# MisEty/RTG-SLAM

Measured on AMD Instinct MI355X. Metric: hot_path_units_per_sec, higher is better.
Workload: dtype f32; 1 GPU; `value` counts UNITS, not SLAM frames (the SLAM frame rate by the reference's definition is `slam_frames_per_sec`, from the `slam_sequence` leg of --full).  One UNIT per step = 1 ICP track (3 levels x 5 GN iters, 1200x680, on a second HIP stream) + 1 map-optimisation iteration (raster fwd + masked L1 colour / gated depth loss + attach regulariser + raster bwd + fused Adam) over 1200000 random Gaus; gaussians=1200000, mode=single, parallelism=1 GPU

## Files before the change

include/rtgs_raster.h:

```cpp
#ifndef RTGS_RASTER_H
#define RTGS_RASTER_H

#include <stddef.h>
#include <stdint.h>

#ifdef __cplusplus
extern "C" {
#endif

#define RTGS_OK 0
#define RTGS_E_INVALID (-1)
#define RTGS_E_HIP (-2)
#define RTGS_E_ALLOC (-3)

#define RTGS_TILE 16

typedef struct rtgs_raster_settings {
  int32_t image_height;
  int32_t image_width;
  float tanfovx;
  float tanfovy;
  const float* bg;
  float scale_modifier;
  const float* viewmatrix;
// ... 168 lines not shown
                       float* m_raw8, float* v_raw8, const float* lr_xyz, const float* lr_shs, const float* lr_raw8,
                       uint8_t* ever_xyz, uint8_t* ever_shs, uint8_t* ever_raw8, int64_t rows, int32_t step, float beta1,
                       float beta2, float eps, const rtgs_attach* attach, float* confidence, const uint32_t* skip_flag,
                       const rtgs_activated* refresh, void* stream);

typedef struct rtgs_loss_cfg {
  float color_weight, depth_weight, ssim_weight, add_depth_thres;
  const uint8_t* render_mask;
  int32_t sums_zeroed;
} rtgs_loss_cfg;
size_t rtgs_slam_loss_scratch_bytes(int32_t H, int32_t W, int32_t with_ssim);
int rtgs_slam_loss(const float* color, const float* depth, const int32_t* depth_index, const float* gt_color,
                   const float* gt_depth, int32_t H, int32_t W, const rtgs_loss_cfg* cfg, void* scratch,
                   float* loss_out4, float* g_color, float* g_depth, void* stream);
int rtgs_slam_loss_sums(const float* color, const float* depth, const int32_t* depth_index, const float* gt_color,
                        const float* gt_depth, int32_t H, int32_t W, const rtgs_loss_cfg* cfg, void* scratch, void* stream);
int rtgs_slam_loss_grads(const float* color, const float* depth, const int32_t* depth_index, const float* gt_color,
                         const float* gt_depth, int32_t H, int32_t W, const rtgs_loss_cfg* cfg, void* scratch,
                         float* loss_out4, float* g_color, float* g_depth, void* stream);

typedef struct rtgs_map_step_args {
  const rtgs_raster_settings* settings;
  int32_t P, sh_coeffs;
  float *xyz, *shs, *raw8;
  const int32_t* tile_mask;
  const float *gt_color, *gt_depth;
  rtgs_loss_cfg loss;
  void* loss_scratch;
  float *opacity, *scales, *rotations, *normal;
  float *out_color, *out_depth;
  int32_t *out_color_index, *out_depth_index;
  float *out_color_weight, *out_depth_weight, *out_T;
  int32_t* out_radii;
  float *dL_dcolor, *dL_ddepth, *loss4;
  float *d_xyz, *d_opacity, *d_shs, *d_scales, *d_rotations, *d_normal, *d_raw8;
  void* grad_scratch;
  uint8_t* row_state;
  float *m_xyz, *v_xyz, *m_shs, *v_shs, *m_raw8, *v_raw8;
  const float *lr_xyz, *lr_shs, *lr_raw8;
  uint8_t *ever_xyz, *ever_shs, *ever_raw8;
  int32_t step;
  float beta1, beta2, eps;
  const rtgs_attach* attach;
  float* confidence;
  int32_t activated_valid;
  rtgs_resize_fn geom_resize; void* geom_user;
  rtgs_resize_fn binning_resize; void* binning_user;
  rtgs_resize_fn image_resize; void* image_user;
  float normal_weight;
  const float* gt_normal;
  int32_t train_begin, train_end;
  int32_t tail_mode;
  uint32_t* live_counts;
} rtgs_map_step_args;
int rtgs_slam_normal_loss(const float* normal_w, const int32_t* depth_index, const float* gt_normal,
                          const uint8_t* render_mask, int32_t H, int32_t W, float normal_weight, float* scratch2,
                          float* loss_out4, float* d_normal, uint8_t* row_state, const uint32_t* skip_flag, void* stream);
int rtgs_slam_normal_loss_range(const float* normal_w, const int32_t* depth_index, const float* gt_normal,
                                const uint8_t* render_mask, int32_t H, int32_t W, float normal_weight, float* scratch2,
                                float* loss_out4, float* d_normal, uint8_t* row_state, const uint32_t* skip_flag,
                                int32_t train_begin, int32_t train_end, void* stream);
int rtgs_slam_normal_loss_sums(const float* normal_w, const int32_t* depth_index, const float* gt_normal,
                               const uint8_t* render_mask, int32_t H, int32_t W, float* scratch2, const uint32_t* skip_flag,
                               void* stream);
int rtgs_slam_normal_loss_grads(const float* normal_w, const int32_t* depth_index, const float* gt_normal,
                                const uint8_t* render_mask, int32_t H, int32_t W, float normal_weight, const float* sums2,
                                float* loss_out4, float* d_normal, uint8_t* row_state, const uint32_t* skip_flag,
                                int32_t train_begin, int32_t train_end, void* stream);
int rtgs_slam_map_step(const rtgs_map_step_args* args, int64_t* num_rendered_host, void* stream);
void* rtgs_stream_create_reserving(int32_t reserve_cus);
void rtgs_stream_destroy(void* stream);
int rtgs_map_fused_tail(const rtgs_raster_settings* settings, const rtgs_map_step_args* args, void* geom_buffer,
                        const void* image_buffer, const uint32_t* spec_fail, uint32_t* live_counts2, void* stream);
int rtgs_map_fused_tail_hint(const rtgs_raster_settings* settings, const rtgs_map_step_args* args, void* geom_buffer,
                             const void* image_buffer, const uint32_t* spec_fail, uint32_t* live_counts2,
                             uint32_t listed_hint, void* stream);
uint32_t rtgs_raster_last_listed_ctx(rtgs_ctx* ctx);
int rtgs_raster_backward_buffers(int32_t P, int32_t image_height, int32_t image_width, size_t* out8_host);
int rtgs_raster_last_buffers_ctx(rtgs_ctx* ctx, void** out3_host);
void rtgs_raster_set_aux_zero_ctx(rtgs_ctx* ctx, void* eight_words);
int rtgs_slam_map_step_front(const rtgs_map_step_args* args, int64_t* num_rendered_host, void* stream);
int rtgs_slam_map_step_ctx(rtgs_ctx* ctx, const rtgs_map_step_args* args, int64_t* num_rendered_host, void* stream);
int rtgs_slam_map_step_front_ctx(rtgs_ctx* ctx, const rtgs_map_step_args* args, int64_t* num_rendered_host, void* stream);

int rtgs_rows_pack(const uint8_t* row_state, int32_t P, float* d_xyz, float* d_shs, float* d_opacity, float* d_scales,
                   float* d_rotations, float* d_normal, float* out_list, int32_t capacity, uint32_t* count_scratch,
                   void* stream);
int rtgs_rows_overflow(const float* gathered_lists, int32_t world, int32_t capacity, uint32_t* flag_and_counts, void* stream);
int rtgs_rows_apply(const float* list, int32_t capacity, int32_t mode, float* d_xyz, float* d_shs, float* d_opacity,
                    float* d_scales, float* d_rotations, float* d_normal, uint8_t* row_state, const uint32_t* skip_flag,
                    void* stream);

size_t rtgs_map_step_args_size(void);
size_t rtgs_raster_settings_size(void);

const char* rtgs_version(void);

#ifdef __cplusplus
}
#endif
#endif
```

rtg_slam_amd/_lib.py:

```python
from __future__ import annotations

import ctypes as C
import os
import threading

_HERE = os.path.dirname(os.path.abspath(__file__))
LIB_PATH = os.environ.get("RTGS_LIB_PATH") or os.path.join(_HERE, "librtgs_hip.so")

RESIZE_FN = C.CFUNCTYPE(C.c_void_p, C.c_void_p, C.c_size_t)
FWD_NO_BACKWARD = 1


class RasterSettingsC(C.Structure):
    _fields_ = [
        ("image_height", C.c_int32), ("image_width", C.c_int32),
        ("tanfovx", C.c_float), ("tanfovy", C.c_float),
        ("bg", C.c_void_p), ("scale_modifier", C.c_float),
        ("viewmatrix", C.c_void_p), ("projmatrix", C.c_void_p),
        ("sh_degree", C.c_int32), ("campos", C.c_void_p),
        ("opaque_threshold", C.c_float), ("depth_threshold", C.c_float),
        ("normal_threshold", C.c_float), ("color_sigma", C.c_float),
        ("prefiltered", C.c_int32), ("debug", C.c_int32),
        ("cx", C.c_float), ("cy", C.c_float), ("T_threshold", C.c_float),
    ]


class IcpLevelC(C.Structure):
    _fields_ = [
        ("H", C.c_int32), ("W", C.c_int32), ("downscale", C.c_float), ("iters", C.c_int32),
        ("vertex_src", C.c_void_p), ("normal_src", C.c_void_p),
        ("vertex_tgt", C.c_void_p), ("normal_tgt", C.c_void_p),
    ]


_lock = threading.Lock()
_lib = None

_P = C.c_void_p


class LossCfgC(C.Structure):
    _fields_ = [("color_weight", C.c_float), ("depth_weight", C.c_float), ("ssim_weight", C.c_float),
                ("add_depth_thres", C.c_float), ("render_mask", C.c_void_p), ("sums_zeroed", C.c_int32)]


class AttachC(C.Structure):
    _fields_ = [("init_xyz", C.c_void_p), ("init_raw8", C.c_void_p), ("attach_info", C.c_void_p)]


class ActivatedC(C.Structure):
    _fields_ = [(n, C.c_void_p) for n in ("opacity", "scales", "rotations", "normal")]


class MapStepArgsC(C.Structure):
    _fields_ = (
        [("settings", C.POINTER(RasterSettingsC)), ("P", C.c_int32), ("sh_coeffs", C.c_int32)]
        + [(n, C.c_void_p) for n in ("xyz", "shs", "raw8", "tile_mask", "gt_color", "gt_depth")]
        + [("loss", LossCfgC), ("loss_scratch", C.c_void_p)]
        + [(n, C.c_void_p) for n in (
            "opacity", "scales", "rotations", "normal", "out_color", "out_depth", "out_color_index", "out_depth_index",
            "out_color_weight", "out_depth_weight", "out_T", "out_radii", "dL_dcolor", "dL_ddepth", "loss4",
            "d_xyz", "d_opacity", "d_shs", "d_scales", "d_rotations", "d_normal", "d_raw8", "grad_scratch", "row_state",
            "m_xyz", "v_xyz", "m_shs", "v_shs", "m_raw8", "v_raw8", "lr_xyz", "lr_shs", "lr_raw8",
            "ever_xyz", "ever_shs", "ever_raw8")]
        + [("step", C.c_int32), ("beta1", C.c_float), ("beta2", C.c_float), ("eps", C.c_float)]
        + [("attach", C.POINTER(AttachC)), ("confidence", C.c_void_p), ("activated_valid", C.c_int32)]
        + [("geom_resize", RESIZE_FN), ("geom_user", C.c_void_p), ("binning_resize", RESIZE_FN),
           ("binning_user", C.c_void_p), ("image_resize", RESIZE_FN), ("image_user", C.c_void_p)]
        + [("normal_weight", C.c_float), ("gt_normal", C.c_void_p), ("train_begin", C.c_int32), ("train_end", C.c_int32),
           ("tail_mode", C.c_int32), ("live_counts", C.c_void_p)])


_SIGNATURES = {
    "rtgs_version": (C.c_char_p, []),
    "rtgs_raster_forward": (C.c_int, [C.POINTER(RasterSettingsC), C.c_int32, C.c_int32] + [_P] * 6 + [_P]
                            + [_P] * 8 + [RESIZE_FN, _P, RESIZE_FN, _P, RESIZE_FN, _P,
                                          C.POINTER(C.c_int64), _P]),
    "rtgs_raster_backward": (C.c_int, [C.POINTER(RasterSettingsC), C.c_int32, C.c_int32, C.c_int64] + [_P] * 6
                             + [_P] * 3 + [_P, _P, _P] + [_P, _P] + [_P] * 6 + [_P, _P]),
    "rtgs_raster_backward_rows": (C.c_int, [C.POINTER(RasterSettingsC), C.c_int32, C.c_int32, C.c_int64] + [_P] * 6
                                  + [_P] * 3 + [_P, _P, _P] + [_P, _P] + [_P] * 6 + [_P, _P, _P]),
    "rtgs_raster_backward_scratch_bytes": (C.c_size_t, [C.c_int32]),
    "rtgs_raster_geom_bytes": (C.c_size_t, [C.c_int32, C.c_int32, C.c_int32]),
    "rtgs_raster_binning_bytes": (C.c_size_t, [C.c_int64, C.c_int32, C.c_int32]),
    "rtgs_raster_image_bytes": (C.c_size_t, [C.c_int32, C.c_int32]),
    "rtgs_raster_last_stats": (C.c_int, [C.POINTER(C.c_int64)]),
    "rtgs_raster_set_counters": (None, [_P]),
    "rtgs_fused_adam": (C.c_int, [_P, _P, _P, _P, _P, C.c_int64, C.c_int32, C.c_int32, C.c_float, C.c_float, C.c_float, _P]),
    "rtgs_fused_adam_rows": (C.c_int, [_P, _P, _P, _P, _P, _P, _P, C.c_int64, C.c_int32, C.c_int32, C.c_float, C.c_float, C.c_float, _P]),
    "rtgs_map_activate8_forward": (C.c_int, [_P, C.c_int64, _P, _P, _P, _P, _P]),
    "rtgs_map_activate8_backward": (C.c_int, [_P, C.c_int64, _P, _P, _P, _P, _P, _P]),
    "rtgs_map_activate8_backward_rows": (C.c_int, [_P, C.c_int64, _P, _P, _P, _P, _P, _P, _P]),
    "rtgs_map_tail_rows": (C.c_int, [_P] * 23 + [C.c_int64, C.c_int32, C.c_float, C.c_float, C.c_float,
                                     C.POINTER(AttachC), _P, _P, C.POINTER(ActivatedC), _P]),
    "rtgs_attach_prepare": (C.c_int, [_P, _P, C.POINTER(AttachC), C.c_int64, _P]),
    "rtgs_history_merge": (C.c_int, [_P] * 8 + [C.c_int64, C.c_float, _P]),
    "rtgs_map_fused_tail": (C.c_int, [C.POINTER(RasterSettingsC), C.POINTER(MapStepArgsC), _P, _P, _P, _P, _P]),
    "rtgs_map_fused_tail_hint": (C.c_int, [C.POINTER(RasterSettingsC), C.POINTER(MapStepArgsC), _P, _P, _P, _P, C.c_uint32, _P]),
    "rtgs_raster_last_listed_ctx": (C.c_uint32, [_P]),
    "rtgs_stream_create_reserving": (C.c_void_p, [C.c_int]),
    "rtgs_stream_destroy": (None, [_P]),
    "rtgs_raster_backward_buffers": (C.c_int, [C.c_int32, C.c_int32, C.c_int32, C.POINTER(C.c_size_t)]),
    "rtgs_raster_last_buffers_ctx": (C.c_int, [_P, C.POINTER(C.c_void_p)]),
    "rtgs_raster_set_aux_zero_ctx": (None, [_P, _P]),
    "rtgs_raster_backward_walk_ctx": (C.c_int, [_P, C.POINTER(RasterSettingsC), C.c_int32, C.c_int32, C.c_int64] + [_P] * 6
                                      + [_P] * 3 + [_P, _P, _P] + [_P, _P] + [_P] * 6 + [_P, _P, C.c_int32, C.c_int32, _P]),
    "rtgs_slam_loss_scratch_bytes": (C.c_size_t, [C.c_int32, C.c_int32, C.c_int32]),
    "rtgs_slam_map_step_front": (C.c_int, [C.POINTER(MapStepArgsC), C.POINTER(C.c_int64), _P]),
    "rtgs_rows_pack": (C.c_int, [_P, C.c_int32] + [_P] * 7 + [C.c_int32, _P, _P]),
    "rtgs_rows_overflow": (C.c_int, [_P, C.c_int32, C.c_int32, _P, _P]),
    "rtgs_rows_apply": (C.c_int, [_P, C.c_int32, C.c_int32] + [_P] * 7 + [_P, _P]),
    "rtgs_map_step_args_size": (C.c_size_t, []),
    "rtgs_raster_settings_size": (C.c_size_t, []),
    "rtgs_slam_map_step": (C.c_int, [C.POINTER(MapStepArgsC), C.POINTER(C.c_int64), _P]),
    "rtgs_slam_loss": (C.c_int, [_P, _P, _P, _P, _P, C.c_int32, C.c_int32, C.POINTER(LossCfgC), _P, _P, _P, _P, _P]),
    "rtgs_slam_normal_loss": (C.c_int, [_P, _P, _P, _P, C.c_int32, C.c_int32, C.c_float, _P, _P, _P, _P, _P, _P]),
    "rtgs_slam_loss_sums": (C.c_int, [_P, _P, _P, _P, _P, C.c_int32, C.c_int32, C.POINTER(LossCfgC), _P, _P]),
    "rtgs_slam_loss_grads": (C.c_int, [_P, _P, _P, _P, _P, C.c_int32, C.c_int32, C.POINTER(LossCfgC), _P, _P, _P, _P, _P]),
    "rtgs_raster_set_profiling": (None, [C.c_int]),
    "rtgs_raster_force_sort_path": (None, [C.c_int]),
    "rtgs_raster_set_near_slice": (None, [C.c_int, C.c_int]),
    "rtgs_raster_last_slice_stats": (C.c_int, [C.POINTER(C.c_int64)]),
    "rtgs_raster_last_timings": (C.c_int, [C.POINTER(C.c_float)]),
    "rtgs_ctx_create": (C.c_void_p, []),
    "rtgs_ctx_destroy": (None, [_P]),
    "rtgs_raster_forward_ctx": (C.c_int, [_P, C.POINTER(RasterSettingsC), C.c_int32, C.c_int32] + [_P] * 6 + [_P]
                                + [_P] * 8 + [RESIZE_FN, _P, RESIZE_FN, _P, RESIZE_FN, _P, C.POINTER(C.c_int64),
                                              C.c_int32, _P]),
    "rtgs_raster_backward_ctx": (C.c_int, [_P, C.POINTER(RasterSettingsC), C.c_int32, C.c_int32, C.c_int64] + [_P] * 6
                                 + [_P] * 3 + [_P, _P, _P] + [_P, _P] + [_P] * 6 + [_P, _P]),
    "rtgs_raster_backward_rows_ctx": (C.c_int, [_P, C.POINTER(RasterSettingsC), C.c_int32, C.c_int32, C.c_int64] + [_P] * 6
                                      + [_P] * 3 + [_P, _P, _P] + [_P, _P] + [_P] * 6 + [_P, _P, _P]),
    "rtgs_raster_backward_range_ctx": (C.c_int, [_P, C.POINTER(RasterSettingsC), C.c_int32, C.c_int32, C.c_int64] + [_P] * 6
                                       + [_P] * 3 + [_P, _P, _P] + [_P, _P] + [_P] * 6 + [_P, _P, C.c_int32, C.c_int32, _P]),
    "rtgs_slam_normal_loss_range": (C.c_int, [_P, _P, _P, _P, C.c_int32, C.c_int32, C.c_float, _P, _P, _P, _P, _P,
                                              C.c_int32, C.c_int32, _P]),
    "rtgs_slam_normal_loss_sums": (C.c_int, [_P, _P, _P, _P, C.c_int32, C.c_int32, _P, _P, _P]),
    "rtgs_slam_normal_loss_grads": (C.c_int, [_P, _P, _P, _P, C.c_int32, C.c_int32, C.c_float, _P, _P, _P, _P, _P,
                                              C.c_int32, C.c_int32, _P]),
    "rtgs_raster_geom_bytes_ctx": (C.c_size_t, [_P, C.c_int32, C.c_int32, C.c_int32]),
    "rtgs_raster_last_stats_ctx": (C.c_int, [_P, C.POINTER(C.c_int64)]),
    "rtgs_raster_set_counters_ctx": (None, [_P, _P]),
    "rtgs_raster_set_profiling_ctx": (None, [_P, C.c_int]),
    "rtgs_raster_force_sort_path_ctx": (None, [_P, C.c_int]),
    "rtgs_raster_set_bwd_walk_ctx": (None, [_P, C.c_int]),
    "rtgs_raster_set_bwd_debug": (None, [C.c_int]),
    "rtgs_raster_set_bwd_stamps": (None, [C.c_void_p]),
    "rtgs_raster_set_fwd_stamps": (None, [C.c_void_p]),
    "rtgs_icp_set_stamps": (None, [C.c_void_p]),
    "rtgs_raster_set_onepass_ctx": (None, [_P, C.c_int]),
    "rtgs_raster_forward_verify_ctx": (C.c_int, [_P, C.POINTER(C.c_int64)]),
    "rtgs_raster_spec_fail_ptr_ctx": (C.c_void_p, [_P]),
    "rtgs_raster_set_speculation_ctx": (None, [_P, C.c_int]),
    "rtgs_raster_speculation_stats_ctx": (C.c_int, [_P, C.POINTER(C.c_int64)]),
    "rtgs_raster_plain_stats_ctx": (C.c_int, [_P, C.POINTER(C.c_int64)]),
    "rtgs_raster_set_plain_onepass_ctx": (None, [_P, C.c_int]),
    "rtgs_raster_image_offsets": (C.c_int, [C.c_int32, C.c_int32, C.POINTER(C.c_size_t)]),
# ... 96 lines not shown
```

rtg_slam_amd/csrc/map_step.hip:

```cpp
#include <hip/hip_runtime.h>

#include "../../include/rtgs_raster.h"

static int map_step_front(rtgs_ctx* ctx, const rtgs_map_step_args* a, int64_t* num_rendered_host, int32_t fwd_flags,
                          void* stream, bool walk_only = false) {
  if (!a || !num_rendered_host || !a->settings) return RTGS_E_INVALID;
  const int32_t P = a->P, M = a->sh_coeffs;
  if (P <= 0 || M != 16 || a->step < 1) return RTGS_E_INVALID;
  if (!a->xyz || !a->shs || !a->raw8 || !a->tile_mask || !a->gt_color || !a->gt_depth) return RTGS_E_INVALID;
  const int32_t H = a->settings->image_height, W = a->settings->image_width;
  int rc = 0;
  if (!a->activated_valid) {
    rc = rtgs_map_activate8_forward(a->raw8, P, a->opacity, a->scales, a->rotations, a->normal, stream);
    if (rc != 0) return RTGS_E_HIP;
  }
  if (!a->loss_scratch || !a->loss4) return RTGS_E_INVALID;
  rtgs_raster_set_aux_zero_ctx(ctx, a->loss_scratch);
  rc = rtgs_raster_forward_ctx(ctx, a->settings, P, M, a->xyz, a->opacity, a->shs, a->scales, a->rotations, a->normal,
                           a->tile_mask, a->out_color, a->out_depth, a->out_color_index, a->out_depth_index,
                           a->out_color_weight, a->out_depth_weight, a->out_T, a->out_radii, a->geom_resize,
                           a->geom_user, a->binning_resize, a->binning_user, a->image_resize, a->image_user,
                           num_rendered_host, fwd_flags, stream);
  if (rc != RTGS_OK) return rc;
  void* bufs[3];
  if (rtgs_raster_last_buffers_ctx(ctx, bufs) != RTGS_OK) return RTGS_E_ALLOC;
  void *geom = bufs[0], *bin = bufs[1], *img = bufs[2];
  rtgs_loss_cfg lcfg = a->loss;
  lcfg.sums_zeroed = P > 0 ? 1 : 0;
  rc = rtgs_slam_loss(a->out_color, a->out_depth, a->out_depth_index, a->gt_color, a->gt_depth, H, W, &lcfg,
                      a->loss_scratch, a->loss4, a->dL_dcolor, a->dL_ddepth, stream);
  if (rc != 0) return RTGS_E_HIP;
  int32_t t0 = 0, t1 = P;
  if (a->train_begin != 0 || a->train_end != 0) { t0 = a->train_begin; t1 = a->train_end; }
  if (t0 < 0 || t1 > P || t1 < t0) return RTGS_E_INVALID;
  if (t1 == t0) return RTGS_OK;
  rc = (walk_only ? rtgs_raster_backward_walk_ctx : rtgs_raster_backward_range_ctx)(
      ctx, a->settings, P, M, *num_rendered_host, a->xyz, a->opacity, a->shs, a->scales, a->rotations, a->normal, geom, bin, img,
      a->out_color, a->out_T, a->out_depth_index, a->dL_dcolor, a->dL_ddepth, a->d_xyz, a->d_opacity, a->d_shs, a->d_scales,
      a->d_rotations, a->d_normal, a->grad_scratch, a->row_state, t0, t1, stream);
  if (rc != RTGS_OK) return rc;
  if (a->normal_weight > 0.f && a->gt_normal) {
    rc = rtgs_slam_normal_loss_range(a->normal, a->out_depth_index, a->gt_normal, a->loss.render_mask, H, W, a->normal_weight,
                                     reinterpret_cast<float*>(a->loss_scratch) + 5, a->loss4, a->d_normal, a->row_state,
                                     rtgs_raster_spec_fail_ptr_ctx(ctx), t0, t1, stream);
    if (rc != 0) return RTGS_E_HIP;
  }
  return RTGS_OK;
}

extern "C" int rtgs_slam_map_step_front_ctx(rtgs_ctx* ctx, const rtgs_map_step_args* a, int64_t* num_rendered_host,
                                            void* stream) {
  return map_step_front(ctx, a, num_rendered_host, 0, stream);
}

extern "C" int rtgs_slam_map_step_front(const rtgs_map_step_args* a, int64_t* num_rendered_host, void* stream) {
  return rtgs_slam_map_step_front_ctx(nullptr, a, num_rendered_host, stream);
}

static int map_step_once(rtgs_ctx* ctx, const rtgs_map_step_args* a, int64_t* num_rendered_host, bool speculate, void* stream) {
  const bool fused = a->tail_mode == 0 && !(a->normal_weight > 0.f && a->gt_normal);
  int rc = map_step_front(ctx, a, num_rendered_host, speculate ? RTGS_FWD_SPECULATE : 0, stream, fused);
  if (rc != RTGS_OK) return rc;
  if ((a->train_begin != 0 || a->train_end != 0) && a->train_end == a->train_begin) return RTGS_OK;
  if (fused) {
    void* bufs[3];
    if (rtgs_raster_last_buffers_ctx(ctx, bufs) != RTGS_OK) return RTGS_E_ALLOC;
    return rtgs_map_fused_tail_hint(a->settings, a, bufs[0], bufs[2], rtgs_raster_spec_fail_ptr_ctx(ctx), a->live_counts,
                                    rtgs_raster_last_listed_ctx(ctx), stream);
  }
  const int32_t P = a->P;
  int32_t t0 = 0, t1 = P;
  if (a->train_begin != 0 || a->train_end != 0) { t0 = a->train_begin; t1 = a->train_end; }
  const size_t o = (size_t)t0;
  const rtgs_activated act{a->opacity + o, a->scales + 3 * o, a->rotations + 4 * o, a->normal + 3 * o};
  rc = rtgs_map_tail_rows(a->xyz + 3 * o, a->shs + 48 * o, a->raw8 + 8 * o, a->d_opacity + o, a->d_scales + 3 * o,
                          a->d_rotations + 4 * o, a->d_normal + 3 * o, a->d_xyz + 3 * o, a->d_shs + 48 * o, a->d_raw8 + 8 * o,
                          a->row_state + o, a->m_xyz, a->v_xyz, a->m_shs, a->v_shs, a->m_raw8, a->v_raw8,
                          a->lr_xyz, a->lr_shs, a->lr_raw8, a->ever_xyz, a->ever_shs, a->ever_raw8, (int64_t)(t1 - t0), a->step,
                          a->beta1, a->beta2, a->eps, a->attach, a->confidence, rtgs_raster_spec_fail_ptr_ctx(ctx), &act, stream);
  return rc != 0 ? RTGS_E_HIP : RTGS_OK;
}

extern "C" int rtgs_slam_map_step_ctx(rtgs_ctx* ctx, const rtgs_map_step_args* a, int64_t* num_rendered_host, void* stream) {
  int rc = map_step_once(ctx, a, num_rendered_host, true, stream);
  const int v = rtgs_raster_forward_verify_ctx(ctx, num_rendered_host);
  if (rc != RTGS_OK) return rc;
  if (v < 0) return v;
  if (v == 1) rc = map_step_once(ctx, a, num_rendered_host, false, stream);
  return rc;
}

extern "C" int rtgs_slam_map_step(const rtgs_map_step_args* a, int64_t* num_rendered_host, void* stream) {
  return rtgs_slam_map_step_ctx(nullptr, a, num_rendered_host, stream);
}

extern "C" size_t rtgs_map_step_args_size(void) { return sizeof(rtgs_map_step_args); }
extern "C" size_t rtgs_raster_settings_size(void) { return sizeof(rtgs_raster_settings); }

extern "C" void* rtgs_stream_create_reserving(int32_t reserve_cus) {
  int dev = 0, cus = 0;
  if (hipGetDevice(&dev) != hipSuccess) return nullptr;
  if (hipDeviceGetAttribute(&cus, hipDeviceAttributeMultiprocessorCount, dev) != hipSuccess) return nullptr;
  if (reserve_cus <= 0 || reserve_cus >= cus || cus > 1024) return nullptr;
  uint32_t mask[32] = {0};
  const int words = (cus + 31) / 32;
  for (int i = 0; i < cus - reserve_cus; ++i) mask[i >> 5] |= 1u << (i & 31);
  hipStream_t s = nullptr;
  if (hipExtStreamCreateWithCUMask(&s, (uint32_t)words, mask) != hipSuccess) return nullptr;
  return (void*)s;
}
extern "C" void rtgs_stream_destroy(void* stream) {
  if (stream) (void)hipStreamDestroy((hipStream_t)stream);
}
```

rtg_slam_amd/csrc/raster_api.hip:

```cpp
#include "../../include/rtgs_raster.h"
#include "../../include/rtgs_debug.h"
#include "raster_common.h"

#include <rocprim/device/device_radix_sort.hpp>
#include <rocprim/device/device_scan.hpp>
#include <math.h>
#include <new>
#include <stdlib.h>
#include <string.h>

namespace rtgs {
void launch_mask_sat(const int32_t*, int, int, int32_t*, hipStream_t);
void launch_preprocess_fwd(const RasterParams&, const float*, const float*, const float*, const float*, const float*,
                           const float*, const int32_t*, Splat*, uint32_t*, int32_t*, uint8_t*, int32_t*, uint32_t*, int,
                           uint8_t*, hipStream_t);
void launch_emit_keys(const RasterParams&, const Splat*, const int32_t*, const uint32_t*, const int32_t*, uint64_t*,
                      uint32_t*, hipStream_t);
void launch_tile_ranges(int64_t, const uint64_t*, uint2*, hipStream_t);
void set_fwd_stamps(void* dev);
void set_bwd_debug(int bits);
void set_bwd_stamps(void* dev);
void launch_blend_fwd(const RasterParams&, const uint2*, const uint32_t*, const Splat*, float*, float*, int32_t*,
                      int32_t*, float*, float*, float*, uint32_t*, unsigned long long*, SlicePass, uint32_t*, uint32_t*, uint32_t*, int, uint32_t*,
                      TileCache, uint32_t, hipStream_t);
void launch_blend_bwd(const RasterParams&, const uint2*, const uint32_t*, const Splat*, const float*, const float*,
                      const uint32_t*, const int32_t*, const float*, const float*, const uint32_t*, uint32_t*,
                      const BwdInfo*, SplatGrad*, uint8_t*, const uint32_t*, int, uint32_t, uint32_t, hipStream_t);
void launch_blend_bwd_entry(const RasterParams&, const uint2*, const uint32_t*, const Splat*, const float*, const uint32_t*,
                            const int32_t*, const uint32_t*, const uint32_t*, const float*, const float*, const uint32_t*, uint32_t*,
                            const BwdInfo*, SplatGrad*, uint8_t*, const uint32_t*, uint32_t, uint32_t, TileCache, uint32_t, hipStream_t);
void launch_grad_reduce(int, const uint8_t*, const uint32_t*, uint32_t*, const BwdInfo*, SplatGrad*, const uint32_t*, hipStream_t);
void launch_preprocess_bwd(const RasterParams&, const float*, const float*, const float*, const float*, const float*,
                           const float*, const int32_t*, const uint8_t*, SplatGrad*, uint8_t*, uint8_t*, float*, float*,
                           float*, float*, float*, float*, hipStream_t);

size_t bin_lds_limit_tiles();
int bin_sort_capacity();
size_t bin_block_counts_bytes(int, int);
int launch_bin_count(const RasterParams&, const Splat*, const int32_t*, const int32_t*, uint32_t*, uint16_t*, SliceSel,
                     SliceList, size_t, hipStream_t);
size_t bin_slice_block_counts_bytes(int, size_t, int);
size_t bin_list_block_counts_bytes(int, int);
void launch_visible_compact(int, const uint8_t*, uint32_t*, uint32_t*, const uint32_t*, uint32_t*, uint32_t*, const uint32_t*, hipStream_t,
                            const SliceSel* = nullptr, int32_t* = nullptr, uint32_t* = nullptr);
void launch_slice_compact(int, SliceSel, uint32_t*, uint32_t*, const uint32_t*, uint32_t*, uint32_t*, uint32_t*, uint32_t, uint32_t*, hipStream_t);
void launch_slice_publish(int, const int32_t*, const int32_t*, const uint32_t*, uint32_t*, uint32_t*, uint32_t, uint32_t*, hipStream_t,
                          const uint32_t* seg_count = nullptr);
void launch_preprocess_cull(const RasterParams&, const float*, const float*, const float*, uint32_t*, int32_t*, int32_t*,
                            uint32_t*, int, uint8_t*, float2*, hipStream_t);
void launch_preprocess_shade(const RasterParams&, const float*, const float*, const float*, const float*, const float*,
                             const float*, Splat*, int32_t*, uint8_t*, float2*, SliceList, SliceSel, size_t, hipStream_t);
void launch_bin_tilescan(int, const uint32_t*, uint2*, uint32_t*, uint32_t*, uint32_t*, const uint32_t*, const uint32_t*,
                         const uint32_t*, const uint32_t*, uint32_t, SpecCaps, hipStream_t);
void launch_bin_scatter(const RasterParams&, const Splat*, const int32_t*, const int32_t*, const uint16_t*, uint32_t*,
                        unsigned long long*, SliceSel, SliceList, size_t, hipStream_t);
void launch_slice_hist(int, const uint8_t*, const uint32_t*, const int32_t*, uint32_t*, unsigned long long*, hipStream_t,
                       BwdInfoInit bi = BwdInfoInit{nullptr, nullptr, 0u, 0u});
void launch_bin_tilesort(int, uint32_t, const uint2*, const unsigned long long*, uint32_t*, const uint32_t*, hipStream_t,
                         const uint32_t* seg_count = nullptr, uint32_t seg = 0, uint2* ranges_out = nullptr,
                         const BinFinish* finish = nullptr);
void launch_bin_place(const RasterParams&, const Splat*, const int32_t*, const int32_t*, uint32_t*, unsigned long long*, uint32_t,
                      uint32_t*, SliceSel, SliceList, size_t, hipStream_t);

}

enum { EV_F0 = 0, EV_PRE, EV_SL_BIN, EV_SL_BLEND, EV_SCAN, EV_BIN0, EV_EMIT, EV_SORT, EV_RANGES, EV_BLEND0, EV_BLEND, EV_B0,
       EV_BWALK, EV_BBLEND, EV_BPRE, EV_N };
struct rtgs_ctx {
  int64_t stats[8] = {0};
  int slice_mode = 2;
  int slice_budget = 384;
  int64_t slice_stats[4] = {0};
  unsigned long long* counters = nullptr;
  uint32_t last_listed = 0;
  bool onepass = true;
  bool prof = false;
  bool force_sort_path = false;
  int bwd_walk = 0;
  bool ev_init = false;
  hipEvent_t ev[EV_N];
  bool ev_set[EV_N] = {false};
  uint32_t* info_host = nullptr;
  uint32_t seq = 0;
  const void* hint_geom = nullptr;
  bool hint_slice_lists = true, hint_main_lists = true;
  int hint_walk = -2;
  void *last_geom = nullptr, *last_bin = nullptr, *last_img = nullptr;
  uint32_t* aux_zero = nullptr;
  bool ask_first = false;
  struct Plan {
    bool valid = false;
    int32_t P = 0, H = 0, W = 0;
    int kind = -1;
    int slice_mode = 0, slice_budget = 0;
    uint32_t R = 0, R1 = 0, longest = 0, slots = 0, n_fin = 0;
    uint32_t R_hi = 0, longest_hi = 0, slots_hi = 0;
    void note(uint32_t r, uint32_t l, uint32_t s) {
      R = r; longest = l; slots = s;
      R_hi = r > R_hi - R_hi / 16 ? r : R_hi - R_hi / 16;
      longest_hi = l > longest_hi - longest_hi / 16 ? l : longest_hi - longest_hi / 16;
      slots_hi = s > slots_hi - slots_hi / 16 ? s : slots_hi - slots_hi / 16;
    }
  } plan;
  struct Spec {
    bool pending = false;
    int kind = -1;
    uint32_t seq = 0, capR = 0, capL = 0, capS = 0;
    const void* geom = nullptr;
    const uint32_t* fail_dev = nullptr;
    void* stream = nullptr;
    int32_t ntiles = 0;
    int64_t G_total = 0, B_total = 0, I_total = 0;
  } spec;
  bool speculation = true;
  int64_t spec_stats[3] = {0, 0, 0};
  Plan plan_plain;
  Plan plan_plain0;
  bool plain_onepass = true;
  int64_t plain_stats[2] = {0, 0};
};

namespace rtgs {

static rtgs_ctx* default_ctx() {
  static rtgs_ctx* c = [] {
    rtgs_ctx* n = new rtgs_ctx();
    if (const char* e = getenv("RTGS_NEAR_SLICE")) n->slice_mode = atoi(e);
    if (const char* e = getenv("RTGS_NEAR_SLICE_BUDGET")) { const int b = atoi(e); if (b > 0) n->slice_budget = b; }
    if (const char* e = getenv("RTGS_SPECULATE")) n->speculation = atoi(e) != 0;
    if (const char* e = getenv("RTGS_BIN_ONEPASS")) n->onepass = atoi(e) != 0;
    if (const char* e = getenv("RTGS_PLAIN_ONEPASS")) n->plain_onepass = atoi(e) != 0;
    if (const char* e = getenv("RTGS_BWD_WALK")) { const int m = atoi(e); n->bwd_walk = (m >= 1 && m <= 4) ? m : 0; }
    return n;
  }();
  return c;
}
static inline rtgs_ctx* use(rtgs_ctx* c) { return c ? c : default_ctx(); }

static void prof_mark(rtgs_ctx* c, int which, hipStream_t st) {
  if (!c->prof) return;
  if (!c->ev_init) {
// ... 85 lines not shown
    L.block_counts_vis = off; off = align_up(off + bin_list_block_counts_bytes((int)Pn, gx * gy));
    L.slice_seg = (Pn >= (size_t)large_map_min() && nt >= 256) ? (size_t)SLICE_MAX_LIST : 0;
    const size_t cap1 = L.slice_seg ? (nt * L.slice_seg > L.slice_cap ? nt * L.slice_seg : L.slice_cap) : L.slice_cap;
    L.list1 = off; off = align_up(off + cap1 * sizeof(uint32_t));
    L.block_counts1 = off; off = align_up(off + bin_slice_block_counts_bytes((int)Pn, L.slice_max_list, gx * gy));
    L.slice_ids = off; off = align_up(off + L.slice_max_list * sizeof(uint32_t));
    L.bucket1 = off; off = align_up(off + cap1 * sizeof(uint64_t));
  }
  size_t tb = 0, tb2 = 0;
  (void)rocprim::inclusive_scan(nullptr, tb, (uint32_t*)nullptr, (uint32_t*)nullptr, Pn, rocprim::plus<uint32_t>());
  (void)rocprim::exclusive_scan(nullptr, tb2, (uint32_t*)nullptr, (uint32_t*)nullptr, 0u, Pn, rocprim::plus<uint32_t>());
  if (tb2 > tb) tb = tb2;
  L.scan_temp_bytes = tb;
  L.scan_temp = off; off = align_up(off + tb);
  L.total = off;
  return L;
}

static BinLayout bin_layout(int64_t R, int ntiles, bool sort_path, size_t slots) {
  BinLayout L{};
  size_t off = 0;
  const size_t Rn = (size_t)(R > 0 ? R : 1);
  L.vals_b = off; off = align_up(off + Rn * sizeof(uint32_t));
  L.keys_a = off; off = align_up(off + Rn * sizeof(uint64_t));
  if (!sort_path) {
    L.keys_b = L.vals_a = L.sort_temp = off; L.sort_temp_bytes = 0;
    if (slots > 0) { L.slot_grads = off; off = align_up(off + slots * sizeof(SplatGrad)); }
    L.total = off;
    return L;
  }
  L.keys_b = off; off = align_up(off + Rn * sizeof(uint64_t));
  L.vals_a = off; off = align_up(off + Rn * sizeof(uint32_t));
  size_t tb = 0;
  (void)rocprim::radix_sort_pairs(nullptr, tb, (uint64_t*)nullptr, (uint64_t*)nullptr, (uint32_t*)nullptr,
                                  (uint32_t*)nullptr, Rn, 0u, (unsigned)(32 + bits_for((uint32_t)ntiles)));
  L.sort_temp_bytes = tb;
  L.sort_temp = off; off = align_up(off + tb);
  L.total = off;
  return L;
}

static ImgLayout img_layout(int H, int W, int ntiles) {
  ImgLayout L{};
  size_t off = 0;
  L.ranges = off; off = align_up(off + (size_t)ntiles * sizeof(uint2));
  L.n_contrib = off; off = align_up(off + (size_t)H * W * sizeof(uint32_t));
  L.bwd_info = off; off = align_up(off + sizeof(BwdInfo));
  L.tile_mode = off; off = align_up(off + (size_t)ntiles * sizeof(uint32_t));
  L.depth_pos = off; off = align_up(off + (size_t)H * W * sizeof(uint32_t));
  L.tile_last = off; off = align_up(off + (size_t)ntiles * sizeof(uint32_t));
  L.tile_recs = off; off = align_up(off + (size_t)ntiles * TILE_RECS * 3 * sizeof(float4));
  L.tile_masks = off; off = align_up(off + (size_t)ntiles * TILE_RECS * sizeof(uint16_t));
  L.depth_aux = off; off = align_up(off + (size_t)H * W * sizeof(float2));
  L.total = off;
  return L;
}

static int make_params(const rtgs_raster_settings* s, int32_t P, int32_t M, RasterParams& p) {
  if (!s || P < 0 || M < 1 || M > 16) return RTGS_E_INVALID;
  if (s->image_height <= 0 || s->image_width <= 0) return RTGS_E_INVALID;
  if (s->sh_degree < 0 || s->sh_degree > 3 || (s->sh_degree + 1) * (s->sh_degree + 1) > M) return RTGS_E_INVALID;
  if (!s->bg || !s->viewmatrix || !s->campos) return RTGS_E_INVALID;
  p.H = s->image_height; p.W = s->image_width;
  p.gx = (p.W + TILE - 1) / TILE; p.gy = (p.H + TILE - 1) / TILE;
  p.P = P; p.M = M; p.deg = s->sh_degree;
  p.tanfovx = s->tanfovx; p.tanfovy = s->tanfovy;
  p.fx = (float)(p.W / (2.0 * (double)s->tanfovx));
  p.fy = (float)(p.H / (2.0 * (double)s->tanfovy));
  p.cx = s->cx > 0.f ? s->cx : 0.5f * (float)(p.W - 1);
  p.cy = s->cy > 0.f ? s->cy : 0.5f * (float)(p.H - 1);
  p.scale_modifier = s->scale_modifier;
  p.opaque_thr = s->opaque_threshold; p.depth_thr = s->depth_threshold; p.normal_thr = s->normal_threshold;
  p.color_sigma = s->color_sigma; p.T_thr = s->T_threshold;
  p.view = s->viewmatrix; p.campos = s->campos; p.bg = s->bg;
  p.spec_fail = nullptr;
  return RTGS_OK;
}

#define HIP_TRY(expr)                         \
  do {                                        \
    hipError_t e_ = (expr);                   \
    if (e_ != hipSuccess) return RTGS_E_HIP;  \
  } while (0)

static int dbg_sync(const rtgs_raster_settings* s, hipStream_t st) {
  if (s->debug) {
    HIP_TRY(hipStreamSynchronize(st));
    HIP_TRY(hipGetLastError());
  }
  return RTGS_OK;
}
#define DBG(s, st)                              \
  do {                                          \
    int r_ = dbg_sync(s, st);                   \
    if (r_ != RTGS_OK) return r_;               \
  } while (0)

}

using namespace rtgs;

extern "C" {

const char* rtgs_version(void) { return "rtgs-hip 0.2.0 (gfx950)"; }

rtgs_ctx* rtgs_ctx_create(void) {
  rtgs_ctx* c = new (std::nothrow) rtgs_ctx();
  if (c) { c->slice_mode = default_ctx()->slice_mode; c->slice_budget = default_ctx()->slice_budget; c->bwd_walk = default_ctx()->bwd_walk; c->onepass = default_ctx()->onepass; c->speculation = default_ctx()->speculation; c->plain_onepass = default_ctx()->plain_onepass; }
  return c;
}
void rtgs_ctx_destroy(rtgs_ctx* c) {
  if (!c || c == default_ctx()) return;
  if (c->ev_init) for (int i = 0; i < EV_N; ++i) (void)hipEventDestroy(c->ev[i]);
  if (c->info_host) (void)hipHostFree(c->info_host);
  delete c;
}

size_t rtgs_raster_geom_bytes_ctx(rtgs_ctx* c, int32_t P, int32_t H, int32_t W) {
  return geom_layout(P, (W + TILE - 1) / TILE, (H + TILE - 1) / TILE, use(c)->slice_budget).total;
}
size_t rtgs_raster_geom_bytes(int32_t P, int32_t H, int32_t W) { return rtgs_raster_geom_bytes_ctx(nullptr, P, H, W); }
size_t rtgs_raster_binning_bytes(int64_t R, int32_t H, int32_t W) {
  const int gx = (W + TILE - 1) / TILE, gy = (H + TILE - 1) / TILE;
  return bin_layout(R, gx * gy, true, 0).total;
}
size_t rtgs_raster_image_bytes(int32_t H, int32_t W) {
  const int gx = (W + TILE - 1) / TILE, gy = (H + TILE - 1) / TILE;
  return img_layout(H, W, gx * gy).total;
}
size_t rtgs_raster_backward_scratch_bytes(int32_t P) {
  const size_t n = (size_t)(P > 0 ? P : 1);
  return align_up(n * sizeof(SplatGrad)) + align_up(n);
}

int rtgs_raster_last_stats_ctx(rtgs_ctx* c, int64_t* out) {
  if (!out) return RTGS_E_INVALID;
  memcpy(out, use(c)->stats, sizeof(use(c)->stats));
  return RTGS_OK;
}
void rtgs_raster_set_counters_ctx(rtgs_ctx* c, void* counters) { use(c)->counters = (unsigned long long*)counters; }

int rtgs_raster_forward_ctx(rtgs_ctx* ctx, const rtgs_raster_settings* s, int32_t P, int32_t M, const float* means3D,
                            const float* opacities, const float* shs, const float* scales, const float* rotations,
                            const float* normal_w, const int32_t* tile_mask, float* out_color, float* out_depth,
                            int32_t* out_cidx, int32_t* out_didx, float* out_cw, float* out_dw, float* out_T,
                            int32_t* out_radii, rtgs_resize_fn geom_resize, void* geom_user,
                            rtgs_resize_fn binning_resize, void* binning_user, rtgs_resize_fn image_resize,
                            void* image_user, int64_t* num_rendered_host, int32_t flags, void* stream) {
  rtgs_ctx* c = use(ctx);
  uint32_t* const aux_zero = c->aux_zero;
  c->aux_zero = nullptr;
  RasterParams p;
  int rc = make_params(s, P, M, p);
  if (rc != RTGS_OK) return rc;
  if (P > 0 && (!means3D || !opacities || !shs || !scales || !rotations || !normal_w)) return RTGS_E_INVALID;
  if (!tile_mask || !out_color || !out_depth || !out_cidx || !out_didx || !out_cw || !out_dw || !out_T)
    return RTGS_E_INVALID;
  if (!geom_resize || !binning_resize || !image_resize || !num_rendered_host) return RTGS_E_INVALID;
  hipStream_t st = (hipStream_t)stream;
  const int ntiles = p.gx * p.gy;

  const GeomLayout G = geom_layout(P, p.gx, p.gy, c->slice_budget);
  char* geom = (char*)geom_resize(geom_user, G.total);
  const ImgLayout I = img_layout(p.H, p.W, ntiles);
  char* img = (char*)image_resize(image_user, I.total);
  if (!geom || !img) return RTGS_E_ALLOC;
  Splat* splats = (Splat*)(geom + G.splats);
  uint32_t* tiles_touched = (uint32_t*)(geom + G.tiles_touched);
  uint32_t* offsets = (uint32_t*)(geom + G.offsets);
  int32_t* radii = (int32_t*)(geom + G.radii);
  uint8_t* clamped = (uint8_t*)(geom + G.clamped);
  int32_t* sat = (int32_t*)(geom + G.sat);
  uint2* ranges = (uint2*)(img + I.ranges);
  uint32_t* n_contrib = (uint32_t*)(img + I.n_contrib);
  uint32_t* depth_pos = (uint32_t*)(img + I.depth_pos);
  uint32_t* tile_last = (uint32_t*)(img + I.tile_last);
  uint32_t* const tile_mode = (uint32_t*)(img + I.tile_mode);
  const int fwd_walk = c->bwd_walk == 0 || c->bwd_walk == 3 ? 2 : (c->bwd_walk == 4 ? -1 : c->bwd_walk - 1);
  c->last_geom = geom; c->last_img = img; c->last_bin = nullptr;
  const TileCache tcache = (flags & RTGS_FWD_NO_BACKWARD) ? TileCache{nullptr, nullptr, nullptr}
                                                          : TileCache{(float4*)(img + I.tile_recs), (uint16_t*)(img + I.tile_masks), (float2*)(img + I.depth_aux)};

  int64_t R = 0, R1 = 0;
  for (int i = 0; i < EV_B0; ++i) c->ev_set[i] = false;
  prof_mark(c, EV_F0, st);
  uint32_t* tile_count = (uint32_t*)(geom + G.tile_count);
  uint32_t* cursor = (uint32_t*)(geom + G.cursor);
  uint32_t* info = (uint32_t*)(geom + G.info);
  uint16_t* block_counts = (uint16_t*)(geom + G.block_counts);
  uint32_t* zero_words = (uint32_t*)(geom + G.zero_begin);
  const int zero_n = (int)((G.zero_end - G.zero_begin) / sizeof(uint32_t));
  uint32_t* tile_count1 = (uint32_t*)(geom + G.tile_count1);
  uint2* ranges1_bwd = (uint2*)(geom + G.ranges1_bwd);
  uint32_t* slice_hist = (uint32_t*)(geom + G.slice_hist);
  unsigned long long* slice_cover = (unsigned long long*)(geom + G.slice_cover);
  uint32_t* slice_ctr = (uint32_t*)(geom + G.slice_ctr);
  uint8_t* zbin = (uint8_t*)(geom + G.zbin);
  uint2* ranges1 = (uint2*)(geom + G.ranges1);
  int32_t* mask2 = (int32_t*)(geom + G.mask2);
  uint32_t* list1 = (uint32_t*)(geom + G.list1);
  uint32_t longest = 0;
  const uint32_t seg1 = c->onepass ? (uint32_t)G.slice_seg : 0u;
  const bool want_bwd = !(flags & RTGS_FWD_NO_BACKWARD);
  uint32_t slots = 0;
  auto scan_all = [&]() -> int {
    size_t tb = G.scan_temp_bytes;
    HIP_TRY(rocprim::exclusive_scan(geom + G.scan_temp, tb, tiles_touched, offsets, 0u, (size_t)P, rocprim::plus<uint32_t>(), st));
    return RTGS_OK;
  };
  bool sort_path = (size_t)ntiles > bin_lds_limit_tiles() || c->force_sort_path;
  const bool slice_auto = c->slice_mode == 2;
  bool sliced = !sort_path && P > 0 && (c->slice_mode == 1 || (slice_auto && P >= large_map_min() && ntiles >= 256));
  const bool sliced0 = sliced;
  SlicePass pass{0, nullptr, nullptr, nullptr, nullptr};
  bool declined = false, considered = false;
  SliceList vis{nullptr, nullptr};
  if (!c->info_host) {
    HIP_TRY(hipHostMalloc((void**)&c->info_host, HOST_WORDS * sizeof(uint32_t), hipHostMallocCoherent));
    memset(c->info_host, 0, HOST_WORDS * sizeof(uint32_t));
  }
  uint32_t* const info_host = c->info_host;
  uint32_t pub[7] = {0, 0, 0, 0, 0, 0, 0};
  auto wait_published = [&](uint32_t seq) -> int { return wait_published_words(info_host, seq, st, pub); };
  const int32_t* mask_main = tile_mask;
  uint32_t n_left = 0, n_fin = 0;

  if (c->spec.pending) return RTGS_E_INVALID;
  c->spec.geom = nullptr; c->spec.fail_dev = nullptr;
  {
    rtgs_ctx::Plan& pp = sliced ? c->plan_plain : c->plan_plain0;
    const bool immediate = !(flags & RTGS_FWD_SPECULATE) && !want_bwd && c->speculation && c->plain_onepass && c->onepass &&
                           P > 0 && !sort_path && !s->debug && pp.valid && (sliced ? (pp.kind == 2 && G.slice_seg) : pp.kind == 0) &&
// ... 2 lines not shown
    const bool eligible = immediate ||
                          ((flags & RTGS_FWD_SPECULATE) && c->speculation && want_bwd && P > 0 && !sort_path && !s->debug &&
                           pl.valid && pl.P == P && pl.H == p.H && pl.W == p.W && pl.slice_mode == c->slice_mode &&
                           pl.slice_budget == c->slice_budget && (pl.kind == 0 ? !sliced : (pl.kind == 1 || pl.kind == 2) && sliced));
    const uint32_t capR = pl.R_hi + pl.R_hi / 8u + 8192u, capL = sort_class_cap(pl.longest_hi),
                   capS = immediate ? 0u : pl.slots_hi + pl.slots_hi / 8u + 8192u;
    if ((flags & RTGS_FWD_SPECULATE) && !(eligible && (pl.kind == 1 || capS <= SLOTS_MAX))) ++c->spec_stats[2];
    if (eligible && (pl.kind == 1 || capS <= SLOTS_MAX)) {
      uint32_t* const fail = slice_ctr + 6;
      const SliceSel sel1{1, zbin, slice_hist, (uint32_t)G.slice_cap, (uint32_t)G.slice_max_list, slice_ctr, nullptr, nullptr,
                          slice_cover, (uint32_t)ntiles * (uint32_t)(TILE * TILE), slice_auto ? 1 : 0};
      const SpecCaps nocaps{nullptr, 0u, 0u, 0u, nullptr};
      if (++c->seq == 0u) c->seq = 1u;
      size_t b_total = 0;
      bool seg_main = false;
      if (pl.kind == 1) {
        launch_preprocess_cull(p, means3D, scales, rotations, tiles_touched, radii, out_radii, zero_words, zero_n, zbin,
                               (float2*)(geom + G.uv), st);
        prof_mark(c, EV_PRE, st);
        const uint32_t sl = (uint32_t)G.slice_cap;
        const bool use_sl = sl > 0 && sl <= SLOTS_MAX;
        const BinLayout B = bin_layout(0, ntiles, false, use_sl ? (size_t)sl : 0);
        char* bin = (char*)binning_resize(binning_user, B.total);
        if (!bin) return RTGS_E_ALLOC;
        c->last_bin = bin;
        b_total = B.total;
        launch_slice_hist(P, zbin, tiles_touched, radii, slice_hist, slice_cover, st,
                          BwdInfoInit{(BwdInfo*)(img + I.bwd_info), (SplatGrad*)(bin + B.slot_grads), use_sl ? sl : 0u, use_sl ? 1u : 0u});
        launch_slice_compact(P, sel1, (uint32_t*)(geom + G.slice_ids), slice_ctr + 2, tiles_touched, offsets, slice_ctr + 4,
                             nullptr, 0u, nullptr, st);
        const SliceList work{(const uint32_t*)(geom + G.slice_ids), slice_ctr + 2};
        launch_preprocess_shade(p, means3D, opacities, shs, scales, rotations, normal_w, splats, radii, clamped,
                                (float2*)(geom + G.uv), work, sel1, G.slice_max_list, st);
        if (seg1) {
          launch_bin_place(p, splats, radii, tile_mask, tile_count1, (unsigned long long*)(geom + G.bucket1), seg1, nullptr,
                           sel1, work, G.slice_max_list, st);
          launch_bin_tilesort(ntiles, (uint32_t)SLICE_MAX_LIST, ranges1, (const unsigned long long*)(geom + G.bucket1), list1,
                              nullptr, st, tile_count1, seg1, ranges1);
        } else {
        if (launch_bin_count(p, splats, radii, tile_mask, tile_count1, (uint16_t*)(geom + G.block_counts1), sel1, work,
                             G.slice_max_list, st) != 0)
          return RTGS_E_HIP;
        launch_bin_tilescan(ntiles, tile_count1, ranges1, (uint32_t*)(geom + G.cursor1), info + 2, nullptr, nullptr,
                            nullptr, nullptr, nullptr, 0u, nocaps, st);
        launch_bin_scatter(p, splats, radii, tile_mask, (const uint16_t*)(geom + G.block_counts1),
                           (uint32_t*)(geom + G.cursor1), (unsigned long long*)(geom + G.bucket1), sel1, work,
                           G.slice_max_list, st);
        launch_bin_tilesort(ntiles, (uint32_t)SLICE_MAX_LIST, ranges1, (const unsigned long long*)(geom + G.bucket1), list1,
                            nullptr, st);
        }
        prof_mark(c, EV_SL_BIN, st);
        const SlicePass pass1{1, tile_mask, mask2, ranges1_bwd, ranges};
        launch_blend_fwd(p, ranges1, list1, splats, out_color, out_depth, out_cidx, out_didx, out_cw, out_dw, out_T,
                         n_contrib, c->counters, pass1, tile_mode, depth_pos, tile_last, fwd_walk, aux_zero, tcache, seg1, st);
        prof_mark(c, EV_SL_BLEND, st);
        launch_slice_publish(ntiles, tile_mask, mask2, info + 2, slice_ctr, info_host, c->seq, fail, st, seg1 ? tile_count1 : nullptr);
        prof_mark(c, EV_BLEND0, st); prof_mark(c, EV_BLEND, st);
        c->hint_slice_lists = true; c->hint_main_lists = false;
        c->slice_stats[0] = 1; c->slice_stats[1] = pl.R1; c->slice_stats[2] = pl.n_fin; c->slice_stats[3] = 0;
      } else {
        const uint32_t seg2 = (c->onepass && ((pl.kind == 2 && G.slice_seg) || (immediate && pl.kind == 0))) ? capL : 0u;
        const BinLayout B = bin_layout(seg2 ? (int64_t)ntiles * (int64_t)seg2 : (int64_t)capR, ntiles, false, (size_t)capS);
        seg_main = seg2 != 0u;
        char* bin = (char*)binning_resize(binning_user, B.total);
        if (!bin) return RTGS_E_ALLOC;
        c->last_bin = bin;
        b_total = B.total;
        RasterParams pg = p;
        pg.spec_fail = fail;
        SliceList vl{nullptr, nullptr};
        if (pl.kind == 2) {
          launch_preprocess_cull(p, means3D, scales, rotations, tiles_touched, radii, out_radii, zero_words, zero_n, zbin,
                                 (float2*)(geom + G.uv), st);
          prof_mark(c, EV_PRE, st);
          launch_slice_hist(P, zbin, tiles_touched, radii, slice_hist, slice_cover, st,
                            BwdInfoInit{(BwdInfo*)(img + I.bwd_info), (SplatGrad*)(bin + B.slot_grads), capS, immediate ? 0u : 1u});
          vl = SliceList{(const uint32_t*)(geom + G.vis_ids), slice_ctr + 4};
          launch_visible_compact(P, zbin, (uint32_t*)(geom + G.vis_ids), slice_ctr + 4, tiles_touched, offsets, slice_ctr + 5, fail, st,
                                 &sel1, (int32_t*)(slice_ctr + 3), fail);
          launch_preprocess_shade(pg, means3D, opacities, shs, scales, rotations, normal_w, splats, radii, clamped,
                                  (float2*)(geom + G.uv), vl, sel1, (size_t)P, st);
        } else {
          launch_preprocess_fwd(p, means3D, opacities, shs, scales, rotations, normal_w, nullptr, splats, tiles_touched, radii,
                                clamped, out_radii, zero_words, zero_n, nullptr, st);
          if (!immediate && (rc = scan_all()) != RTGS_OK) return rc;
          prof_mark(c, EV_PRE, st);
        }
        const SliceSel sel2{0, nullptr, nullptr, 0u, 0u, slice_ctr, nullptr, (const float2*)(geom + G.uv), nullptr, 0u, 0};
        if (seg2) {
          if (pl.kind != 2)
            hipLaunchKernelGGL(bwd_info_kernel, dim3(1), dim3(1), 0, st, (BwdInfo*)(img + I.bwd_info),
                               (SplatGrad*)(bin + B.slot_grads), capS, immediate ? 0u : 1u);
          launch_bin_place(pg, splats, radii, tile_mask, tile_count, (unsigned long long*)(bin + B.keys_a), seg2, fail, sel2, vl,
                           (size_t)P, st);
          prof_mark(c, EV_SCAN, st); prof_mark(c, EV_BIN0, st); prof_mark(c, EV_EMIT, st);
          const BinFinish fin{tile_count, ntiles, info, info_host, slice_ctr + 5, nullptr, slice_ctr + 4, c->seq,
                              SpecCaps{fail, 0xffffffffu, capL, immediate ? 0xffffffffu : capS,
                                       pl.kind == 2 ? (const int32_t*)(slice_ctr + 3) : nullptr}};
          launch_bin_tilesort(ntiles, capL, ranges, (const unsigned long long*)(bin + B.keys_a), (uint32_t*)(bin + B.vals_b), fail, st,
                              tile_count, seg2, ranges, &fin);
        } else {
        if (launch_bin_count(pg, splats, radii, tile_mask, tile_count, vl.ids ? (uint16_t*)(geom + G.block_counts_vis) : block_counts,
                             sel2, vl, (size_t)P, st) != 0)
          return RTGS_E_HIP;
        const SpecCaps caps{fail, capR, capL, immediate ? 0xffffffffu : capS, pl.kind == 2 ? (const int32_t*)(slice_ctr + 3) : nullptr};
        launch_bin_tilescan(ntiles, tile_count, ranges, cursor, info, info_host, nullptr, nullptr,
                            vl.ids ? slice_ctr + 5 : offsets + (P - 1), vl.ids ? nullptr : tiles_touched + (P - 1), c->seq, caps, st);
        prof_mark(c, EV_SCAN, st);
        if (pl.kind != 2)
          hipLaunchKernelGGL(bwd_info_kernel, dim3(1), dim3(1), 0, st, (BwdInfo*)(img + I.bwd_info),
                             (SplatGrad*)(bin + B.slot_grads), capS, 1u);
        prof_mark(c, EV_BIN0, st);
        launch_bin_scatter(pg, splats, radii, tile_mask, vl.ids ? (const uint16_t*)(geom + G.block_counts_vis) : block_counts,
                           cursor, (unsigned long long*)(bin + B.keys_a), sel2, vl, (size_t)P, st);
        prof_mark(c, EV_EMIT, st);
        launch_bin_tilesort(ntiles, capL, ranges, (const unsigned long long*)(bin + B.keys_a), (uint32_t*)(bin + B.vals_b), fail, st);
        }
        prof_mark(c, EV_SORT, st);
        prof_mark(c, EV_BLEND0, st);
        launch_blend_fwd(pg, ranges, (uint32_t*)(bin + B.vals_b), splats, out_color, out_depth, out_cidx, out_didx, out_cw,
                         out_dw, out_T, n_contrib, c->counters, SlicePass{0, nullptr, nullptr, nullptr, nullptr}, tile_mode, depth_pos, tile_last, fwd_walk, aux_zero, tcache, seg2, st);
        prof_mark(c, EV_BLEND, st);
        c->hint_slice_lists = false; c->hint_main_lists = true;
        c->slice_stats[0] = pl.kind == 2 ? 1 : 0; c->slice_stats[1] = 0; c->slice_stats[2] = 0;
        c->slice_stats[3] = pl.kind == 2 ? (int64_t)ntiles : 0;
      }
      HIP_TRY(hipGetLastError());
      c->hint_geom = geom; c->hint_walk = fwd_walk;
      if (immediate) {
        if ((rc = wait_published(c->seq)) != RTGS_OK) return rc;
        const bool ok = (seg_main || pub[0] <= capR) && pub[1] <= capL && (pl.kind != 2 || (int32_t)pub[6] < 0);
        ++c->plain_stats[0];
        if (ok) {
          pp.note(pub[0], pub[1], 0u);
          c->last_listed = pub[2];
          c->plan.valid = false;
          c->stats[0] = (int64_t)pub[0]; c->stats[1] = 32 + bits_for((uint32_t)ntiles); c->stats[2] = ntiles;
          c->stats[3] = (int64_t)G.total; c->stats[4] = (int64_t)b_total; c->stats[5] = (int64_t)I.total; c->stats[6] = 1;
          c->stats[7] = (int64_t)pub[1];
          *num_rendered_host = (int64_t)pub[0];
          return RTGS_OK;
        }
        pp.valid = false;
        ++c->plain_stats[1];
      } else {
      c->spec.pending = true; c->spec.kind = pl.kind; c->spec.seq = c->seq; c->spec.capR = seg_main ? 0xffffffffu : capR; c->spec.capL = capL;
      c->spec.capS = capS; c->spec.geom = geom; c->spec.fail_dev = fail; c->spec.stream = stream; c->spec.ntiles = ntiles;
      c->spec.G_total = (int64_t)G.total; c->spec.B_total = (int64_t)b_total; c->spec.I_total = (int64_t)I.total;
      ++c->spec_stats[0];
      *num_rendered_host = (int64_t)pl.R + (int64_t)pl.R1;
      if (*num_rendered_host < 1) *num_rendered_host = 1;
      return RTGS_OK;
      }
    }
  }
  if (P == 0) HIP_TRY(hipMemsetAsync(zero_words, 0, (size_t)zero_n * sizeof(uint32_t), st));
  if (P > 0) {
    if (sort_path) {
      launch_mask_sat(tile_mask, p.gx, p.gy, sat, st);
      DBG(s, st);
    }
    const SliceSel sel1{1, zbin, slice_hist, (uint32_t)G.slice_cap, (uint32_t)G.slice_max_list, slice_ctr, nullptr, nullptr,
                        slice_cover, (uint32_t)ntiles * (uint32_t)(TILE * TILE), slice_auto ? 1 : 0};
    if (!sliced) {
      launch_preprocess_fwd(p, means3D, opacities, shs, scales, rotations, normal_w, sort_path ? sat : nullptr, splats,
                            tiles_touched, radii, clamped, out_radii, zero_words, zero_n, nullptr, st);
      if (!sort_path && want_bwd && (rc = scan_all()) != RTGS_OK) return rc;
    } else {
      launch_preprocess_cull(p, means3D, scales, rotations, tiles_touched, radii, out_radii, zero_words, zero_n, zbin,
                             (float2*)(geom + G.uv), st);
    }
    DBG(s, st);
    prof_mark(c, EV_PRE, st);
    if (sliced) {
      launch_slice_hist(P, zbin, tiles_touched, radii, slice_hist, slice_cover, st);
      const bool ask = slice_auto && c->ask_first;
      if (ask && ++c->seq == 0u) c->seq = 1u;
      launch_slice_compact(P, sel1, (uint32_t*)(geom + G.slice_ids), slice_ctr + 2, tiles_touched, offsets, slice_ctr + 4,
                           ask ? info_host : nullptr, c->seq, nullptr, st);
      if (ask) {
        if ((rc = wait_published(c->seq)) != RTGS_OK) return rc;
        declined = (int32_t)pub[6] < 0;
      }
    }
    if (sliced && declined) {
      vis = SliceList{(const uint32_t*)(geom + G.vis_ids), slice_ctr + 4};
      launch_visible_compact(P, zbin, (uint32_t*)(geom + G.vis_ids), slice_ctr + 4, tiles_touched, offsets, slice_ctr + 5, nullptr, st);
      launch_preprocess_shade(p, means3D, opacities, shs, scales, rotations, normal_w, splats, radii, clamped,
                              (float2*)(geom + G.uv), vis, sel1, (size_t)P, st);
      sliced = false;
      considered = true;
    }
    if (sliced) {
      const SliceList work{(const uint32_t*)(geom + G.slice_ids), slice_ctr + 2};
      launch_preprocess_shade(p, means3D, opacities, shs, scales, rotations, normal_w, splats, radii, clamped,
                              (float2*)(geom + G.uv), work, sel1, G.slice_max_list, st);
      if (seg1) {
        launch_bin_place(p, splats, radii, tile_mask, tile_count1, (unsigned long long*)(geom + G.bucket1), seg1, nullptr,
                         sel1, work, G.slice_max_list, st);
        launch_bin_tilesort(ntiles, (uint32_t)SLICE_MAX_LIST, ranges1, (const unsigned long long*)(geom + G.bucket1), list1,
                            nullptr, st, tile_count1, seg1, ranges1);
      } else {
      if (launch_bin_count(p, splats, radii, tile_mask, tile_count1, (uint16_t*)(geom + G.block_counts1), sel1, work,
                           G.slice_max_list, st) != 0)
        return RTGS_E_HIP;
      launch_bin_tilescan(ntiles, tile_count1, ranges1, (uint32_t*)(geom + G.cursor1), info + 2, nullptr, nullptr,
                          nullptr, nullptr, nullptr, 0u, SpecCaps{nullptr, 0u, 0u, 0u, nullptr}, st);
      launch_bin_scatter(p, splats, radii, tile_mask, (const uint16_t*)(geom + G.block_counts1),
                         (uint32_t*)(geom + G.cursor1), (unsigned long long*)(geom + G.bucket1), sel1, work,
                         G.slice_max_list, st);
      launch_bin_tilesort(ntiles, (uint32_t)SLICE_MAX_LIST, ranges1, (const unsigned long long*)(geom + G.bucket1), list1,
                          nullptr, st);
      }
      DBG(s, st);
      prof_mark(c, EV_SL_BIN, st);
      if (++c->seq == 0u) c->seq = 1u;
      const SlicePass pass1{1, tile_mask, mask2, ranges1_bwd, ranges};
      launch_blend_fwd(p, ranges1, list1, splats, out_color, out_depth, out_cidx, out_didx, out_cw, out_dw, out_T,
                       n_contrib, c->counters, pass1, tile_mode, depth_pos, tile_last, fwd_walk, aux_zero, tcache, seg1, st);
      prof_mark(c, EV_SL_BLEND, st);
      launch_slice_publish(ntiles, tile_mask, mask2, info + 2, slice_ctr, info_host, c->seq, nullptr, st, seg1 ? tile_count1 : nullptr);
      DBG(s, st);
      if ((rc = wait_published(c->seq)) != RTGS_OK) return rc;
      n_left = pub[2]; n_fin = pub[3];
      R1 = (int64_t)pub[4];
      if (n_left > 0) {
        mask_main = mask2;
        pass = SlicePass{2, nullptr, mask2, nullptr, nullptr};
        launch_mask_sat(mask2, p.gx, p.gy, sat, st);
        SliceSel sel_rest = sel1;
        sel_rest.sat = sat; sel_rest.uv = (const float2*)(geom + G.uv);
        launch_preprocess_shade(p, means3D, opacities, shs, scales, rotations, normal_w, splats, radii, clamped,
                                (float2*)(geom + G.uv), SliceList{nullptr, nullptr}, sel_rest, 0, st);
        if (want_bwd && (rc = scan_all()) != RTGS_OK) return rc;
      } else if (want_bwd) {
        slots = (uint32_t)G.slice_cap;
      }
    }
    if (!sort_path && !(sliced && n_left == 0)) {
      const SliceSel sel2{sliced ? 2 : 0, nullptr, nullptr, 0u, 0u, slice_ctr, sliced ? sat : nullptr,
                          (const float2*)(geom + G.uv), nullptr, 0u, 0};
      if (launch_bin_count(p, splats, radii, mask_main, tile_count,
                           vis.ids ? (uint16_t*)(geom + G.block_counts_vis) : block_counts, sel2, vis, (size_t)P, st) != 0)
        return RTGS_E_HIP;
      if (++c->seq == 0u) c->seq = 1u;
      launch_bin_tilescan(ntiles, tile_count, ranges, cursor, info, info_host, nullptr, nullptr,
                          want_bwd ? (vis.ids ? slice_ctr + 5 : offsets + (P - 1)) : nullptr,
                          want_bwd && !vis.ids ? tiles_touched + (P - 1) : nullptr, c->seq,
                          SpecCaps{nullptr, 0u, 0u, 0u, nullptr}, st);
      DBG(s, st);
      prof_mark(c, EV_SCAN, st);
      if ((rc = wait_published(c->seq)) != RTGS_OK) return rc;
      R = (int64_t)pub[0];
      longest = pub[1];
      slots = pub[5];
      if ((int)longest > bin_sort_capacity()) {
        sort_path = true;
        if (sliced) {
          HIP_TRY(hipMemsetAsync(ranges1_bwd, 0, (size_t)ntiles * sizeof(uint2), st));
          sliced = false; R1 = 0; n_left = n_fin = 0;
          pass = SlicePass{0, nullptr, nullptr, nullptr, nullptr};
          mask_main = tile_mask;
        }
        launch_mask_sat(tile_mask, p.gx, p.gy, sat, st);
        launch_preprocess_fwd(p, means3D, opacities, shs, scales, rotations, normal_w, sat, splats, tiles_touched,
                              radii, clamped, out_radii, nullptr, 0, nullptr, st);
        DBG(s, st);
      }
    }
    if (sort_path) {
      size_t tb = G.scan_temp_bytes;
      HIP_TRY(rocprim::inclusive_scan(geom + G.scan_temp, tb, tiles_touched, offsets, (size_t)P, rocprim::plus<uint32_t>(), st));
      uint32_t total = 0;
      HIP_TRY(hipMemcpyAsync(&total, offsets + (P - 1), sizeof(uint32_t), hipMemcpyDeviceToHost, st));
      prof_mark(c, EV_SCAN, st);
      HIP_TRY(hipStreamSynchronize(st));
      R = (int64_t)total;
    }
  }
  *num_rendered_host = R + R1;

  const bool use_slots = want_bwd && !sort_path && slots > 0 && slots <= SLOTS_MAX;
  const BinLayout B = bin_layout(R, ntiles, sort_path, use_slots ? (size_t)slots : 0);
  char* bin = (char*)binning_resize(binning_user, B.total);
  if (!bin) return RTGS_E_ALLOC;
  c->last_bin = bin;
  hipLaunchKernelGGL(bwd_info_kernel, dim3(1), dim3(1), 0, st, (BwdInfo*)(img + I.bwd_info),
                     (SplatGrad*)(bin + B.slot_grads), use_slots ? slots : 0u, use_slots ? 1u : 0u);
  uint64_t* keys_a = (uint64_t*)(bin + B.keys_a);
  uint64_t* keys_b = (uint64_t*)(bin + B.keys_b);
  uint32_t* vals_a = (uint32_t*)(bin + B.vals_a);
  uint32_t* vals_b = (uint32_t*)(bin + B.vals_b);

  const int sort_bits = 32 + bits_for((uint32_t)ntiles);
  if (P == 0 || sort_path) HIP_TRY(hipMemsetAsync(ranges, 0, (size_t)ntiles * sizeof(uint2), st));
  if (R > 0 && !sort_path) {
    prof_mark(c, EV_BIN0, st);
    launch_bin_scatter(p, splats, radii, mask_main, vis.ids ? (const uint16_t*)(geom + G.block_counts_vis) : block_counts, cursor,
                       (unsigned long long*)keys_a,
                       SliceSel{sliced ? 2 : 0, nullptr, nullptr, 0u, 0u, slice_ctr, sliced ? sat : nullptr,
                                (const float2*)(geom + G.uv), nullptr, 0u, 0},
                       vis, (size_t)P, st);
    DBG(s, st);
    prof_mark(c, EV_EMIT, st);
    launch_bin_tilesort(ntiles, longest, ranges, (const unsigned long long*)keys_a, vals_b, nullptr, st);
    DBG(s, st);
    prof_mark(c, EV_SORT, st);
  } else if (R > 0) {
    prof_mark(c, EV_BIN0, st);
    launch_emit_keys(p, splats, radii, offsets, tile_mask, keys_a, vals_a, st);
    DBG(s, st);
    prof_mark(c, EV_EMIT, st);
    size_t tb = B.sort_temp_bytes;
    HIP_TRY(rocprim::radix_sort_pairs(bin + B.sort_temp, tb, keys_a, keys_b, vals_a, vals_b, (size_t)R, 0u,
                                      (unsigned)sort_bits, st));
    DBG(s, st);
    prof_mark(c, EV_SORT, st);
    launch_tile_ranges(R, keys_b, ranges, st);
    DBG(s, st);
    prof_mark(c, EV_RANGES, st);
  }
  prof_mark(c, EV_BLEND0, st);
  if (!sliced || n_left > 0)
    launch_blend_fwd(p, ranges, vals_b, splats, out_color, out_depth, out_cidx, out_didx, out_cw, out_dw, out_T,
                     n_contrib, c->counters, pass, tile_mode, depth_pos, tile_last, fwd_walk, aux_zero, tcache, 0u, st);
  prof_mark(c, EV_BLEND, st);
  DBG(s, st);
  HIP_TRY(hipGetLastError());
  c->stats[0] = R + R1; c->stats[1] = sort_bits; c->stats[2] = ntiles; c->stats[3] = (int64_t)G.total;
  c->stats[4] = (int64_t)B.total; c->stats[5] = (int64_t)I.total;
  c->stats[6] = sort_path ? 0 : 1; c->stats[7] = (int64_t)longest;
  c->slice_stats[0] = (sliced || considered) ? 1 : 0; c->slice_stats[1] = R1; c->slice_stats[2] = n_fin;
  c->slice_stats[3] = considered ? (int64_t)ntiles : (int64_t)n_left;
  if (slice_auto && (sliced || considered)) c->ask_first = considered || (R1 == 0 && n_fin == 0);
  c->hint_geom = geom; c->hint_slice_lists = sliced && n_fin > 0; c->hint_main_lists = R > 0; c->hint_walk = fwd_walk;
  {
    rtgs_ctx::Plan& pl = c->plan;
    const bool same_shape = pl.valid && pl.P == P && pl.H == p.H && pl.W == p.W;
    pl.kind = sort_path ? -1 : ((sliced && n_left == 0) ? 1 : (considered ? 2 : (!sliced && P > 0 ? 0 : -1)));
    pl.valid = pl.kind >= 0 && want_bwd && R <= 0xffffffffll;
    pl.P = P; pl.H = p.H; pl.W = p.W; pl.slice_mode = c->slice_mode; pl.slice_budget = c->slice_budget;
    if (!same_shape || !pl.valid) { pl.R_hi = pl.longest_hi = pl.slots_hi = 0; }
    pl.note((uint32_t)R, longest, slots);
    pl.R1 = (uint32_t)R1; pl.n_fin = n_fin;
    if (!want_bwd) {
      rtgs_ctx::Plan& pp = sliced0 ? c->plan_plain : c->plan_plain0;
      const bool same_image = pp.valid && pp.H == p.H && pp.W == p.W;
      pp.kind = sort_path ? -1 : (sliced0 ? (considered ? 2 : -1) : (P > 0 ? 0 : -1));
      pp.valid = pp.kind >= 0 && R <= 0xffffffffll;
      pp.P = P; pp.H = p.H; pp.W = p.W; pp.slice_mode = c->slice_mode; pp.slice_budget = c->slice_budget;
      if (!same_image || !pp.valid) { pp.R_hi = pp.longest_hi = pp.slots_hi = 0; }
      pp.note((uint32_t)R, longest, 0u);
    }
  }
  return RTGS_OK;
}

static int backward_impl(rtgs_ctx* ctx, const rtgs_raster_settings* s, int32_t P, int32_t M, int64_t R, const float* means3D,
                         const float* opacities, const float* shs, const float* scales, const float* rotations,
                         const float* normal_w, void* geom_buffer, void* binning_buffer,
                         const void* image_buffer, const float* out_color, const float* out_T,
                         const int32_t* out_didx,
                         const float* dL_dcolor, const float* dL_ddepth, float* dL_dmeans3D, float* dL_dopacities,
                         float* dL_dshs, float* dL_dscales, float* dL_drotations, float* dL_dnormal_w,
                         void* grad_scratch, uint8_t* row_state, int32_t train_begin, int32_t train_end, void* stream,
                         bool walk_only = false) {
  rtgs_ctx* c = use(ctx);
  RasterParams p;
  int rc = make_params(s, P, M, p);
  if (rc != RTGS_OK) return rc;
  if (P == 0) return RTGS_OK;
  if (c->spec.geom == geom_buffer && c->spec.fail_dev) p.spec_fail = c->spec.fail_dev;
  if (!means3D || !opacities || !shs || !scales || !rotations || !normal_w || !geom_buffer || !binning_buffer ||
      !image_buffer || !out_color || !out_T || !out_didx || !dL_dcolor || !dL_ddepth || !grad_scratch || R < 0)
    return RTGS_E_INVALID;
  if (!walk_only && (!dL_dmeans3D || !dL_dopacities || !dL_dshs || !dL_dscales || !dL_drotations || !dL_dnormal_w)) return RTGS_E_INVALID;
  hipStream_t st = (hipStream_t)stream;
  const int ntiles = p.gx * p.gy;
  const GeomLayout G = geom_layout(P, p.gx, p.gy, 1);
  const BinLayout B = bin_layout(R, ntiles, false, 0);
  const ImgLayout I = img_layout(p.H, p.W, ntiles);
  const char* geom = (const char*)geom_buffer;
  const char* bin = (const char*)binning_buffer;
  const char* img = (const char*)image_buffer;
  SplatGrad* grads = (SplatGrad*)grad_scratch;
  for (int i = EV_B0; i < EV_N; ++i) c->ev_set[i] = false;
  prof_mark(c, EV_B0, st);
  uint8_t* touched = (uint8_t*)grad_scratch + align_up((size_t)P * sizeof(SplatGrad));
  if (!row_state) HIP_TRY(hipMemsetAsync(grads, 0, rtgs_raster_backward_scratch_bytes(P), st));
  const BwdInfo* binfo = (const BwdInfo*)(img + I.bwd_info);
  const uint32_t* gbase = (const uint32_t*)(geom + G.offsets);
  const int32_t* radii = (const int32_t*)(geom + G.radii);
  uint32_t* slot_count = (uint32_t*)(geom + G.slot_count);
  const uint32_t* tile_mode = (const uint32_t*)(img + I.tile_mode);
  if (R > 0) {
    const bool hinted = c->hint_geom == geom_buffer;
    const int which = !hinted ? 7 : (c->hint_walk == 2 ? 4 : (c->hint_walk == -1 ? 3 : (c->hint_walk == 0 ? 1 : 2)));
    if (train_begin < 0 || train_end > P || train_end < train_begin) return RTGS_E_INVALID;
    const uint32_t t0 = (uint32_t)train_begin, tn = (uint32_t)(train_end - train_begin);
    const uint32_t* depth_pos = (const uint32_t*)(img + I.depth_pos);
    for (int set = 0; set < 2; ++set) {
      if (hinted && !(set == 0 ? c->hint_slice_lists : c->hint_main_lists)) continue;
      const uint2* rg = set == 0 ? (const uint2*)(geom + G.ranges1_bwd) : (const uint2*)(img + I.ranges);
      const uint32_t* pl = set == 0 ? (const uint32_t*)(geom + G.list1) : (const uint32_t*)(bin + B.vals_b);
      if (which & 3)
        launch_blend_bwd(p, rg, pl, (const Splat*)(geom + G.splats), out_color, out_T, (const uint32_t*)(img + I.n_contrib),
                         out_didx, dL_dcolor, dL_ddepth, gbase, slot_count, binfo, grads, touched, tile_mode, which & 3, t0, tn, st);
      if (which & 4)
        launch_blend_bwd_entry(p, rg, pl, (const Splat*)(geom + G.splats), out_color, (const uint32_t*)(img + I.n_contrib),
                               out_didx, depth_pos, (const uint32_t*)(img + I.tile_last), dL_dcolor, dL_ddepth, gbase, slot_count, binfo, grads,
                               touched, tile_mode, t0, tn,
                               TileCache{(float4*)(img + I.tile_recs), (uint16_t*)(img + I.tile_masks), (float2*)(img + I.depth_aux)},
                               set == 0 ? (uint32_t)(BLOCK / 4) : (uint32_t)BLOCK,
                               st);
    }
    prof_mark(c, EV_BWALK, st);
    if (!walk_only) launch_grad_reduce(P, touched, gbase, slot_count, binfo, grads, p.spec_fail, st);
    DBG(s, st);
  }
  prof_mark(c, EV_BBLEND, st);
  if (walk_only) { prof_mark(c, EV_BPRE, st); HIP_TRY(hipGetLastError()); return RTGS_OK; }
  launch_preprocess_bwd(p, means3D, opacities, shs, scales, rotations, normal_w, radii,
                        (const uint8_t*)(geom + G.clamped), grads, touched, row_state, dL_dmeans3D, dL_dopacities,
                        dL_dshs, dL_dscales, dL_drotations, dL_dnormal_w, st);
  prof_mark(c, EV_BPRE, st);
  DBG(s, st);
  HIP_TRY(hipGetLastError());
  return RTGS_OK;
}

int rtgs_raster_backward_ctx(rtgs_ctx* ctx, const rtgs_raster_settings* s, int32_t P, int32_t M, int64_t R,
                             const float* means3D, const float* opacities, const float* shs, const float* scales,
                             const float* rotations, const float* normal_w, void* geom_buffer,
                             void* binning_buffer, const void* image_buffer, const float* out_color,
                             const float* out_T, const int32_t* out_didx, const float* dL_dcolor, const float* dL_ddepth,
                             float* dL_dmeans3D, float* dL_dopacities, float* dL_dshs, float* dL_dscales,
                             float* dL_drotations, float* dL_dnormal_w, void* grad_scratch, void* stream) {
  return backward_impl(ctx, s, P, M, R, means3D, opacities, shs, scales, rotations, normal_w, geom_buffer, binning_buffer,
                       image_buffer, out_color, out_T, out_didx, dL_dcolor, dL_ddepth, dL_dmeans3D, dL_dopacities,
                       dL_dshs, dL_dscales, dL_drotations, dL_dnormal_w, grad_scratch, nullptr, 0, P, stream);
}

int rtgs_raster_backward_rows_ctx(rtgs_ctx* ctx, const rtgs_raster_settings* s, int32_t P, int32_t M, int64_t R,
                                  const float* means3D, const float* opacities, const float* shs, const float* scales,
                                  const float* rotations, const float* normal_w, void* geom_buffer,
                                  void* binning_buffer, const void* image_buffer, const float* out_color,
                                  const float* out_T, const int32_t* out_didx, const float* dL_dcolor,
                                  const float* dL_ddepth, float* dL_dmeans3D, float* dL_dopacities, float* dL_dshs,
                                  float* dL_dscales, float* dL_drotations, float* dL_dnormal_w, void* grad_scratch,
                                  uint8_t* row_state, void* stream) {
  return rtgs_raster_backward_range_ctx(ctx, s, P, M, R, means3D, opacities, shs, scales, rotations, normal_w, geom_buffer,
                                        binning_buffer, image_buffer, out_color, out_T, out_didx, dL_dcolor, dL_ddepth,
                                        dL_dmeans3D, dL_dopacities, dL_dshs, dL_dscales, dL_drotations, dL_dnormal_w,
                                        grad_scratch, row_state, 0, P, stream);
}

int rtgs_raster_backward_range_ctx(rtgs_ctx* ctx, const rtgs_raster_settings* s, int32_t P, int32_t M, int64_t R,
                                   const float* means3D, const float* opacities, const float* shs, const float* scales,
                                   const float* rotations, const float* normal_w, void* geom_buffer,
                                   void* binning_buffer, const void* image_buffer, const float* out_color,
                                   const float* out_T, const int32_t* out_didx, const float* dL_dcolor,
                                   const float* dL_ddepth, float* dL_dmeans3D, float* dL_dopacities, float* dL_dshs,
                                   float* dL_dscales, float* dL_drotations, float* dL_dnormal_w, void* grad_scratch,
                                   uint8_t* row_state, int32_t train_begin, int32_t train_end, void* stream) {
  if (P > 0 && !row_state) return RTGS_E_INVALID;
  return backward_impl(ctx, s, P, M, R, means3D, opacities, shs, scales, rotations, normal_w, geom_buffer, binning_buffer,
                       image_buffer, out_color, out_T, out_didx, dL_dcolor, dL_ddepth, dL_dmeans3D, dL_dopacities,
// ... 33 lines not shown
  if (rc != RTGS_OK) { c->plan.valid = false; return rc; }
  rtgs_ctx::Plan& pl = c->plan;
  bool ok;
  if (c->spec.kind == 1) {
    const uint32_t n_left = pub[2];
    ok = n_left == 0u;
    pl.R1 = pub[4]; pl.n_fin = pub[3]; pl.R = 0; pl.longest = 0;
    c->last_listed = pub[0];
    c->slice_stats[1] = pub[4]; c->slice_stats[2] = pub[3]; c->slice_stats[3] = n_left;
  } else {
    ok = pub[0] <= c->spec.capR && pub[1] <= c->spec.capL && pub[5] <= c->spec.capS && (c->spec.kind != 2 || (int32_t)pub[6] < 0);
    pl.note(pub[0], pub[1], pub[5]); pl.R1 = 0;
    c->last_listed = pub[2];
  }
  c->stats[0] = (int64_t)pl.R + (int64_t)pl.R1; c->stats[1] = 32 + bits_for((uint32_t)c->spec.ntiles); c->stats[2] = c->spec.ntiles;
  c->stats[3] = c->spec.G_total; c->stats[4] = c->spec.B_total; c->stats[5] = c->spec.I_total; c->stats[6] = 1;
  c->stats[7] = (int64_t)pl.longest;
  if (num_rendered_host) *num_rendered_host = c->stats[0] > 0 ? c->stats[0] : 1;
  if (!ok) { pl.valid = false; ++c->spec_stats[1]; }
  return ok ? 0 : 1;
}
const uint32_t* rtgs_raster_spec_fail_ptr_ctx(rtgs_ctx* ctx) {
  rtgs_ctx* c = use(ctx);
  return c->spec.pending ? c->spec.fail_dev : nullptr;
}
void rtgs_raster_set_speculation_ctx(rtgs_ctx* ctx, int enable) {
  rtgs_ctx* c = use(ctx);
  c->speculation = enable != 0;
  c->plan = rtgs_ctx::Plan();
}
int rtgs_raster_speculation_stats_ctx(rtgs_ctx* ctx, int64_t* out3) {
  if (!out3) return RTGS_E_INVALID;
  memcpy(out3, use(ctx)->spec_stats, sizeof(use(ctx)->spec_stats));
  return RTGS_OK;
}
int rtgs_raster_plain_stats_ctx(rtgs_ctx* ctx, int64_t* out2) {
  if (!out2) return RTGS_E_INVALID;
  memcpy(out2, use(ctx)->plain_stats, sizeof(use(ctx)->plain_stats));
  return RTGS_OK;
}
void rtgs_raster_set_plain_onepass_ctx(rtgs_ctx* ctx, int enable) {
  rtgs_ctx* c = use(ctx);
  c->plain_onepass = enable != 0;
  c->plan_plain = rtgs_ctx::Plan();
  c->plan_plain0 = rtgs_ctx::Plan();
}
uint32_t rtgs_raster_last_listed_ctx(rtgs_ctx* c) { return use(c)->last_listed; }
void rtgs_raster_set_bwd_debug(int bits) { rtgs::set_bwd_debug(bits); }
void rtgs_raster_set_bwd_stamps(void* dev) { rtgs::set_bwd_stamps(dev); }
void rtgs_raster_set_fwd_stamps(void* dev) { rtgs::set_fwd_stamps(dev); }
void rtgs_raster_set_onepass_ctx(rtgs_ctx* c, int on) { use(c)->onepass = on != 0; use(c)->plan.valid = false; }
void rtgs_raster_set_bwd_walk_ctx(rtgs_ctx* c, int mode) { use(c)->bwd_walk = (mode >= 1 && mode <= 4) ? mode : 0; }
void rtgs_raster_set_aux_zero_ctx(rtgs_ctx* ctx, void* eight_words) { use(ctx)->aux_zero = (uint32_t*)eight_words; }
int rtgs_raster_last_buffers_ctx(rtgs_ctx* ctx, void** out3) {
  rtgs_ctx* c = use(ctx);
  if (!out3 || !c->last_geom || !c->last_bin || !c->last_img) return RTGS_E_INVALID;
  out3[0] = c->last_geom; out3[1] = c->last_bin; out3[2] = c->last_img;
  return RTGS_OK;
}
int rtgs_raster_backward_buffers(int32_t P, int32_t H, int32_t W, size_t* out) {
  if (!out || P < 0 || H <= 0 || W <= 0) return RTGS_E_INVALID;
  const int gx = (W + TILE - 1) / TILE, gy = (H + TILE - 1) / TILE;
  const GeomLayout G = geom_layout(P, gx, gy, 1);
  const ImgLayout I = img_layout(H, W, gx * gy);
  out[0] = G.clamped; out[1] = G.offsets; out[2] = G.slot_count; out[3] = I.bwd_info;
  out[4] = align_up((size_t)(P > 0 ? P : 1) * sizeof(SplatGrad)); out[5] = G.radii; out[6] = 0; out[7] = 0;
  return RTGS_OK;
}
int rtgs_raster_image_offsets(int32_t H, int32_t W, size_t* out) {
  if (!out || H <= 0 || W <= 0) return RTGS_E_INVALID;
  const int gx = (W + TILE - 1) / TILE, gy = (H + TILE - 1) / TILE;
  const ImgLayout I = img_layout(H, W, gx * gy);
  out[0] = I.ranges; out[1] = I.n_contrib; out[2] = I.bwd_info; out[3] = I.tile_mode; out[4] = I.total; out[5] = I.depth_pos;
  return RTGS_OK;
}

int rtgs_raster_last_timings_ctx(rtgs_ctx* ctx, float* ms) {
  rtgs_ctx* c = use(ctx);
  if (!ms) return RTGS_E_INVALID;
  for (int i = 0; i < 12; ++i) ms[i] = -1.f;
  if (!c->ev_init) return RTGS_OK;
  const int pre_end = c->ev_set[EV_SL_BLEND] ? EV_SL_BLEND : EV_PRE;
  const int pairs[11][2] = {{EV_F0, EV_PRE}, {pre_end, EV_SCAN}, {EV_BIN0, EV_EMIT}, {EV_EMIT, EV_SORT},
                            {EV_SORT, EV_RANGES}, {EV_BLEND0, EV_BLEND}, {EV_B0, EV_BWALK}, {EV_BBLEND, EV_BPRE},
                            {EV_PRE, EV_SL_BIN}, {EV_SL_BIN, EV_SL_BLEND}, {EV_BWALK, EV_BBLEND}};
  for (int i = 0; i < 11; ++i) {
    const int a = pairs[i][0], b = pairs[i][1];
    if (!c->ev_set[a] || !c->ev_set[b]) continue;
    if (hipEventSynchronize(c->ev[b]) != hipSuccess) return RTGS_E_HIP;
    float t = 0.f;
    if (hipEventElapsedTime(&t, c->ev[a], c->ev[b]) == hipSuccess) ms[i] = t;
  }
  return RTGS_OK;
}

int rtgs_raster_forward(const rtgs_raster_settings* s, int32_t P, int32_t M, const float* means3D,
                        const float* opacities, const float* shs, const float* scales, const float* rotations,
                        const float* normal_w, const int32_t* tile_mask, float* out_color, float* out_depth,
                        int32_t* out_cidx, int32_t* out_didx, float* out_cw, float* out_dw, float* out_T,
                        int32_t* out_radii, rtgs_resize_fn geom_resize, void* geom_user,
                        rtgs_resize_fn binning_resize, void* binning_user, rtgs_resize_fn image_resize,
                        void* image_user, int64_t* num_rendered_host, void* stream) {
  return rtgs_raster_forward_ctx(nullptr, s, P, M, means3D, opacities, shs, scales, rotations, normal_w, tile_mask,
                                 out_color, out_depth, out_cidx, out_didx, out_cw, out_dw, out_T, out_radii, geom_resize,
                                 geom_user, binning_resize, binning_user, image_resize, image_user, num_rendered_host, 0, stream);
}
// ... 34 lines not shown
```

rtg_slam_amd/csrc/raster_bwd_entry.hip:

```cpp
#include "raster_common.h"
#include <stdlib.h>

namespace rtgs {

constexpr int MB = 256;
constexpr int MACC = 13;

template <int CTRL>
__device__ __forceinline__ float dppf(float old, float v) {
  return __int_as_float(__builtin_amdgcn_update_dpp(__float_as_int(old), __float_as_int(v), CTRL, 0xf, 0xf, false));
}
template <int N>
__device__ __forceinline__ float bcast(float v) {
  return __int_as_float(__builtin_amdgcn_mov_dpp(__float_as_int(v), 0x150 + N, 0xf, 0xf, false));
}
template <int N>
__device__ __forceinline__ uint32_t bcast_u(uint32_t v) {
  return (uint32_t)__builtin_amdgcn_mov_dpp((int)v, 0x150 + N, 0xf, 0xf, false);
}
__device__ __forceinline__ float row_scan_mul(float v) {
  v *= dppf<0x111>(1.f, v);
  v *= dppf<0x112>(1.f, v);
  v *= dppf<0x114>(1.f, v);
  v *= dppf<0x118>(1.f, v);
// ... 145 lines not shown
    const auto e1 = __builtin_amdgcn_permlane32_swap(__float_as_uint(d1), __float_as_uint(d1), false, false);
    const auto e2 = __builtin_amdgcn_permlane32_swap(__float_as_uint(d2), __float_as_uint(d2), false, false);
    const auto e3 = __builtin_amdgcn_permlane32_swap(__float_as_uint(d3), __float_as_uint(d3), false, false);
    const bool take = same && k == 0;
    d0 += take ? __uint_as_float(e0[1]) : 0.f; d1 += take ? __uint_as_float(e1[1]) : 0.f;
    d2 += take ? __uint_as_float(e2[1]) : 0.f; d3 += take ? __uint_as_float(e3[1]) : 0.f;
    if (same && k == 2) key = NONE;
  }
#define RTGS_DEPTH_LEVEL(SH)                                                                                          \
  {                                                                                                                    \
    const uint32_t up = dppu<0x100 + SH>(NONE, key), down = dppu<0x110 + SH>(NONE, key);  \
    const float u0 = dppf<0x100 + SH>(0.f, d0), u1 = dppf<0x100 + SH>(0.f, d1), u2 = dppf<0x100 + SH>(0.f, d2),        \
                u3 = dppf<0x100 + SH>(0.f, d3);                                                                        \
    const bool lower = k == 0 && (n & (2 * SH - 1)) == 0, upper = k == 0 && (n & (2 * SH - 1)) == SH;                 \
    const bool take = lower && key != NONE && up == key;                                                               \
    d0 += take ? u0 : 0.f; d1 += take ? u1 : 0.f; d2 += take ? u2 : 0.f; d3 += take ? u3 : 0.f;                        \
    if (upper && key != NONE && down == key) key = NONE;                                                               \
  }
  RTGS_DEPTH_LEVEL(1) RTGS_DEPTH_LEVEL(2) RTGS_DEPTH_LEVEL(4) RTGS_DEPTH_LEVEL(8)
#undef RTGS_DEPTH_LEVEL
  if (key != NONE) {
    float* const acc = &s_acc[key * MACC + 9];
    atomicAdd(acc + 0, d0); atomicAdd(acc + 1, d1); atomicAdd(acc + 2, d2); atomicAdd(acc + 3, d3);
  }
}

__device__ __forceinline__ int compact_quadrant(uint2 mk, uint32_t qm, int m, int lane, uint8_t* __restrict__ sub) {
  uint32_t bits = 0;
#pragma unroll
  for (int j = 0; j < 4; ++j) {
    const uint32_t mask = ((j < 2 ? mk.x : mk.y) >> (16 * (j & 1))) & 0xffffu;
    bits |= (((mask & qm) != 0u) & (4 * lane + j < m)) ? (1u << j) : 0u;
  }
  const unsigned long long lt = (1ull << lane) - 1ull;
  uint32_t pre = 0, total = 0;
#pragma unroll
  for (int j = 0; j < 4; ++j) {
    const unsigned long long bal = __builtin_amdgcn_ballot_w64(((bits >> j) & 1u) != 0u);
    pre += (uint32_t)__popcll(bal & lt);
    total += (uint32_t)__popcll(bal);
  }
#pragma unroll
  for (int j = 0; j < 4; ++j)
    if ((bits >> j) & 1u) sub[pre + (uint32_t)__popc(bits & ((1u << j) - 1u))] = (uint8_t)(4 * lane + j);
  return (int)total;
}

struct TileLoads {
  uint32_t tmode, r0, r1, tlast;
  uint32_t fail;
  uint4 info;
  uint32_t last;
  float g0, g1, g2, oc0, oc1, oc2, gD;
  int owner;
  uint32_t dpos;
  float2 aux;
  float4 c0, c1, c2;
  uint2 mk;
};

template <bool STAMP>
__device__ __forceinline__ void blend_bwd_entry_body(
    const RasterParams& p, const uint2* __restrict__ ranges, const uint32_t* __restrict__ point_list,
    const Splat* __restrict__ splats, const float* __restrict__ out_color, const uint32_t* __restrict__ n_contrib,
    const int32_t* __restrict__ depth_index, const uint32_t* __restrict__ depth_pos, const uint32_t* __restrict__ tile_last,
    const float* __restrict__ dL_dcolor, const float* __restrict__ dL_ddepth,
    const uint32_t* __restrict__ gbase, uint32_t* __restrict__ slot_count, const BwdInfo* __restrict__ info,
    SplatGrad* __restrict__ grads, uint8_t* __restrict__ touched, const uint32_t* __restrict__ tile_mode,
    uint32_t t0, uint32_t tn, uint32_t dbg, unsigned long long* __restrict__ stamps, const TileCache& tc, uint32_t pre) {
  __shared__ float4 s_rec[MB * 3];
  __shared__ float s_acc[MB * MACC];
  __shared__ uint8_t s_sub[4][MB];

  const int tid = threadIdx.x;
  const uint32_t HW = (uint32_t)(p.H * p.W);

  auto issue = [&](int packed, TileLoads& L) {
    int tl = tid;
    asm volatile("" : "+v"(tl));
    const int ln = tl & 15, lk = (tl >> 4) & 3, lw = tl >> 6;
    const int lx = (lw & 1) * 8 + 2 * (ln & 3) + (lk & 1), ly = (lw >> 1) * 8 + 2 * (ln >> 2) + (lk >> 1);
    const int bx = packed & 0xffff, by = packed >> 16;
    const int tile = by * p.gx + bx;
    const int px = bx * TILE + lx, py = by * TILE + ly;
    const uint32_t pix = (px < p.W && py < p.H) ? (uint32_t)(py * p.W + px) : 0u;
    int tz = 0;
    asm volatile("" : "+v"(tz));
    tz += tile;
    L.tmode = tile_mode[tz];
    const uint2 rg = ranges[tz];
    L.r0 = rg.x; L.r1 = rg.y;
    L.tlast = tile_last[tz];
    L.fail = p.spec_fail ? p.spec_fail[tz - tile] : 0u;
    L.info = reinterpret_cast<const uint4*>(info)[tz - tile];
    L.last = n_contrib[pix];
    L.g0 = dL_dcolor[pix]; L.g1 = dL_dcolor[HW + pix]; L.g2 = dL_dcolor[2 * HW + pix];
    L.oc0 = out_color[pix]; L.oc1 = out_color[HW + pix]; L.oc2 = out_color[2 * HW + pix];
    L.owner = depth_index[pix];
    L.gD = dL_ddepth[pix];
    L.dpos = depth_pos[pix];
    {
      const float4* const rsrc = tc.recs + ((size_t)tile * TILE_RECS + (size_t)tl) * 3;
      if ((uint32_t)tl < pre) { L.c0 = rsrc[0]; L.c1 = rsrc[1]; L.c2 = rsrc[2]; }
      L.mk = reinterpret_cast<const uint2*>(tc.masks + (size_t)tile * TILE_RECS)[tl & 63];
      L.aux = tc.depth_aux[pix];
    }
  };

  const int cur = (int)((blockIdx.y << 16) | blockIdx.x);
  unsigned long long st_wall = 0, st_cyc = 0, st_walk = 0, st_groups = 0, st_steps = 0;
  unsigned long long st_seg[6] = {0, 0, 0, 0, 0, 0}, st_t = 0, st_p2 = 0, st_p1 = 0;
  if constexpr (STAMP) { st_wall = wall_clock64(); st_cyc = __builtin_readcyclecounter(); }
  TileLoads L;
  issue(cur, L);
  if constexpr (STAMP) st_p1 = __builtin_readcyclecounter() - st_cyc;
  for (int q = tid; q < MB * MACC; q += BLOCK) s_acc[q] = 0.f;
  __syncthreads();

  bool use_slots = false;
  SplatGrad* slot_grads = nullptr;
  auto entry_tail = [&](int m, float cxT, float cyT) {
    int tt = tid;
    asm volatile("" : "+v"(tt));
    float t[13];
    bool any = false;
    uint32_t gid = 0u;
    if (tt < m) {
#pragma unroll
      for (int q = 0; q < 13; ++q) { t[q] = s_acc[tt * MACC + q]; any |= (t[q] != 0.f); }
#pragma unroll
      for (int q = 0; q < 13; ++q) s_acc[tt * MACC + q] = 0.f;
      gid = __float_as_uint(s_rec[tt * 3 + 2].y);
    }
    const bool store = any && gid - t0 < tn && !(dbg & 4u);
    if (!store) return;
    uint32_t slot = 0u;
    if (use_slots) slot = gbase[gid] + atomicAdd(&slot_count[gid], 1u);
    const float4 q0 = s_rec[tt * 3 + 0], q1 = s_rec[tt * 3 + 1];
    const float ut = q0.x - cxT, vt = q0.y - cyT, o = q1.y;
    const float m0 = t[0], mx = t[1], my = t[2], mxx = t[3], mxy = t[4], myy = t[5];
    const float sx = o * (ut * m0 - mx), sy = o * (vt * m0 - my);
    const float sxx = o * (ut * (ut * m0 - 2.f * mx) + mxx);
    const float sxy = o * (ut * (vt * m0 - my) - vt * mx + mxy);
    const float syy = o * (vt * (vt * m0 - 2.f * my) + myy);
    const float du = -(q0.z * sx + q0.w * sy), dv = -(q1.x * sy + q0.w * sx);
    const float dca = -0.5f * sxx, dcb = -sxy, dcc = -0.5f * syy, dop = m0;
    touched[gid] = 1;
    if (use_slots) {
      typedef float vf4 __attribute__((ext_vector_type(4)));
      typedef __attribute__((address_space(1))) vf4 global_vf4;
      global_vf4* dst = (global_vf4*)(slot_grads + slot);
      dst[0] = vf4{du, dv, dca, dcb};
      dst[1] = vf4{dcc, dop, t[6], t[7]};
      dst[2] = vf4{t[8], t[9], t[10], t[11]};
      dst[3] = vf4{t[12], 0.f, 0.f, 0.f};
    } else {
      float* dst = reinterpret_cast<float*>(grads + gid);
      const float vals[13] = {du, dv, dca, dcb, dcc, dop, t[6], t[7], t[8], t[9], t[10], t[11], t[12]};
#pragma unroll
      for (int q = 0; q < 13; ++q)
        if (vals[q] != 0.f) unsafeAtomicAdd(dst + q, vals[q]);
    }
  };
  {
    int tq = tid;
    asm volatile("" : "+v"(tq));
    const int lane = tq & 63, wv = tq >> 6;
    const int n = lane & 15, k = lane >> 4;
    const int qx0 = (wv & 1) * 8, qy0 = (wv >> 1) * 8;
    const int lx = qx0 + 2 * (n & 3) + (k & 1), ly = qy0 + 2 * (n >> 2) + (k >> 1);
    const uint32_t qmask = 0x0033u << (2 * (wv & 1) + 8 * (wv >> 1));
    const int bx = cur & 0xffff, by = cur >> 16;
    const int tile = by * p.gx + bx;
    const int px = bx * TILE + lx, py = by * TILE + ly;
    const bool inside = px < p.W && py < p.H;
    const uint32_t pix = inside ? (uint32_t)(py * p.W + px) : 0u;
    const uint32_t tmode = (uint32_t)__builtin_amdgcn_readfirstlane((int)L.tmode);
    if constexpr (STAMP) { asm volatile("" ::"s"(tmode)); st_p1 |= (__builtin_readcyclecounter() - st_cyc) << 32; }
    const uint32_t range_x = (uint32_t)__builtin_amdgcn_readfirstlane((int)L.r0), range_y = (uint32_t)__builtin_amdgcn_readfirstlane((int)L.r1);
    const uint32_t tlast = (uint32_t)__builtin_amdgcn_readfirstlane((int)L.tlast);
    if (__builtin_amdgcn_readfirstlane((int)L.fail) != 0) return;
    use_slots = __builtin_amdgcn_readfirstlane((int)L.info.w) != 0;
    slot_grads = reinterpret_cast<SplatGrad*>(((unsigned long long)(uint32_t)__builtin_amdgcn_readfirstlane((int)L.info.y) << 32) |
                                                               (unsigned long long)(uint32_t)__builtin_amdgcn_readfirstlane((int)L.info.x));
    const int nuse = ((tmode & 3u) == 2u) ? min((int)(range_y - range_x), (int)tlast) : 0;
    const bool cached = (tmode & 4u) != 0u && !(dbg & 8u);
    if constexpr (STAMP) { asm volatile("s_waitcnt vmcnt(0) lgkmcnt(0)" ::: "memory"); const unsigned long long t = __builtin_readcyclecounter(); st_p2 = t - st_cyc; st_seg[0] = st_p2; st_t = t; }

    const float tx0 = (float)(bx * TILE), ty0 = (float)(by * TILE);
    const float cxT = tx0 + 7.5f, cyT = ty0 + 7.5f;

    EntryWalk W;
    W.n = n;
    W.last = inside ? L.last : 0u;
    W.G0 = inside ? L.g0 : 0.f; W.G1 = inside ? L.g1 : 0.f; W.G2 = inside ? L.g2 : 0.f;
    W.Tc = 1.f;
    W.Qc = L.oc0 * W.G0 + L.oc1 * W.G1 + L.oc2 * W.G2;
    const bool has_owner = inside && L.owner >= 0 && L.gD != 0.f && !(dbg & 2u);
    const uint32_t dpos = has_owner ? L.dpos : 0xffffffffu;
    const uint32_t wave_last = wave_max_u32(W.last);

    auto depth_batch = [&](int base, int m, float iden, float Dd, float gD, bool reload) {
      const bool pend = dpos >= (uint32_t)base && dpos < (uint32_t)(base + m);
      if (__builtin_amdgcn_ballot_w64(pend) == 0ull) return;
      float d0 = 0.f, d1 = 0.f, d2 = 0.f, d3 = 0.f;
      if (pend) {
        const float rx = ((float)px - p.cx) / p.fx, ry = ((float)py - p.cy) / p.fy;
        uint32_t pl = pix;
        asm volatile("" : "+v"(pl));
        if (reload) { gD = dL_ddepth[pl]; const float2 a2 = cached ? tc.depth_aux[pl] : make_float2(0.f, 0.f); iden = a2.x; Dd = a2.y; }
        if (!cached) {
          const int owner = depth_index[pl];
          const float4 r2 = reinterpret_cast<const float4*>(splats + owner)[2];
          const float pd = reinterpret_cast<const float*>(splats + owner)[12];
          iden = 1.f / (r2.y * rx + r2.z * ry + r2.w);
          Dd = pd * iden;
        }
        const float kk = -gD * Dd * iden;
        d0 = kk * rx; d1 = kk * ry; d2 = kk; d3 = gD * iden;
      }
      depth_adds(pend, dpos - (uint32_t)base, d0, d1, d2, d3, s_acc, lane);
    };
    auto stage_gather = [&](int base, int m) -> int {
      float txl = tx0, tyl = ty0;
      asm volatile("" : "+v"(txl), "+v"(tyl));
      int tl = tid, ll = lane;
      asm volatile("" : "+v"(tl), "+v"(ll));
      if (tid < m) {
        const uint32_t id = point_list[range_x + base + tl];
        const float4* src = reinterpret_cast<const float4*>(splats + id);
        const float4 q0 = src[0];
        s_rec[tid * 3 + 0] = q0;
        const float4 q1 = src[1];
        s_rec[tid * 3 + 1] = q1;
        const float b = reinterpret_cast<const float*>(splats + id)[8];
        const float2 hxy = reinterpret_cast<const float2*>(splats + id)[7];
        const uint32_t reach = quads_reached(q0.x, q0.y, hxy.x, hxy.y, q0.z, q0.w, q1.x, q1.y, txl, tyl);
        const uint32_t bm = ((reach & 1u) ? 0x0033u : 0u) | ((reach & 2u) ? 0x00ccu : 0u) | ((reach & 4u) ? 0x3300u : 0u) | ((reach & 8u) ? 0xcc00u : 0u);
        s_rec[tid * 3 + 2] = make_float4(b, __uint_as_float(id), __uint_as_float(bm), 0.f);
      }
      __syncthreads();
      const int e0 = 4 * ll;
      const uint32_t m0 = e0 + 0 < m ? __float_as_uint(s_rec[(e0 + 0) * 3 + 2].z) : 0u, m1 = e0 + 1 < m ? __float_as_uint(s_rec[(e0 + 1) * 3 + 2].z) : 0u;
      const uint32_t m2 = e0 + 2 < m ? __float_as_uint(s_rec[(e0 + 2) * 3 + 2].z) : 0u, m3 = e0 + 3 < m ? __float_as_uint(s_rec[(e0 + 3) * 3 + 2].z) : 0u;
      return compact_quadrant(make_uint2(m0 | (m1 << 16), m2 | (m3 << 16)), qmask, m, lane, s_sub[wv]);
    };

    int base = 0, m = min(MB, nuse), cnt = 0;
    if (nuse > 0) {
      if (cached) {
        if (tid < m) {
          if ((uint32_t)tid >= pre) {
            int tl = tid;
            asm volatile("" : "+v"(tl));
            const float4* const rsrc = tc.recs + ((size_t)tile * TILE_RECS + (size_t)tl) * 3;
            L.c0 = rsrc[0]; L.c1 = rsrc[1]; L.c2 = rsrc[2];
          }
          s_rec[tid * 3 + 0] = L.c0; s_rec[tid * 3 + 1] = L.c1; s_rec[tid * 3 + 2] = L.c2;
        }
        cnt = compact_quadrant(L.mk, qmask, m, lane, s_sub[wv]);
      } else {
        cnt = stage_gather(0, m);
      }
// ... 27 lines not shown
        const uint32_t stepmask = (uint32_t)((lb | (lb >> 16) | (lb >> 32) | (lb >> 48)) & 0xffffull);
        if (stepmask == 0u) continue;
        if constexpr (STAMP) { st_groups += 1; st_steps += (unsigned long long)__popc(stepmask); }
        const float4 r0 = s_rec[e * 3 + 0], r1 = s_rec[e * 3 + 1];
        const float rb = s_rec[e * 3 + 2].x;
        W.u = r0.x; W.v = r0.y; W.ca = r0.z; W.cb = r0.w; W.cc = r1.x; W.o = r1.y; W.cr = r1.z; W.cg_ = r1.w; W.cbl = rb;
        W.s0 = W.sx = W.sy = W.sxx = W.sxy = W.syy = W.sr = W.sg = W.sb = 0.f;
        W.run16_lane(stepmask);
        const float f0 = sum_rows(W.s0), f1 = sum_rows(W.sx), f2 = sum_rows(W.sy), f3 = sum_rows(W.sxx), f4 = sum_rows(W.sxy);
        const float f5 = sum_rows(W.syy), f6 = sum_rows(W.sr), f7 = sum_rows(W.sg), f8 = sum_rows(W.sb);
        if (have && k == 0) {
          float* const acc = &s_acc[e * MACC];
          atomicAdd(acc + 0, f0); atomicAdd(acc + 1, f1); atomicAdd(acc + 2, f2); atomicAdd(acc + 3, f3); atomicAdd(acc + 4, f4);
          atomicAdd(acc + 5, f5); atomicAdd(acc + 6, f6); atomicAdd(acc + 7, f7); atomicAdd(acc + 8, f8);
        }
      }
      if constexpr (STAMP) { st_t = __builtin_readcyclecounter(); st_walk += st_t - w_in; }
      __syncthreads();
      if constexpr (STAMP) { const unsigned long long t = __builtin_readcyclecounter(); st_seg[4] += t - st_t; st_t = t; }

      if (lastb) {
        entry_tail(m, cxT, cyT);
        if constexpr (STAMP) { asm volatile("s_waitcnt vmcnt(0) lgkmcnt(0)" ::: "memory"); const unsigned long long t2 = __builtin_readcyclecounter(); st_seg[5] += t2 - st_t; st_t = t2; }
        break;
      }
      entry_tail(m, cxT, cyT);
      __syncthreads();
      if constexpr (STAMP) { const unsigned long long t2 = __builtin_readcyclecounter(); st_seg[5] += t2 - st_t; st_t = t2; }
      base += MB;
      m = min(MB, nuse - base);
      cnt = stage_gather(base, m);
      depth_batch(base, m, 0.f, 0.f, 0.f, true);
      if constexpr (STAMP) { const unsigned long long t2 = __builtin_readcyclecounter(); st_seg[2] += t2 - st_t; st_t = t2; }
    }
    if constexpr (STAMP) {
      if (lane == 0) {
        unsigned long long* o = stamps + (size_t)(tile * 4 + wv) * 14;
        o[0] = st_wall; o[1] = wall_clock64(); o[2] = st_walk; o[3] = __builtin_readcyclecounter() - st_cyc; o[4] = st_groups; o[5] = st_steps;
#pragma unroll
        for (int q = 0; q < 6; ++q) o[6 + q] = st_seg[q];
        o[12] = st_p1; o[13] = st_p2;
      }
    }
  }
}

#define RTGS_BWD_ARGS                                                                                                             \
  RasterParams p, const uint2 *__restrict__ ranges, const uint32_t *__restrict__ point_list, const Splat *__restrict__ splats,       \
      const float *__restrict__ out_color, const uint32_t *__restrict__ n_contrib, const int32_t *__restrict__ depth_index,          \
      const uint32_t *__restrict__ depth_pos, const uint32_t *__restrict__ tile_last, const float *__restrict__ dL_dcolor,           \
      const float *__restrict__ dL_ddepth, const uint32_t *__restrict__ gbase, uint32_t *__restrict__ slot_count,                    \
      const BwdInfo *__restrict__ info, SplatGrad *__restrict__ grads, uint8_t *__restrict__ touched,                               \
      const uint32_t *__restrict__ tile_mode, uint32_t t0, uint32_t tn, uint32_t dbg, unsigned long long *__restrict__ stamps,       \
      TileCache tc, uint32_t pre
#define RTGS_BWD_PASS                                                                                                             \
  p, ranges, point_list, splats, out_color, n_contrib, depth_index, depth_pos, tile_last, dL_dcolor, dL_ddepth, gbase, slot_count, \
      info, grads, touched, tile_mode, t0, tn, dbg, stamps, tc, pre
__global__ void __launch_bounds__(256, 5) blend_bwd_entry_kernel(RTGS_BWD_ARGS) { blend_bwd_entry_body<false>(RTGS_BWD_PASS); }
__global__ void __launch_bounds__(256, 5) blend_bwd_entry_stamped_kernel(RTGS_BWD_ARGS) { blend_bwd_entry_body<true>(RTGS_BWD_PASS); }
#undef RTGS_BWD_ARGS
#undef RTGS_BWD_PASS

static int g_bwd_dbg = 0;
static unsigned long long* g_bwd_stamps = nullptr;
void set_bwd_debug(int bits) { g_bwd_dbg = bits & 15; }
void set_bwd_stamps(void* dev) { g_bwd_stamps = (unsigned long long*)dev; }

void launch_blend_bwd_entry(const RasterParams& p, const uint2* ranges, const uint32_t* point_list, const Splat* splats,
                            const float* out_color, const uint32_t* n_contrib, const int32_t* depth_index,
                            const uint32_t* depth_pos, const uint32_t* tile_last, const float* dL_dcolor, const float* dL_ddepth,
                            const uint32_t* gbase, uint32_t* slot_count, const BwdInfo* info, SplatGrad* grads, uint8_t* touched,
                            const uint32_t* tile_mode, uint32_t t0, uint32_t tn, TileCache tc, uint32_t pre, hipStream_t st) {
  const uint32_t dbg = (uint32_t)g_bwd_dbg;
#define RTGS_BWD_LAUNCH(KERNEL)                                                                                                      \
  hipLaunchKernelGGL(KERNEL, dim3(p.gx, p.gy), dim3(BLOCK), 0, st, p, ranges, point_list, splats, out_color, n_contrib, depth_index, \
                     depth_pos, tile_last, dL_dcolor, dL_ddepth, gbase, slot_count, info, grads, touched, tile_mode, t0, tn, dbg,    \
                     g_bwd_stamps, tc, pre)
  if (g_bwd_stamps) RTGS_BWD_LAUNCH(blend_bwd_entry_stamped_kernel); else RTGS_BWD_LAUNCH(blend_bwd_entry_kernel);
#undef RTGS_BWD_LAUNCH
}

}
```

rtg_slam_amd/csrc/raster_common.h:

```cpp
#pragma once
#include <hip/hip_runtime.h>
#include <stdint.h>
#include <stddef.h>

namespace rtgs {

constexpr int TILE = 16;
constexpr int BLOCK = TILE * TILE;
constexpr int WAVE = 64;
#ifndef RTGS_BWD_BATCH
#define RTGS_BWD_BATCH 128
#endif
constexpr int BATCH = RTGS_BWD_BATCH;

struct __attribute__((aligned(16))) Splat {
  float u, v;
  float ca, cb, cc;
  float o;
  float r, g, b;
  float nx, ny, nz;
  float pd;
  float z;
  float hx, hy;
};
// ... 39 lines not shown
  size_t splats, tiles_touched, offsets, radii, clamped, sat, tile_count, cursor, info, block_counts, scan_temp, total;
  size_t scan_temp_bytes;
  size_t zero_begin, zero_end;
  size_t tile_count1, ranges1_bwd, slice_hist, slice_cover, slice_ctr;
  size_t zbin, cursor1, ranges1, mask2, block_counts1, bucket1, list1, uv, slice_ids;
  size_t vis_ids, block_counts_vis;
  size_t slot_count;
  size_t slice_seg;
  size_t slice_cap, slice_max_list;
};

constexpr int SLICE_BINS = 256;
constexpr int SLICE_MAX_LIST = 3072;
constexpr float SLICE_MIN_COVER = 24.f;
constexpr float SLICE_MIN_RATIO = 2.f;
struct SliceSel {
  int mode;
  const uint8_t* zbin;
  const uint32_t* hist;
  uint32_t cap;
  uint32_t max_list;
  const uint32_t* ctr;
  const int32_t* sat;
  const float2* uv;
  const unsigned long long* cover;
  uint32_t npix;
  int decide;
};
__device__ __forceinline__ int sat_count(const int32_t* __restrict__ sat, int gx, int x0, int y0, int x1, int y1) {
  const int sw = gx + 1;
  return sat[y1 * sw + x1] - sat[y0 * sw + x1] - sat[y1 * sw + x0] + sat[y0 * sw + x0];
}
struct SlicePass {
  int mode;
  const int32_t* user_mask;
  int32_t* mask2;
  uint2* ranges_bwd;
  uint2* ranges_main;
};
struct SliceList {
  const uint32_t* ids;
  const uint32_t* count;
};
__device__ __forceinline__ uint32_t slice_bin_of(float z) {
  const int b = (int)(__float_as_uint(z) >> 18) - (int)(0x3E4CCCCDu >> 18);
  return (uint32_t)(b < 0 ? 0 : (b > SLICE_BINS - 2 ? SLICE_BINS - 2 : b));
}
struct BinLayout {
  size_t keys_a, keys_b, vals_a, vals_b, sort_temp, total;
  size_t sort_temp_bytes;
  size_t slot_grads;
};
struct ImgLayout {
  size_t ranges, n_contrib, bwd_info, tile_mode, depth_pos, tile_last, tile_recs, tile_masks, depth_aux, total;
};
constexpr int TILE_RECS = 256;
struct TileCache {
  float4* recs;
  uint16_t* masks;
  float2* depth_aux;
};
#ifndef RTGS_ROWS_MAX_SHARE
#define RTGS_ROWS_MAX_SHARE 0.6f
#endif
constexpr float ROWS_MAX_SHARE = RTGS_ROWS_MAX_SHARE;

struct BwdInfo {
  SplatGrad* slot_grads;
  uint32_t slots;
  uint32_t use_slots;
};
struct BwdInfoInit { BwdInfo* dst; SplatGrad* slot_grads; uint32_t slots, use_slots; };
constexpr uint32_t SLOTS_MAX = 12u << 20;

__device__ __forceinline__ void tile_rect_of(float u, float v, int radius, int gx, int gy, int& x0, int& y0, int& x1, int& y1) {
  const float r = (float)radius;
  x0 = min(gx, max(0, (int)((u - r) / (float)TILE)));
  y0 = min(gy, max(0, (int)((v - r) / (float)TILE)));
  x1 = min(gx, max(0, (int)((u + r + (float)(TILE - 1)) / (float)TILE)));
  y1 = min(gy, max(0, (int)((v + r + (float)(TILE - 1)) / (float)TILE)));
}

__device__ __forceinline__ uint32_t blocks_reached(float u, float v, float hx, float hy, float ca, float cb, float cc,
                                                   float o, float tx0, float ty0) {
  const float tau = 1.01f * fmaxf(2.f * __logf(255.f * fmaxf(o, 1e-12f)), 0.f) + 0.02f;
  const float kc = -cb / cc, ka = -cb / ca, twob = 2.f * cb;
  float ex[4], lox[4];
  uint32_t xm = 0, ym = 0;
#pragma unroll
  for (int i = 0; i < 4; ++i) {
    const float lo_x = tx0 + 4.f * (float)i, lo_y = ty0 + 4.f * (float)i;
    xm |= (!((u + hx < lo_x) | (u - hx > lo_x + 3.f))) ? (1u << i) : 0u;
    ym |= (!((v + hy < lo_y) | (v - hy > lo_y + 3.f))) ? (0x000fu << (4 * i)) : 0u;
    lox[i] = lo_x - u;
    ex[i] = __builtin_amdgcn_fmed3f(0.f, lox[i], lox[i] + 3.f);
  }
  uint32_t em = 0;
#pragma unroll 1
  for (int j = 0; j < 4; ++j) {
    const float loy = ty0 + 4.f * (float)j - v;
    const float ey = __builtin_amdgcn_fmed3f(0.f, loy, loy + 3.f);
    const float dxu = ka * ey, cey2 = cc * ey * ey, tbey = twob * ey;
#pragma unroll
    for (int i = 0; i < 4; ++i) {
      const float dy1 = __builtin_amdgcn_fmed3f(kc * ex[i], loy, loy + 3.f);
      const float q1 = fmaf(dy1, fmaf(cc, dy1, twob * ex[i]), ca * ex[i] * ex[i]);
      const float dx2 = __builtin_amdgcn_fmed3f(dxu, lox[i], lox[i] + 3.f);
      const float q2 = fmaf(dx2, fmaf(ca, dx2, tbey), cey2);
      em |= (fminf(q1, q2) <= tau) ? ((1u << i) << (4 * j)) : 0u;
    }
  }
  return (xm * 0x1111u) & ym & em;
}
// ... 111 lines not shown
```

rtg_slam_amd/csrc/raster_fwd.hip:

```cpp
#include "raster_common.h"
#include <stdlib.h>

namespace rtgs {

constexpr int SAT_LDS = 12288;
__global__ void __launch_bounds__(256) mask_sat_kernel(const int32_t* __restrict__ mask, int gx, int gy,
                                                       int32_t* __restrict__ sat) {
  __shared__ int32_t s_sat[SAT_LDS];
  const int sw = gx + 1, n = (gy + 1) * sw;
  int32_t* const w = n <= SAT_LDS ? s_sat : sat;
  for (int i = threadIdx.x; i < n; i += blockDim.x) {
    int y = i / sw, x = i % sw;
    w[i] = (y == 0 || x == 0) ? 0 : (mask[(y - 1) * gx + (x - 1)] != 0);
  }
  __syncthreads();
  for (int y = 1 + threadIdx.x; y <= gy; y += blockDim.x) {
    int acc = 0;
    for (int x = 1; x <= gx; ++x) { acc += w[y * sw + x]; w[y * sw + x] = acc; }
  }
  __syncthreads();
  for (int x = 1 + threadIdx.x; x <= gx; x += blockDim.x) {
    int acc = 0;
    for (int y = 1; y <= gy; ++y) { acc += w[y * sw + x]; w[y * sw + x] = acc; }
  }
// ... 182 lines not shown
  if constexpr (MODE == 0) {
    radii[i] = radius;
    if (out_radii) out_radii[i] = radius;
    tiles_touched[i] = (uint32_t)touched;
    if (zbin) zbin[i] = (uint8_t)slice_bin_of(pcz);
  }
}

__global__ void __launch_bounds__(256) emit_keys_kernel(
    RasterParams p, const Splat* __restrict__ splats, const int32_t* __restrict__ radii,
    const uint32_t* __restrict__ offsets, const int32_t* __restrict__ mask,
    uint64_t* __restrict__ keys, uint32_t* __restrict__ vals) {
  const int i = blockIdx.x * blockDim.x + threadIdx.x;
  if (i >= p.P) return;
  const int radius = radii[i];
  if (radius <= 0) return;
  uint32_t off = (i == 0) ? 0u : offsets[i - 1];
  const uint32_t end = offsets[i];
  if (off == end) return;
  const float u = splats[i].u, v = splats[i].v;
  const uint32_t zbits = __float_as_uint(splats[i].z);
  int x0, y0, x1, y1;
  tile_rect_of(u, v, radius, p.gx, p.gy, x0, y0, x1, y1);
  for (int y = y0; y < y1; ++y)
    for (int x = x0; x < x1; ++x) {
      const int t = y * p.gx + x;
      if (mask[t] != 0) {
        keys[off] = ((uint64_t)(uint32_t)t << 32) | zbits;
        vals[off] = (uint32_t)i;
        ++off;
      }
    }
}

__global__ void __launch_bounds__(256) tile_ranges_kernel(int64_t R, const uint64_t* __restrict__ keys,
                                                          uint2* __restrict__ ranges) {
  const int64_t i = (int64_t)blockIdx.x * blockDim.x + threadIdx.x;
  if (i >= R) return;
  const uint32_t t = (uint32_t)(keys[i] >> 32);
  if (i == 0) ranges[t].x = 0;
  else {
    const uint32_t tp = (uint32_t)(keys[i - 1] >> 32);
    if (tp != t) { ranges[tp].y = (uint32_t)i; ranges[t].x = (uint32_t)i; }
  }
  if (i == R - 1) ranges[t].y = (uint32_t)R;
}

constexpr int FWD_BATCH = BLOCK;
constexpr int FWD_CHUNKS = FWD_BATCH / 32;

typedef float f4v __attribute__((ext_vector_type(4)));
typedef float f2v __attribute__((ext_vector_type(2)));

template <int OCC, bool STAMP, bool COUNT, bool ASMW>
__global__ void __launch_bounds__(256, OCC) blend_fwd_kernel(
    RasterParams p, const uint2* __restrict__ ranges, const uint32_t* __restrict__ point_list,
    const Splat* __restrict__ splats, float* __restrict__ out_color, float* __restrict__ out_depth,
    int32_t* __restrict__ out_cidx, int32_t* __restrict__ out_didx, float* __restrict__ out_cw,
    float* __restrict__ out_dw, float* __restrict__ out_T, uint32_t* __restrict__ n_contrib,
    unsigned long long* __restrict__ counters, SlicePass sp, uint32_t* __restrict__ tile_mode,
    uint32_t* __restrict__ depth_pos, uint32_t* __restrict__ tile_last, int walk, uint32_t* __restrict__ aux_zero,
    TileCache tc, unsigned long long* __restrict__ stamps, uint32_t seg) {
  __shared__ float4 s_rec[FWD_BATCH * 4];
#define RI(e, j) ((e) * 4 + (j))
  __shared__ float s_z[FWD_BATCH];
  __shared__ uint32_t s_live[16][FWD_CHUNKS];

  unsigned long long st_wall = 0, st_cyc = 0, st_range = 0, st_first = 0, st_walk = 0, st_steps = 0, st_batches = 0;
  if constexpr (STAMP) { st_wall = wall_clock64(); st_cyc = __builtin_readcyclecounter(); }
  const int tid = threadIdx.x;
  const int lane = tid & 63, wv = tid >> 6;
  const int tile = blockIdx.y * p.gx + blockIdx.x;
  int z = 0;
  asm volatile("" : "+v"(z));
  const uint2 range_v = ranges[tile + z];
  const uint32_t fail_v = p.spec_fail ? p.spec_fail[z] : 0u;
  const int32_t m2_v = sp.mode == 2 ? sp.mask2[tile + z] : 1;
  const int32_t on_v = sp.mode == 1 ? sp.user_mask[tile + z] : 1;
  uint32_t id_first = 0u;
  if (seg != 0u) id_first = point_list[(size_t)tile * seg + (size_t)tid];
  if (aux_zero && blockIdx.x == 0 && blockIdx.y == 0 && tid < 8) aux_zero[tid] = 0u;
  const int bx = ((wv & 1) << 1) | ((lane >> 4) & 1), by = (wv & 2) | (lane >> 5);
  const int blk = by * 4 + bx;
  const int px = blockIdx.x * TILE + bx * 4 + (lane & 3);
  const int py = blockIdx.y * TILE + by * 4 + ((lane >> 2) & 3);
  const bool inside = px < p.W && py < p.H;
  const float pxf = (float)px, pyf = (float)py;
  const float tx0 = (float)(blockIdx.x * TILE), ty0 = (float)(blockIdx.y * TILE);
  if (__builtin_amdgcn_readfirstlane((int)fail_v) != 0) return;
  if (__builtin_amdgcn_readfirstlane(m2_v) == 0) return;
  const uint2 range = make_uint2((uint32_t)__builtin_amdgcn_readfirstlane((int)range_v.x), (uint32_t)__builtin_amdgcn_readfirstlane((int)range_v.y));
  int n = (int)(range.y - range.x);
  if (sp.mode == 1 && n > SLICE_MAX_LIST) n = 0;
  if constexpr (STAMP) { st_range = __builtin_readcyclecounter() - st_cyc; }

  bool done = !inside;
  unsigned long long Dm = __builtin_amdgcn_ballot_w64(!inside);
  unsigned long long evals_w = 0;
  float T = 1.f, C0 = 0.f, C1 = 0.f, C2 = 0.f;
  float best_w = 0.f; int best_id = -1;
  float D = 0.f, d_w = 0.f; int d_id = -1;
  float d_iden = 0.f;
  uint32_t d_pos = 0u;
  uint32_t last_contributor = 0;
  uint32_t evals = 0;
  uint32_t reach_sum = 0, staged = 0;

  int bs = sp.mode == 1 ? FWD_BATCH / 4 : FWD_BATCH;
  for (int base = 0; base < n; base += bs, bs = FWD_BATCH) {
    if (base > 0 && __syncthreads_and(ASMW ? (Dm == ~0ull) : done)) break;
    const int m = min(bs, n - base);
    {
      uint32_t reach = 0;
      if (tid < m) {
        const uint32_t id = (seg != 0u && base == 0) ? id_first : point_list[range.x + base + tid];
// ... 150 lines not shown
      }
#undef RTGS_FWD_WALK
      if constexpr (STAMP) st_steps += steps_w;
      if constexpr (COUNT) evals_w += evals_lo;
    } else
    for (;;) {
      while (cur == 0u && c + 1 < nch) { ++c; cur = s_live[blk][c]; }
      const bool has = cur != 0u && !done;
      if (__builtin_amdgcn_ballot_w64(has) == 0ull) break;
      const int e = has ? (c << 5) + __builtin_ctz(cur) : 0;
      cur &= cur - 1u;
      if constexpr (STAMP) st_steps += 1;
      const float4 r0 = s_rec[RI(e, 0)];
      const float4 r1 = s_rec[RI(e, 1)];
      const float4 r2 = s_rec[RI(e, 2)];
      const float dx = r0.x - pxf, dy = r0.y - pyf;
      const float power = splat_power(r0.z, r0.w, r1.x, dx, dy);
      const float al = fminf(0.99f, r1.y * splat_exp(fminf(power, 0.f)));
      const bool ok = has && !(power > 0.f) && !(al < 1.f / 255.f);
      const float test_T = T * (1.f - al);
      const bool stop = ok && (test_T < p.T_thr);
      const bool contrib = ok && !stop;
      if constexpr (COUNT) evals += has ? 1u : 0u;
      done = done || stop;
      const float w = contrib ? al * T : 0.f;
      T = contrib ? test_T : T;
      last_contributor = contrib ? (uint32_t)(base + e + 1) : last_contributor;
      if (__builtin_amdgcn_ballot_w64(contrib) == 0ull) continue;
      C0 += r1.z * w; C1 += r1.w * w; C2 += r2.x * w;
      const bool better = w > best_w;
      const int gid = (int)__float_as_uint(r2.w);
      best_w = better ? w : best_w;
      best_id = better ? gid : best_id;
      const bool want_depth = contrib && d_id < 0 && al > p.opaque_thr;
      if (__builtin_amdgcn_ballot_w64(want_depth) != 0ull) {
        if (want_depth) {
          const float rx = (pxf - p.cx) / p.fx, ry = (pyf - p.cy) / p.fy;
          const float rnorm = sqrtf(rx * rx + ry * ry + 1.f);
          const float4 r3 = s_rec[RI(e, 3)];
          const float den = r3.x * rx + r3.y * ry + r3.z;
          if (fabsf(den) / rnorm > p.normal_thr) {
            const float zhit = r3.w / den;
            if (zhit > 0.f && fabsf(zhit - s_z[e]) < p.depth_thr) {
              D = zhit; d_w = al; d_id = gid; d_pos = (uint32_t)(base + e); d_iden = 1.f / den;
            }
          }
        }
      }
    }
    if constexpr (STAMP) st_walk += __builtin_readcyclecounter() - w_in;
  }

  __shared__ uint32_t s_ep[4][4];
  {
    const uint32_t wl = wave_max_u32(last_contributor);
    const bool wave_done = ASMW ? (Dm == ~0ull) : (__builtin_amdgcn_ballot_w64(done) == ~0ull);
    if (lane == 0) { s_ep[wv][0] = reach_sum; s_ep[wv][1] = staged; s_ep[wv][2] = wl; s_ep[wv][3] = wave_done ? 1u : 0u; }
  }
  __syncthreads();
  const uint32_t reach_all = s_ep[0][0] + s_ep[1][0] + s_ep[2][0] + s_ep[3][0], staged_all = s_ep[0][1] + s_ep[1][1] + s_ep[2][1] + s_ep[3][1];
  const uint32_t tl_all = max(max(s_ep[0][2], s_ep[1][2]), max(s_ep[2][2], s_ep[3][2]));
  bool write_out = true;
  if (sp.mode == 1) {
    const bool finished = (s_ep[0][3] & s_ep[1][3] & s_ep[2][3] & s_ep[3][3]) != 0u;
    const bool on = __builtin_amdgcn_readfirstlane(on_v) != 0;
    if (tid == 0) {
      sp.mask2[tile] = (on && !finished) ? 1 : 0;
      sp.ranges_bwd[tile] = finished ? range : make_uint2(0u, 0u);
      sp.ranges_main[tile] = make_uint2(0u, 0u);
    }
    write_out = finished || !on;
  }

  if (inside && write_out) {
    const size_t pix = (size_t)py * p.W + px;
    const size_t HW = (size_t)p.H * p.W;
    out_color[pix] = C0 + T * p.bg[0];
    out_color[HW + pix] = C1 + T * p.bg[1];
    out_color[2 * HW + pix] = C2 + T * p.bg[2];
    out_depth[pix] = D;
    out_cidx[pix] = best_id;
    out_didx[pix] = d_id;
    out_cw[pix] = best_w;
    out_dw[pix] = d_w;
    out_T[pix] = T;
    n_contrib[pix] = last_contributor;
    depth_pos[pix] = d_pos;
    if (tc.depth_aux != nullptr) tc.depth_aux[pix] = make_float2(d_iden, D);
  }
  if (tid == 0 && write_out) {
    const float share = staged_all ? (float)reach_all / (16.f * (float)staged_all) : 1.f;
    tile_mode[tile] = (walk >= 0 ? (uint32_t)walk : (share < ROWS_MAX_SHARE ? 1u : 0u)) | (tc.recs != nullptr ? 4u : 0u) |
                      ((uint32_t)(share * 1000.f) << 8);
    tile_last[tile] = tl_all;
  }
  if (COUNT && counters) {
    __shared__ unsigned int s_max;
    __shared__ unsigned long long s_ev;
    if (tid == 0) { s_max = 0; s_ev = 0; }
    __syncthreads();
    atomicMax(&s_max, last_contributor);
    if constexpr (ASMW) { if (lane == 0) atomicAdd(&s_ev, evals_w); }
    else atomicAdd(&s_ev, (unsigned long long)evals);
    __syncthreads();
    if (tid == 0) {
      const bool add = sp.mode == 2;
      counters[2 * tile] = (add ? counters[2 * tile] : 0ull) + (unsigned long long)s_max;
      counters[2 * tile + 1] = (add ? counters[2 * tile + 1] : 0ull) + s_ev;
    }
  }
  if constexpr (STAMP) {
    if (lane == 0 && stamps != nullptr) {
      unsigned long long* o = stamps + (size_t)(tile * 4 + wv) * 8;
      o[0] = st_wall; o[1] = wall_clock64(); o[2] = st_range; o[3] = st_first; o[4] = st_walk;
      o[5] = __builtin_readcyclecounter() - st_cyc; o[6] = st_steps; o[7] = st_batches;
    }
  }
}
#undef RI


static int g_f1_occ = [] { const char* e = getenv("RTGS_F1_OCC"); const int v = e ? atoi(e) : 6; return v == 5 ? 5 : 6; }();
static int g_f1_asm = [] { const char* e = getenv("RTGS_F1_ASM"); return e ? atoi(e) : 1; }();
static unsigned long long* g_fwd_stamps = nullptr;
void set_fwd_stamps(void* dev) { g_fwd_stamps = (unsigned long long*)dev; }

void launch_mask_sat(const int32_t* mask, int gx, int gy, int32_t* sat, hipStream_t st) {
  hipLaunchKernelGGL(mask_sat_kernel, dim3(1), dim3(256), 0, st, mask, gx, gy, sat);
}
void launch_preprocess_fwd(const RasterParams& p, const float* means, const float* opac, const float* shs,
                           const float* scales, const float* rots, const float* normal_w, const int32_t* sat,
                           Splat* splats, uint32_t* tiles_touched, int32_t* radii, uint8_t* clamped,
                           int32_t* out_radii, uint32_t* zero_words, int zero_n, uint8_t* zbin, hipStream_t st) {
  if (p.P == 0) return;
  hipLaunchKernelGGL(preprocess_fwd_kernel<0>, dim3((p.P + 255) / 256), dim3(256), 0, st, p, means, opac, shs, scales,
                     rots, normal_w, sat, splats, tiles_touched, radii, clamped, out_radii, zero_words, zero_n, zbin,
                     (float2*)nullptr, SliceList{nullptr, nullptr}, SliceSel{0, nullptr, nullptr, 0u, 0u, nullptr, nullptr, nullptr});
}
void launch_preprocess_cull(const RasterParams& p, const float* means, const float* scales, const float* rots,
                            uint32_t* tiles_touched, int32_t* radii, int32_t* out_radii, uint32_t* zero_words, int zero_n,
                            uint8_t* zbin, float2* uv, hipStream_t st) {
  if (p.P == 0) return;
  hipLaunchKernelGGL(preprocess_fwd_kernel<1>, dim3((p.P + 255) / 256), dim3(256), 0, st, p, means, (const float*)nullptr,
                     (const float*)nullptr, scales, rots, (const float*)nullptr, (const int32_t*)nullptr, (Splat*)nullptr,
                     tiles_touched, radii, (uint8_t*)nullptr, out_radii, zero_words, zero_n, zbin, uv,
                     SliceList{nullptr, nullptr}, SliceSel{0, nullptr, nullptr, 0u, 0u, nullptr, nullptr, nullptr});
}
void launch_preprocess_shade(const RasterParams& p, const float* means, const float* opac, const float* shs,
                             const float* scales, const float* rots, const float* normal_w, Splat* splats,
                             int32_t* radii, uint8_t* clamped, float2* uv, SliceList list, SliceSel sel, size_t max_items,
                             hipStream_t st) {
  if (p.P == 0) return;
  const size_t n = list.ids ? (max_items < (size_t)p.P ? max_items : (size_t)p.P) : (size_t)p.P;
  hipLaunchKernelGGL(preprocess_fwd_kernel<2>, dim3((unsigned)((n + 255) / 256)), dim3(256), 0, st, p, means, opac, shs,
                     scales, rots, normal_w, (const int32_t*)nullptr, splats, (uint32_t*)nullptr, radii, clamped,
                     (int32_t*)nullptr, (uint32_t*)nullptr, 0, (uint8_t*)nullptr, uv, list, sel);
}
void launch_emit_keys(const RasterParams& p, const Splat* splats, const int32_t* radii, const uint32_t* offsets,
                      const int32_t* mask, uint64_t* keys, uint32_t* vals, hipStream_t st) {
  if (p.P == 0) return;
  hipLaunchKernelGGL(emit_keys_kernel, dim3((p.P + 255) / 256), dim3(256), 0, st, p, splats, radii, offsets, mask,
                     keys, vals);
}
void launch_tile_ranges(int64_t R, const uint64_t* keys, uint2* ranges, hipStream_t st) {
  if (R == 0) return;
  hipLaunchKernelGGL(tile_ranges_kernel, dim3((unsigned)((R + 255) / 256)), dim3(256), 0, st, R, keys, ranges);
}
__global__ void __launch_bounds__(256) slice_publish_kernel(int ntiles, const int32_t* __restrict__ user_mask,
                                                            const int32_t* __restrict__ mask2,
                                                            const uint32_t* __restrict__ r1, uint32_t* __restrict__ ctr,
                                                            uint32_t* __restrict__ host, uint32_t seq,
                                                            uint32_t* __restrict__ spec_fail,
                                                            const uint32_t* __restrict__ seg_count) {
  int left = 0, fin = 0, inst = 0;
  for (int t = threadIdx.x; t < ntiles; t += 256) {
    const bool on = user_mask[t] != 0, l = mask2[t] != 0;
    left += l ? 1 : 0;
    fin += (on && !l) ? 1 : 0;
    if (seg_count) inst += (int)seg_count[t];
  }
  __shared__ int s_l[4], s_f[4], s_i[4];
#pragma unroll
  for (int off = 32; off > 0; off >>= 1) { left += __shfl_xor(left, off); fin += __shfl_xor(fin, off); inst += __shfl_xor(inst, off); }
  if ((threadIdx.x & 63) == 0) { s_l[threadIdx.x >> 6] = left; s_f[threadIdx.x >> 6] = fin; s_i[threadIdx.x >> 6] = inst; }
  __syncthreads();
  if (threadIdx.x == 0) {
    const uint32_t L = (uint32_t)(s_l[0] + s_l[1] + s_l[2] + s_l[3]), F = (uint32_t)(s_f[0] + s_f[1] + s_f[2] + s_f[3]);
    ctr[0] = L; ctr[1] = F;
    if (spec_fail) *spec_fail = L != 0u ? 1u : 0u;
    const uint32_t R1 = seg_count ? (uint32_t)(s_i[0] + s_i[1] + s_i[2] + s_i[3]) : r1[0];
    const uint32_t w[7] = {ctr[2], 0u, L, F, R1, 0u, 0u};
    publish_to_host(host, w, seq);
  }
}
void launch_slice_publish(int ntiles, const int32_t* user_mask, const int32_t* mask2, const uint32_t* r1, uint32_t* ctr,
                          uint32_t* host, uint32_t seq, uint32_t* spec_fail, hipStream_t st, const uint32_t* seg_count) {
  hipLaunchKernelGGL(slice_publish_kernel, dim3(1), dim3(256), 0, st, ntiles, user_mask, mask2, r1, ctr, host, seq, spec_fail,
                     seg_count);
}

void launch_blend_fwd(const RasterParams& p, const uint2* ranges, const uint32_t* point_list, const Splat* splats,
                      float* out_color, float* out_depth, int32_t* out_cidx, int32_t* out_didx, float* out_cw,
                      float* out_dw, float* out_T, uint32_t* n_contrib, unsigned long long* counters,
                      SlicePass sp, uint32_t* tile_mode, uint32_t* depth_pos, uint32_t* tile_last, int walk, uint32_t* aux_zero,
                      TileCache tc, uint32_t seg, hipStream_t st) {
#define RTGS_FWD1(OCC, STAMP, COUNT, ASMW) hipLaunchKernelGGL((blend_fwd_kernel<OCC, STAMP, COUNT, ASMW>), dim3(p.gx, p.gy), dim3(BLOCK), 0, st, p, ranges, point_list, splats, \
                       out_color, out_depth, out_cidx, out_didx, out_cw, out_dw, out_T, n_contrib, counters, sp, tile_mode, \
                       depth_pos, tile_last, walk, aux_zero, tc, g_fwd_stamps, seg)
  if (g_f1_asm == 0) RTGS_FWD1(6, false, true, false);
  else if (counters) RTGS_FWD1(6, false, true, true);
  else if (g_fwd_stamps) RTGS_FWD1(6, true, false, true);
  else if (g_f1_occ == 5) RTGS_FWD1(5, false, false, true); else RTGS_FWD1(6, false, false, true);
#undef RTGS_FWD1
}

}
```

rtg_slam_amd/map_optim.py:

```python
from __future__ import annotations

import ctypes as C
import math
from typing import Callable, Dict, Optional

import torch
import torch.distributed as dist

COLS = 59
BLOCKS = (("xyz", 0, 3), ("shs", 3, 51), ("raw8", 51, 59))


def default_lr_columns(position_lr=1e-3, feature_lr=5e-4, opacity_lr=0.0, scaling_lr=4e-3, rotation_lr=1e-3):
    lr = torch.zeros(COLS)
    lr[0:3] = position_lr
    lr[3:6] = feature_lr
    lr[6:51] = feature_lr / 20.0
    lr[51:52] = opacity_lr
    lr[52:55] = scaling_lr
    lr[55:59] = rotation_lr
    return lr


def global_lr_scale(final: bool = False, feature_lr_coef: float = 1.0, scaling_lr_coef: float = 1.0,
# ... 133 lines not shown
                self.tensor = torch.empty(max(int(nbytes * 1.25), 256), dtype=torch.uint8, device=self.device)
            return self.tensor.data_ptr()
        except Exception:
            return 0


class ShardedMapOptimizer:

    def __init__(self, packed: torch.Tensor, lr_col: Optional[torch.Tensor] = None, eps: float = 1e-15,
                 group=None, adam_fn: Optional[Callable] = None, activate_fn: Optional[Callable] = None,
                 n_frozen: int = 0, capacity: Optional[int] = None):
        self.group = group
        self.row_skip = adam_fn is None and packed.is_cuda
        self.adam_fn = adam_fn if adam_fn is not None else _adam_hip
        self.activate_fn = activate_fn if activate_fn is not None else activate8_hip
        self.world = dist.get_world_size(group) if dist.is_initialized() else 1
        self.rank = dist.get_rank(group) if dist.is_initialized() else 0
        self.backend = dist.get_backend(group) if dist.is_initialized() else "none"
        self.N = int(packed.shape[0])
        self.n_frozen = int(n_frozen)
        if not 0 <= self.n_frozen <= self.N:
            raise ValueError("n_frozen must be in [0, N]")
        self.device = packed.device
        self.lr_full = (default_lr_columns() if lr_col is None else lr_col).to(self.device).float()
        self.eps = eps
        self._use_arena = self.row_skip and activate_fn is None
        self.state = {}
        self.grad_rows = None
        self.act = None
        self._slam_ws = None
        self._slam_state = None
        self.capacity = 0
        self.aux = {}
        self._aux_spec = {}
        self._scope = "local"
        self._lr_scope = None
        self.version = 0
        self._gd_views = {}
        self._adam_dirty = None
        self._frozen_version = 0
        self._allocate(max(int(capacity) if capacity is not None else self.N, self.N, 1), packed)
        self.step_count = 0
        self.total_steps = getattr(self, "total_steps", 0)
        self.last_render = None
        self.last_num_rendered = 0
        self.attach_init = None
        self._history = None
        self._row_capacity = 16384
        self._pending = None
        self.overflow_redos = 0
        self._cap_peak, self._cap_steps, self._shrink_every = 0, 0, 32
        self._act_valid = False
        self.tail_mode = 1 if __import__("os").environ.get("RTGS_TAIL_MODE", "0") == "1" else 0
        self.live_counts = torch.zeros(2, dtype=torch.int32, device=self.device) if packed.is_cuda else None
        self._mode = None

    @property
    def n_train(self) -> int:
        return self.N - self.n_frozen

    def _active(self):
        return (self.n_frozen, 0) if self._scope == "global" else (self.N, self.n_frozen)

    @property
    def frozen_key(self):
        return (self.state["xyz"]["p"].data_ptr(), int(self.n_frozen), int(self._frozen_version))

    @property
    def n_active_train(self) -> int:
        n, t0 = self._active()
        return n - t0

    @property
    def per(self) -> int:
        return shard_rows(self.n_active_train, self.world)[0]

    @property
    def Npad(self) -> int:
        return self._active()[1] + shard_rows(self.n_active_train, self.world)[1]

    def _lr(self, name):
        return self._lr_scope[name] if self._lr_scope is not None else self.state[name]["lr"]

    def _allocate(self, cap: int, packed: Optional[torch.Tensor] = None):
        dev, N = self.device, self.N
        rows = cap + self.world
        old = self.state
        self._gd_views = {}
        self._frozen_version = getattr(self, "_frozen_version", 0) + 1
        f = dict(dtype=torch.float32, device=dev)
        per_cap = (cap + self.world - 1) // self.world + 1
        adam_rows = cap if self.world == 1 else per_cap
        self.state = {}
        for name, c0, c1 in BLOCKS:
            full = torch.zeros(rows, c1 - c0, **f)
            if packed is not None:
                full[:N] = packed[:, c0:c1]
            elif old:
                full[:N] = old[name]["p"][:N]
            self.state[name] = dict(
                p=full, lr=self.lr_full[c0:c1].contiguous(),
                m=torch.zeros(adam_rows, c1 - c0, **f), v=torch.zeros(adam_rows, c1 - c0, **f),
                ever=torch.zeros(adam_rows, dtype=torch.uint8, device=dev),
                gpad=(torch.zeros(rows, c1 - c0, **f) if self.world > 1 else None),
                gshard=(torch.zeros(per_cap, c1 - c0, **f) if self.world > 1 else None))
            if old and self.world == 1:
# ... 385 lines not shown
                    n: dict(m=torch.zeros(cap, c1 - c0, dtype=torch.float32, device=dev),
                            v=torch.zeros(cap, c1 - c0, dtype=torch.float32, device=dev),
                            ever=torch.zeros(cap, dtype=torch.uint8, device=dev)) for n, c0, c1 in BLOCKS}
        ad = self._slam_state if self.world > 1 else st
        H, W = int(rs.image_height), int(rs.image_width)
        ws = self._slam_ws
        if ws is None or ws["hw"] != (H, W):
            f = dict(dtype=torch.float32, device=dev)
            i = dict(dtype=torch.int32, device=dev)
            ws = self._slam_ws = dict(
                hw=(H, W), color=torch.empty(3, H, W, **f), depth=torch.empty(1, H, W, **f),
                cidx=torch.empty(1, H, W, **i), didx=torch.empty(1, H, W, **i), cw=torch.empty(1, H, W, **f),
                dw=torch.empty(1, H, W, **f), T=torch.empty(1, H, W, **f), radii=torch.empty(st["xyz"]["p"].shape[0], **i),
                g_color=torch.empty(3, H, W, **f), g_depth=torch.empty(1, H, W, **f), loss=torch.empty(4, **f),
                loss_scratch=None,
                ones=torch.ones((H + 15) // 16, (W + 15) // 16, **i),
                arenas=[_GrowArena(dev), _GrowArena(dev), _GrowArena(dev)])
        act = self.act
        if tile_mask is None:
            tile_mask = ws["ones"]
        tile_mask = tile_mask.to(device=dev, dtype=torch.int32).contiguous()
        gt_color, gt_depth = gt_color.contiguous(), gt_depth.contiguous()
        if normal_weight > 0 and gt_normal is not None:
            gt_normal = gt_normal.to(device=dev, dtype=torch.float32).contiguous()
        else:
            gt_normal = None
        rm = None if render_mask is None else (render_mask if render_mask.dtype == torch.uint8 else (render_mask != 0).to(torch.uint8)).contiguous()
        need = lib.rtgs_slam_loss_scratch_bytes(H, W, int(rm is None))
        if ws["loss_scratch"] is None or ws["loss_scratch"].numel() < need:
            ws["loss_scratch"] = torch.empty(need, dtype=torch.uint8, device=dev)
        attach = None
        if getattr(self, "attach_init", None) is not None:
            ai = self.attach_init
            attach = _lib.AttachC(ai["xyz"].data_ptr(), ai["raw8"].data_ptr(), ai["info"].data_ptr())
        keep = _Keep(rs, dev)
        self.step_count += 1
        self.total_steps = getattr(self, "total_steps", 0) + 1
        P = lambda t: t.data_ptr()
        geom, binning, img = ws["arenas"]
        args = _lib.MapStepArgsC(
            C.pointer(keep.c), N, 16, P(st["xyz"]["p"]), P(st["shs"]["p"]), P(st["raw8"]["p"]), P(tile_mask), P(gt_color),
            P(gt_depth), _lib.LossCfgC(float(color_weight), float(depth_weight), float(ssim_weight), float(add_depth_thres),
                                       rm.data_ptr() if rm is not None else None),
            P(ws["loss_scratch"]), P(act["opacity"]), P(act["scales"]), P(act["rotations"]),
            P(act["normal"]), P(ws["color"]), P(ws["depth"]), P(ws["cidx"]), P(ws["didx"]), P(ws["cw"]), P(ws["dw"]),
            P(ws["T"]), P(ws["radii"]), P(ws["g_color"]), P(ws["g_depth"]), P(ws["loss"]), P(a.d_means), P(a.d_opac),
            P(a.d_shs), P(a.d_scales), P(a.d_rots), P(a.d_normal), P(a.d_raw8), P(a.scratch), P(a.row_state),
            P(ad["xyz"]["m"]), P(ad["xyz"]["v"]), P(ad["shs"]["m"]), P(ad["shs"]["v"]), P(ad["raw8"]["m"]),
            P(ad["raw8"]["v"]), P(self._lr("xyz")), P(self._lr("shs")), P(self._lr("raw8")), P(ad["xyz"]["ever"]),
            P(ad["shs"]["ever"]), P(ad["raw8"]["ever"]), int(self.step_count), 0.9, 0.999, float(self.eps),
            C.pointer(attach) if attach is not None else None, P(confidence) if confidence is not None else None,
            int(self._act_valid), geom.cb, None, binning.cb, None, img.cb, None,
            float(normal_weight) if gt_normal is not None else 0.0, P(gt_normal) if gt_normal is not None else None,
            int(nf), int(N), int(self.tail_mode), P(self.live_counts) if self.live_counts is not None else None)
        R = C.c_int64(0)
        stream = torch.cuda.current_stream(dev).cuda_stream
        if tile_band and self.world > 1:
            if rm is None:
                raise RuntimeError("step_slam(tile_band=True) needs a render_mask (the SSIM window of the unmasked loss "
                                   "crosses band boundaries; the reference always passes one, mapper.py:196-203)")
            self._front_tileband(lib, args, ws, keep, tile_mask, rm, R, dev)
            self._exchange_and_tail(dict(step=int(self.step_count), attach=attach, confidence=confidence, keep=(keep, attach)))
        elif self.world == 1:
            self._mark_adam(0, N - nf)
            with torch.cuda.device(dev):
                rc = lib.rtgs_slam_map_step_ctx(current_context().ptr, C.byref(args), C.byref(R), C.c_void_p(stream))
            _lib.check(rc, "rtgs_slam_map_step")
        else:
            with torch.cuda.device(dev):
                rc = lib.rtgs_slam_map_step_front_ctx(current_context().ptr, C.byref(args), C.byref(R), C.c_void_p(stream))
            _lib.check(rc, "rtgs_slam_map_step_front")
            self._exchange_and_tail(dict(step=int(self.step_count), attach=attach, confidence=confidence, keep=(keep, attach)))
        a.calls = 1
        self._act_valid = True
        self.last_render = (ws["color"], ws["depth"], ws["cidx"], ws["didx"], ws["cw"], ws["dw"], ws["T"])
        self.last_num_rendered = int(R.value)
        self.last_losses = ws["loss"]
        return ws["loss"][0]

    def band_tile_mask(self, tile_mask: torch.Tensor, with_region: bool = False):
        on = (tile_mask.reshape(-1) != 0)
        cum = torch.cumsum(on.to(torch.int64), 0) - on.to(torch.int64)
        owner = ((cum * self.world) // on.sum().clamp_min(1)).clamp_max(self.world - 1)
        mine = owner == self.rank
        band = (on & mine).to(torch.int32).reshape(tile_mask.shape).contiguous()
        return (band, mine.reshape(tile_mask.shape)) if with_region else band

    def _front_tileband(self, lib, args, ws, keep, tile_mask, rm, R, dev):
        from . import _lib
        from .rasterizer import current_context
        N, t0 = self._active()
        H, W = ws["hw"]
        objs = ws.get("band_objs")
        same = (objs is not None and objs[0] is tile_mask and objs[1] is rm and objs[2] == (tile_mask._version, rm._version))
        if not same:
            band, region = self.band_tile_mask(tile_mask, with_region=True)
            pix = region.repeat_interleave(16, 0).repeat_interleave(16, 1)[:H, :W].to(torch.uint8)
            ws["band"], ws["band_rm"] = band, (pix * (rm != 0).to(torch.uint8)).contiguous()
            ws["band_objs"] = (tile_mask, rm, (tile_mask._version, rm._version))
        band, band_rm = ws["band"], ws["band_rm"]
        V = lambda t: C.c_void_p(t.data_ptr())
        st = lambda: C.c_void_p(torch.cuda.current_stream(dev).cuda_stream)
        geom, binning, img = ws["arenas"]
        x = self.state
        a = self.grad_rows
        cfg = _lib.LossCfgC(args.loss.color_weight, args.loss.depth_weight, args.loss.ssim_weight, args.loss.add_depth_thres,
                            band_rm.data_ptr())
# ... 272 lines not shown
```

Baseline: 2584 units/s.

## Fold masked L1 loss into blend forward and backward kernels

Adds a loss-fold path in which the forward blend kernel computes per-tile partial sums of the masked colour and gated depth L1 loss. A single-workgroup reduce, run standalone or merged into the slice-publish kernel, turns these into the loss scalars. The backward entry kernel can then compute dL/dcolor and dL/ddepth inline instead of reading them from separate loss kernel output. This removes the standalone loss kernel launches and the image-sized gradient buffer round trips, at the cost of more template variants, extra registers in the blend kernels and more complex state in the context.

Result: slower. 2507 units/s (-3.0%).

```diff
diff --git a/include/rtgs_raster.h b/include/rtgs_raster.h
--- a/include/rtgs_raster.h
+++ b/include/rtgs_raster.h
@@ -244,6 +244,7 @@
   int32_t train_begin, train_end;
   int32_t tail_mode;
   uint32_t* live_counts;
+  int32_t loss_mode;
 } rtgs_map_step_args;
 int rtgs_slam_normal_loss(const float* normal_w, const int32_t* depth_index, const float* gt_normal,
                           const uint8_t* render_mask, int32_t H, int32_t W, float normal_weight, float* scratch2,
@@ -271,6 +272,15 @@
 int rtgs_raster_backward_buffers(int32_t P, int32_t image_height, int32_t image_width, size_t* out8_host);
 int rtgs_raster_last_buffers_ctx(rtgs_ctx* ctx, void** out3_host);
 void rtgs_raster_set_aux_zero_ctx(rtgs_ctx* ctx, void* eight_words);
+typedef struct rtgs_loss_fold {
+  const float *gt_color, *gt_depth;
+  const uint8_t* render_mask;
+  float add_depth_thres, color_weight, depth_weight;
+  float* sums;
+  float* loss4;
+  int32_t backward;
+} rtgs_loss_fold;
+int rtgs_raster_set_loss_fold_ctx(rtgs_ctx* ctx, const rtgs_loss_fold* fold);
 int rtgs_slam_map_step_front(const rtgs_map_step_args* args, int64_t* num_rendered_host, void* stream);
 int rtgs_slam_map_step_ctx(rtgs_ctx* ctx, const rtgs_map_step_args* args, int64_t* num_rendered_host, void* stream);
 int rtgs_slam_map_step_front_ctx(rtgs_ctx* ctx, const rtgs_map_step_args* args, int64_t* num_rendered_host, void* stream);
diff --git a/rtg_slam_amd/_lib.py b/rtg_slam_amd/_lib.py
--- a/rtg_slam_amd/_lib.py
+++ b/rtg_slam_amd/_lib.py
@@ -68,7 +68,7 @@
         + [("geom_resize", RESIZE_FN), ("geom_user", C.c_void_p), ("binning_resize", RESIZE_FN),
            ("binning_user", C.c_void_p), ("image_resize", RESIZE_FN), ("image_user", C.c_void_p)]
         + [("normal_weight", C.c_float), ("gt_normal", C.c_void_p), ("train_begin", C.c_int32), ("train_end", C.c_int32),
-           ("tail_mode", C.c_int32), ("live_counts", C.c_void_p)])
+           ("tail_mode", C.c_int32), ("live_counts", C.c_void_p), ("loss_mode", C.c_int32)])
 
 
 _SIGNATURES = {
@@ -103,6 +103,7 @@
     "rtgs_raster_backward_buffers": (C.c_int, [C.c_int32, C.c_int32, C.c_int32, C.POINTER(C.c_size_t)]),
     "rtgs_raster_last_buffers_ctx": (C.c_int, [_P, C.POINTER(C.c_void_p)]),
     "rtgs_raster_set_aux_zero_ctx": (None, [_P, _P]),
+    "rtgs_raster_set_loss_fold_ctx": (C.c_int, [_P, _P]),
     "rtgs_raster_backward_walk_ctx": (C.c_int, [_P, C.POINTER(RasterSettingsC), C.c_int32, C.c_int32, C.c_int64] + [_P] * 6
                                       + [_P] * 3 + [_P, _P, _P] + [_P, _P] + [_P] * 6 + [_P, _P, C.c_int32, C.c_int32, _P]),
     "rtgs_slam_loss_scratch_bytes": (C.c_size_t, [C.c_int32, C.c_int32, C.c_int32]),
diff --git a/rtg_slam_amd/csrc/map_step.hip b/rtg_slam_amd/csrc/map_step.hip
--- a/rtg_slam_amd/csrc/map_step.hip
+++ b/rtg_slam_amd/csrc/map_step.hip
@@ -1,9 +1,13 @@
 #include <hip/hip_runtime.h>
+
+#include <stdlib.h>
 
 #include "../../include/rtgs_raster.h"
 
+static const int g_loss_mode_env = [] { const char* e = getenv("RTGS_LOSS_MODE"); const int v = e ? atoi(e) : 0; return v == 1 || v == 2 ? v : 0; }();
+
 static int map_step_front(rtgs_ctx* ctx, const rtgs_map_step_args* a, int64_t* num_rendered_host, int32_t fwd_flags,
-                          void* stream, bool walk_only = false) {
+                          void* stream, bool walk_only = false, bool may_fold = false) {
   if (!a || !num_rendered_host || !a->settings) return RTGS_E_INVALID;
   const int32_t P = a->P, M = a->sh_coeffs;
   if (P <= 0 || M != 16 || a->step < 1) return RTGS_E_INVALID;
@@ -15,7 +19,14 @@
     if (rc != 0) return RTGS_E_HIP;
   }
   if (!a->loss_scratch || !a->loss4) return RTGS_E_INVALID;
-  rtgs_raster_set_aux_zero_ctx(ctx, a->loss_scratch);
+  const int loss_mode = a->loss_mode != 0 ? a->loss_mode : g_loss_mode_env;
+  int fold = 0;
+  if (may_fold && loss_mode != 1 && (a->loss.render_mask != nullptr || a->loss.ssim_weight == 0.f)) {
+    const rtgs_loss_fold lf{a->gt_color, a->gt_depth, a->loss.render_mask, a->loss.add_depth_thres, a->loss.color_weight,
+                            a->loss.depth_weight, reinterpret_cast<float*>(a->loss_scratch), a->loss4, loss_mode == 2 ? 0 : 1};
+    fold = rtgs_raster_set_loss_fold_ctx(ctx, &lf);
+  }
+  if (!fold) rtgs_raster_set_aux_zero_ctx(ctx, a->loss_scratch);
   rc = rtgs_raster_forward_ctx(ctx, a->settings, P, M, a->xyz, a->opacity, a->shs, a->scales, a->rotations, a->normal,
                            a->tile_mask, a->out_color, a->out_depth, a->out_color_index, a->out_depth_index,
                            a->out_color_weight, a->out_depth_weight, a->out_T, a->out_radii, a->geom_resize,
@@ -27,13 +38,17 @@
   void *geom = bufs[0], *bin = bufs[1], *img = bufs[2];
   rtgs_loss_cfg lcfg = a->loss;
   lcfg.sums_zeroed = P > 0 ? 1 : 0;
-  rc = rtgs_slam_loss(a->out_color, a->out_depth, a->out_depth_index, a->gt_color, a->gt_depth, H, W, &lcfg,
-                      a->loss_scratch, a->loss4, a->dL_dcolor, a->dL_ddepth, stream);
+  if (!fold)
+    rc = rtgs_slam_loss(a->out_color, a->out_depth, a->out_depth_index, a->gt_color, a->gt_depth, H, W, &lcfg,
+                        a->loss_scratch, a->loss4, a->dL_dcolor, a->dL_ddepth, stream);
+  else if (!(fold & 2))
+    rc = rtgs_slam_loss_grads(a->out_color, a->out_depth, a->out_depth_index, a->gt_color, a->gt_depth, H, W, &lcfg,
+                              a->loss_scratch, a->loss4, a->dL_dcolor, a->dL_ddepth, stream);
   if (rc != 0) return RTGS_E_HIP;
   int32_t t0 = 0, t1 = P;
   if (a->train_begin != 0 || a->train_end != 0) { t0 = a->train_begin; t1 = a->train_end; }
   if (t0 < 0 || t1 > P || t1 < t0) return RTGS_E_INVALID;
-  if (t1 == t0) return RTGS_OK;
+  if (t1 == t0) { rtgs_raster_set_loss_fold_ctx(ctx, nullptr); return RTGS_OK; }
   rc = (walk_only ? rtgs_raster_backward_walk_ctx : rtgs_raster_backward_range_ctx)(
       ctx, a->settings, P, M, *num_rendered_host, a->xyz, a->opacity, a->shs, a->scales, a->rotations, a->normal, geom, bin, img,
       a->out_color, a->out_T, a->out_depth_index, a->dL_dcolor, a->dL_ddepth, a->d_xyz, a->d_opacity, a->d_shs, a->d_scales,
@@ -59,7 +74,7 @@
 
 static int map_step_once(rtgs_ctx* ctx, const rtgs_map_step_args* a, int64_t* num_rendered_host, bool speculate, void* stream) {
   const bool fused = a->tail_mode == 0 && !(a->normal_weight > 0.f && a->gt_normal);
-  int rc = map_step_front(ctx, a, num_rendered_host, speculate ? RTGS_FWD_SPECULATE : 0, stream, fused);
+  int rc = map_step_front(ctx, a, num_rendered_host, speculate ? RTGS_FWD_SPECULATE : 0, stream, fused, true);
   if (rc != RTGS_OK) return rc;
   if ((a->train_begin != 0 || a->train_end != 0) && a->train_end == a->train_begin) return RTGS_OK;
   if (fused) {
diff --git a/rtg_slam_amd/csrc/raster_api.hip b/rtg_slam_amd/csrc/raster_api.hip
--- a/rtg_slam_amd/csrc/raster_api.hip
+++ b/rtg_slam_amd/csrc/raster_api.hip
@@ -19,16 +19,20 @@
 void launch_tile_ranges(int64_t, const uint64_t*, uint2*, hipStream_t);
 void set_fwd_stamps(void* dev);
 void set_bwd_debug(int bits);
+bool bwd_entry_ignores_cache();
 void set_bwd_stamps(void* dev);
 void launch_blend_fwd(const RasterParams&, const uint2*, const uint32_t*, const Splat*, float*, float*, int32_t*,
                       int32_t*, float*, float*, float*, uint32_t*, unsigned long long*, SlicePass, uint32_t*, uint32_t*, uint32_t*, int, uint32_t*,
-                      TileCache, uint32_t, hipStream_t);
+                      TileCache, uint32_t, hipStream_t, const LossFold* fold = nullptr);
+void launch_loss_reduce(const LossReduce&, hipStream_t);
+bool blend_fwd_folds_loss(bool counters);
 void launch_blend_bwd(const RasterParams&, const uint2*, const uint32_t*, const Splat*, const float*, const float*,
                       const uint32_t*, const int32_t*, const float*, const float*, const uint32_t*, uint32_t*,
                       const BwdInfo*, SplatGrad*, uint8_t*, const uint32_t*, int, uint32_t, uint32_t, hipStream_t);
 void launch_blend_bwd_entry(const RasterParams&, const uint2*, const uint32_t*, const Splat*, const float*, const uint32_t*,
                             const int32_t*, const uint32_t*, const uint32_t*, const float*, const float*, const uint32_t*, uint32_t*,
-                            const BwdInfo*, SplatGrad*, uint8_t*, const uint32_t*, uint32_t, uint32_t, TileCache, uint32_t, hipStream_t);
+                            const BwdInfo*, SplatGrad*, uint8_t*, const uint32_t*, uint32_t, uint32_t, TileCache, uint32_t, hipStream_t,
+                            const LossGrad* lg = nullptr);
 void launch_grad_reduce(int, const uint8_t*, const uint32_t*, uint32_t*, const BwdInfo*, SplatGrad*, const uint32_t*, hipStream_t);
 void launch_preprocess_bwd(const RasterParams&, const float*, const float*, const float*, const float*, const float*,
                            const float*, const int32_t*, const uint8_t*, SplatGrad*, uint8_t*, uint8_t*, float*, float*,
@@ -45,7 +49,7 @@
                             const SliceSel* = nullptr, int32_t* = nullptr, uint32_t* = nullptr);
 void launch_slice_compact(int, SliceSel, uint32_t*, uint32_t*, const uint32_t*, uint32_t*, uint32_t*, uint32_t*, uint32_t, uint32_t*, hipStream_t);
 void launch_slice_publish(int, const int32_t*, const int32_t*, const uint32_t*, uint32_t*, uint32_t*, uint32_t, uint32_t*, hipStream_t,
-                          const uint32_t* seg_count = nullptr);
+                          const uint32_t* seg_count = nullptr, const LossReduce* lr = nullptr);
 void launch_preprocess_cull(const RasterParams&, const float*, const float*, const float*, uint32_t*, int32_t*, int32_t*,
                             uint32_t*, int, uint8_t*, float2*, hipStream_t);
 void launch_preprocess_shade(const RasterParams&, const float*, const float*, const float*, const float*, const float*,
@@ -87,6 +91,9 @@
   int hint_walk = -2;
   void *last_geom = nullptr, *last_bin = nullptr, *last_img = nullptr;
   uint32_t* aux_zero = nullptr;
+  bool fold_fwd = false, fold_want_bwd = false;
+  rtgs_loss_fold fold{};
+  const void* fold_bwd_geom = nullptr;
   bool ask_first = false;
   struct Plan {
     bool valid = false;
@@ -278,6 +285,7 @@
   L.tile_recs = off; off = align_up(off + (size_t)ntiles * TILE_RECS * 3 * sizeof(float4));
   L.tile_masks = off; off = align_up(off + (size_t)ntiles * TILE_RECS * sizeof(uint16_t));
   L.depth_aux = off; off = align_up(off + (size_t)H * W * sizeof(float2));
+  L.loss_part = off; off = align_up(off + (size_t)ntiles * sizeof(float4));
   L.total = off;
   return L;
 }
@@ -376,6 +384,9 @@
   rtgs_ctx* c = use(ctx);
   uint32_t* const aux_zero = c->aux_zero;
   c->aux_zero = nullptr;
+  const bool folding = c->fold_fwd;
+  c->fold_fwd = false;
+  c->fold_bwd_geom = nullptr;
   RasterParams p;
   int rc = make_params(s, P, M, p);
   if (rc != RTGS_OK) return rc;
@@ -404,6 +415,11 @@
   uint32_t* const tile_mode = (uint32_t*)(img + I.tile_mode);
   const int fwd_walk = c->bwd_walk == 0 || c->bwd_walk == 3 ? 2 : (c->bwd_walk == 4 ? -1 : c->bwd_walk - 1);
   c->last_geom = geom; c->last_img = img; c->last_bin = nullptr;
+  const LossFold lfold{c->fold.gt_color, c->fold.gt_depth, c->fold.render_mask, c->fold.add_depth_thres, (float4*)(img + I.loss_part)};
+  const LossFold* const fold = folding ? &lfold : nullptr;
+  const LossReduce lred{folding ? (const float4*)(img + I.loss_part) : nullptr, ntiles, c->fold.sums, c->fold.loss4,
+                        c->fold.color_weight, c->fold.depth_weight};
+  if (folding && c->fold_want_bwd && !(flags & RTGS_FWD_NO_BACKWARD)) c->fold_bwd_geom = geom;
   const TileCache tcache = (flags & RTGS_FWD_NO_BACKWARD) ? TileCache{nullptr, nullptr, nullptr}
                                                           : TileCache{(float4*)(img + I.tile_recs), (uint16_t*)(img + I.tile_masks), (float2*)(img + I.depth_aux)};
 
@@ -512,9 +528,10 @@
         prof_mark(c, EV_SL_BIN, st);
         const SlicePass pass1{1, tile_mask, mask2, ranges1_bwd, ranges};
         launch_blend_fwd(p, ranges1, list1, splats, out_color, out_depth, out_cidx, out_didx, out_cw, out_dw, out_T,
-                         n_contrib, c->counters, pass1, tile_mode, depth_pos, tile_last, fwd_walk, aux_zero, tcache, seg1, st);
+                         n_contrib, c->counters, pass1, tile_mode, depth_pos, tile_last, fwd_walk, aux_zero, tcache, seg1, st, fold);
         prof_mark(c, EV_SL_BLEND, st);
-        launch_slice_publish(ntiles, tile_mask, mask2, info + 2, slice_ctr, info_host, c->seq, fail, st, seg1 ? tile_count1 : nullptr);
+        launch_slice_publish(ntiles, tile_mask, mask2, info + 2, slice_ctr, info_host, c->seq, fail, st, seg1 ? tile_count1 : nullptr,
+                             &lred);
         prof_mark(c, EV_BLEND0, st); prof_mark(c, EV_BLEND, st);
         c->hint_slice_lists = true; c->hint_main_lists = false;
         c->slice_stats[0] = 1; c->slice_stats[1] = pl.R1; c->slice_stats[2] = pl.n_fin; c->slice_stats[3] = 0;
@@ -579,8 +596,9 @@
         prof_mark(c, EV_SORT, st);
         prof_mark(c, EV_BLEND0, st);
         launch_blend_fwd(pg, ranges, (uint32_t*)(bin + B.vals_b), splats, out_color, out_depth, out_cidx, out_didx, out_cw,
-                         out_dw, out_T, n_contrib, c->counters, SlicePass{0, nullptr, nullptr, nullptr, nullptr}, tile_mode, depth_pos, tile_last, fwd_walk, aux_zero, tcache, seg2, st);
+                         out_dw, out_T, n_contrib, c->counters, SlicePass{0, nullptr, nullptr, nullptr, nullptr}, tile_mode, depth_pos, tile_last, fwd_walk, aux_zero, tcache, seg2, st, fold);
         prof_mark(c, EV_BLEND, st);
+        launch_loss_reduce(lred, st);
         c->hint_slice_lists = false; c->hint_main_lists = true;
         c->slice_stats[0] = pl.kind == 2 ? 1 : 0; c->slice_stats[1] = 0; c->slice_stats[2] = 0;
         c->slice_stats[3] = pl.kind == 2 ? (int64_t)ntiles : 0;
@@ -677,7 +695,7 @@
       if (++c->seq == 0u) c->seq = 1u;
       const SlicePass pass1{1, tile_mask, mask2, ranges1_bwd, ranges};
       launch_blend_fwd(p, ranges1, list1, splats, out_color, out_depth, out_cidx, out_didx, out_cw, out_dw, out_T,
-                       n_contrib, c->counters, pass1, tile_mode, depth_pos, tile_last, fwd_walk, aux_zero, tcache, seg1, st);
+                       n_contrib, c->counters, pass1, tile_mode, depth_pos, tile_last, fwd_walk, aux_zero, tcache, seg1, st, fold);
       prof_mark(c, EV_SL_BLEND, st);
       launch_slice_publish(ntiles, tile_mask, mask2, info + 2, slice_ctr, info_host, c->seq, nullptr, st, seg1 ? tile_count1 : nullptr);
       DBG(s, st);
@@ -783,8 +801,9 @@
   prof_mark(c, EV_BLEND0, st);
   if (!sliced || n_left > 0)
     launch_blend_fwd(p, ranges, vals_b, splats, out_color, out_depth, out_cidx, out_didx, out_cw, out_dw, out_T,
-                     n_contrib, c->counters, pass, tile_mode, depth_pos, tile_last, fwd_walk, aux_zero, tcache, 0u, st);
+                     n_contrib, c->counters, pass, tile_mode, depth_pos, tile_last, fwd_walk, aux_zero, tcache, 0u, st, fold);
   prof_mark(c, EV_BLEND, st);
+  launch_loss_reduce(lred, st);
   DBG(s, st);
   HIP_TRY(hipGetLastError());
   c->stats[0] = R + R1; c->stats[1] = sort_bits; c->stats[2] = ntiles; c->stats[3] = (int64_t)G.total;
@@ -832,8 +851,9 @@
   if (P == 0) return RTGS_OK;
   if (c->spec.geom == geom_buffer && c->spec.fail_dev) p.spec_fail = c->spec.fail_dev;
   if (!means3D || !opacities || !shs || !scales || !rotations || !normal_w || !geom_buffer || !binning_buffer ||
-      !image_buffer || !out_color || !out_T || !out_didx || !dL_dcolor || !dL_ddepth || !grad_scratch || R < 0)
+      !image_buffer || !out_color || !out_T || !out_didx || !grad_scratch || R < 0)
     return RTGS_E_INVALID;
+  if ((!dL_dcolor || !dL_ddepth) && !(c->fold_bwd_geom == geom_buffer && c->hint_geom == geom_buffer && c->hint_walk == 2)) return RTGS_E_INVALID;
   if (!walk_only && (!dL_dmeans3D || !dL_dopacities || !dL_dshs || !dL_dscales || !dL_drotations || !dL_dnormal_w)) return RTGS_E_INVALID;
   hipStream_t st = (hipStream_t)stream;
   const int ntiles = p.gx * p.gy;
@@ -859,6 +879,12 @@
     if (train_begin < 0 || train_end > P || train_end < train_begin) return RTGS_E_INVALID;
     const uint32_t t0 = (uint32_t)train_begin, tn = (uint32_t)(train_end - train_begin);
     const uint32_t* depth_pos = (const uint32_t*)(img + I.depth_pos);
+    const bool fold_asked = c->fold_bwd_geom == geom_buffer;
+    const bool fold_bwd = hinted && fold_asked && which == 4;
+    c->fold_bwd_geom = nullptr;
+    if (fold_asked && !fold_bwd) return RTGS_E_INVALID;
+    const LossGrad lgrad{c->fold.gt_color, c->fold.gt_depth, c->fold.render_mask, c->fold.sums, c->fold.add_depth_thres,
+                         c->fold.color_weight, c->fold.depth_weight};
     for (int set = 0; set < 2; ++set) {
       if (hinted && !(set == 0 ? c->hint_slice_lists : c->hint_main_lists)) continue;
       const uint2* rg = set == 0 ? (const uint2*)(geom + G.ranges1_bwd) : (const uint2*)(img + I.ranges);
@@ -872,7 +898,7 @@
                                touched, tile_mode, t0, tn,
                                TileCache{(float4*)(img + I.tile_recs), (uint16_t*)(img + I.tile_masks), (float2*)(img + I.depth_aux)},
                                set == 0 ? (uint32_t)(BLOCK / 4) : (uint32_t)BLOCK,
-                               st);
+                               st, fold_bwd ? &lgrad : nullptr);
     }
     prof_mark(c, EV_BWALK, st);
     if (!walk_only) launch_grad_reduce(P, touched, gbase, slot_count, binfo, grads, p.spec_fail, st);
@@ -1012,6 +1038,17 @@
 void rtgs_raster_set_onepass_ctx(rtgs_ctx* c, int on) { use(c)->onepass = on != 0; use(c)->plan.valid = false; }
 void rtgs_raster_set_bwd_walk_ctx(rtgs_ctx* c, int mode) { use(c)->bwd_walk = (mode >= 1 && mode <= 4) ? mode : 0; }
 void rtgs_raster_set_aux_zero_ctx(rtgs_ctx* ctx, void* eight_words) { use(ctx)->aux_zero = (uint32_t*)eight_words; }
+int rtgs_raster_set_loss_fold_ctx(rtgs_ctx* ctx, const rtgs_loss_fold* f) {
+  rtgs_ctx* c = use(ctx);
+  c->fold_fwd = false; c->fold_want_bwd = false; c->fold_bwd_geom = nullptr;
+  if (!f) return 0;
+  if (!f->gt_color || !f->gt_depth || !f->sums || !f->loss4) return 0;
+  if (!rtgs::blend_fwd_folds_loss(c->counters != nullptr)) return 0;
+  c->fold = *f;
+  c->fold_fwd = true;
+  c->fold_want_bwd = f->backward != 0 && (c->bwd_walk == 0 || c->bwd_walk == 3) && !rtgs::bwd_entry_ignores_cache();
+  return c->fold_want_bwd ? 3 : 1;
+}
 int rtgs_raster_last_buffers_ctx(rtgs_ctx* ctx, void** out3) {
   rtgs_ctx* c = use(ctx);
   if (!out3 || !c->last_geom || !c->last_bin || !c->last_img) return RTGS_E_INVALID;
diff --git a/rtg_slam_amd/csrc/raster_bwd_entry.hip b/rtg_slam_amd/csrc/raster_bwd_entry.hip
--- a/rtg_slam_amd/csrc/raster_bwd_entry.hip
+++ b/rtg_slam_amd/csrc/raster_bwd_entry.hip
@@ -221,6 +221,8 @@
   uint4 info;
   uint32_t last;
   float g0, g1, g2, oc0, oc1, oc2, gD;
+  uint32_t msk;
+  float2 cnt;
   int owner;
   uint32_t dpos;
   float2 aux;
@@ -228,7 +230,7 @@
   uint2 mk;
 };
 
-template <bool STAMP>
+template <bool STAMP, bool LOSS>
 __device__ __forceinline__ void blend_bwd_entry_body(
     const RasterParams& p, const uint2* __restrict__ ranges, const uint32_t* __restrict__ point_list,
     const Splat* __restrict__ splats, const float* __restrict__ out_color, const uint32_t* __restrict__ n_contrib,
@@ -236,7 +238,8 @@
     const float* __restrict__ dL_dcolor, const float* __restrict__ dL_ddepth,
     const uint32_t* __restrict__ gbase, uint32_t* __restrict__ slot_count, const BwdInfo* __restrict__ info,
     SplatGrad* __restrict__ grads, uint8_t* __restrict__ touched, const uint32_t* __restrict__ tile_mode,
-    uint32_t t0, uint32_t tn, uint32_t dbg, unsigned long long* __restrict__ stamps, const TileCache& tc, uint32_t pre) {
+    uint32_t t0, uint32_t tn, uint32_t dbg, unsigned long long* __restrict__ stamps, const TileCache& tc, uint32_t pre,
+    const LossGrad& lg) {
   __shared__ float4 s_rec[MB * 3];
   __shared__ float s_acc[MB * MACC];
   __shared__ uint8_t s_sub[4][MB];
@@ -263,10 +266,16 @@
     L.fail = p.spec_fail ? p.spec_fail[tz - tile] : 0u;
     L.info = reinterpret_cast<const uint4*>(info)[tz - tile];
     L.last = n_contrib[pix];
-    L.g0 = dL_dcolor[pix]; L.g1 = dL_dcolor[HW + pix]; L.g2 = dL_dcolor[2 * HW + pix];
+    if constexpr (LOSS) {
+      L.g0 = lg.gt_color[pix]; L.g1 = lg.gt_color[HW + pix]; L.g2 = lg.gt_color[2 * HW + pix];
+      L.msk = lg.rmask ? (uint32_t)lg.rmask[pix] : 1u;
+      L.cnt = reinterpret_cast<const float2*>(lg.sums + 2)[tz - tile];
+    } else {
+      L.g0 = dL_dcolor[pix]; L.g1 = dL_dcolor[HW + pix]; L.g2 = dL_dcolor[2 * HW + pix];
+    }
     L.oc0 = out_color[pix]; L.oc1 = out_color[HW + pix]; L.oc2 = out_color[2 * HW + pix];
     L.owner = depth_index[pix];
-    L.gD = dL_ddepth[pix];
+    if constexpr (LOSS) L.gD = lg.gt_depth[pix]; else L.gD = dL_ddepth[pix];
     L.dpos = depth_pos[pix];
     {
       const float4* const rsrc = tc.recs + ((size_t)tile * TILE_RECS + (size_t)tl) * 3;
@@ -359,6 +368,22 @@
     const float tx0 = (float)(bx * TILE), ty0 = (float)(by * TILE);
     const float cxT = tx0 + 7.5f, cyT = ty0 + 7.5f;
 
+    float kd = 0.f;
+    if constexpr (LOSS) {
+      const float n_depth = __builtin_bit_cast(float, __builtin_amdgcn_readfirstlane(__builtin_bit_cast(int, L.cnt.x)));
+      const float n_mask = __builtin_bit_cast(float, __builtin_amdgcn_readfirstlane(__builtin_bit_cast(int, L.cnt.y)));
+      const float inv_c = 1.f / (3.f * fmaxf(n_mask, 1.f));
+      const float inv_m = 1.f / fmaxf(n_depth, 1.f);
+      const float kc = lg.cw * inv_c;
+      kd = lg.dw * inv_m;
+      const bool msk = L.msk != 0u;
+      const float d0 = L.oc0 - L.g0, d1 = L.oc1 - L.g1, d2 = L.oc2 - L.g2;
+      L.g0 = !msk ? 0.f : (d0 > 0.f ? kc : (d0 < 0.f ? -kc : 0.f));
+      L.g1 = !msk ? 0.f : (d1 > 0.f ? kc : (d1 < 0.f ? -kc : 0.f));
+      L.g2 = !msk ? 0.f : (d2 > 0.f ? kc : (d2 < 0.f ? -kc : 0.f));
+      const float g = L.gD, e = L.aux.y - g;
+      L.gD = (msk && L.owner != -1 && g > 0.f && e < lg.depth_thr) ? (e > 0.f ? kd : (e < 0.f ? -kd : 0.f)) : 0.f;
+    }
     EntryWalk W;
     W.n = n;
     W.last = inside ? L.last : 0u;
@@ -377,7 +402,16 @@
         const float rx = ((float)px - p.cx) / p.fx, ry = ((float)py - p.cy) / p.fy;
         uint32_t pl = pix;
         asm volatile("" : "+v"(pl));
-        if (reload) { gD = dL_ddepth[pl]; const float2 a2 = cached ? tc.depth_aux[pl] : make_float2(0.f, 0.f); iden = a2.x; Dd = a2.y; }
+        if (reload) {
+          if constexpr (LOSS) {
+            const float2 a2 = tc.depth_aux[pl];
+            const float e = a2.y - lg.gt_depth[pl];
+            gD = e > 0.f ? kd : (e < 0.f ? -kd : 0.f);
+            iden = a2.x; Dd = a2.y;
+          } else {
+            gD = dL_ddepth[pl]; const float2 a2 = cached ? tc.depth_aux[pl] : make_float2(0.f, 0.f); iden = a2.x; Dd = a2.y;
+          }
+        }
         if (!cached) {
           const int owner = depth_index[pl];
           const float4 r2 = reinterpret_cast<const float4*>(splats + owner)[2];
@@ -511,31 +545,37 @@
       const float *__restrict__ dL_ddepth, const uint32_t *__restrict__ gbase, uint32_t *__restrict__ slot_count,                    \
       const BwdInfo *__restrict__ info, SplatGrad *__restrict__ grads, uint8_t *__restrict__ touched,                               \
       const uint32_t *__restrict__ tile_mode, uint32_t t0, uint32_t tn, uint32_t dbg, unsigned long long *__restrict__ stamps,       \
-      TileCache tc, uint32_t pre
+      TileCache tc, uint32_t pre, LossGrad lg
 #define RTGS_BWD_PASS                                                                                                             \
   p, ranges, point_list, splats, out_color, n_contrib, depth_index, depth_pos, tile_last, dL_dcolor, dL_ddepth, gbase, slot_count, \
-      info, grads, touched, tile_mode, t0, tn, dbg, stamps, tc, pre
-__global__ void __launch_bounds__(256, 5) blend_bwd_entry_kernel(RTGS_BWD_ARGS) { blend_bwd_entry_body<false>(RTGS_BWD_PASS); }
-__global__ void __launch_bounds__(256, 5) blend_bwd_entry_stamped_kernel(RTGS_BWD_ARGS) { blend_bwd_entry_body<true>(RTGS_BWD_PASS); }
+      info, grads, touched, tile_mode, t0, tn, dbg, stamps, tc, pre, lg
+__global__ void __launch_bounds__(256, 5) blend_bwd_entry_kernel(RTGS_BWD_ARGS) { blend_bwd_entry_body<false, false>(RTGS_BWD_PASS); }
+__global__ void __launch_bounds__(256, 5) blend_bwd_entry_loss_kernel(RTGS_BWD_ARGS) { blend_bwd_entry_body<false, true>(RTGS_BWD_PASS); }
+__global__ void __launch_bounds__(256, 5) blend_bwd_entry_stamped_kernel(RTGS_BWD_ARGS) { blend_bwd_entry_body<true, false>(RTGS_BWD_PASS); }
+__global__ void __launch_bounds__(256, 5) blend_bwd_entry_loss_stamped_kernel(RTGS_BWD_ARGS) { blend_bwd_entry_body<true, true>(RTGS_BWD_PASS); }
 #undef RTGS_BWD_ARGS
 #undef RTGS_BWD_PASS
 
 static int g_bwd_dbg = 0;
 static unsigned long long* g_bwd_stamps = nullptr;
 void set_bwd_debug(int bits) { g_bwd_dbg = bits & 15; }
+bool bwd_entry_ignores_cache() { return (g_bwd_dbg & 8) != 0; }
 void set_bwd_stamps(void* dev) { g_bwd_stamps = (unsigned long long*)dev; }
 
 void launch_blend_bwd_entry(const RasterParams& p, const uint2* ranges, const uint32_t* point_list, const Splat* splats,
                             const float* out_color, const uint32_t* n_contrib, const int32_t* depth_index,
                             const uint32_t* depth_pos, const uint32_t* tile_last, const float* dL_dcolor, const float* dL_ddepth,
                             const uint32_t* gbase, uint32_t* slot_count, const BwdInfo* info, SplatGrad* grads, uint8_t* touched,
-                            const uint32_t* tile_mode, uint32_t t0, uint32_t tn, TileCache tc, uint32_t pre, hipStream_t st) {
+                            const uint32_t* tile_mode, uint32_t t0, uint32_t tn, TileCache tc, uint32_t pre, hipStream_t st,
+                            const LossGrad* fold) {
   const uint32_t dbg = (uint32_t)g_bwd_dbg;
+  const LossGrad lg = fold ? *fold : LossGrad{nullptr, nullptr, nullptr, nullptr, 0.f, 0.f, 0.f};
 #define RTGS_BWD_LAUNCH(KERNEL)                                                                                                      \
   hipLaunchKernelGGL(KERNEL, dim3(p.gx, p.gy), dim3(BLOCK), 0, st, p, ranges, point_list, splats, out_color, n_contrib, depth_index, \
                      depth_pos, tile_last, dL_dcolor, dL_ddepth, gbase, slot_count, info, grads, touched, tile_mode, t0, tn, dbg,    \
-                     g_bwd_stamps, tc, pre)
-  if (g_bwd_stamps) RTGS_BWD_LAUNCH(blend_bwd_entry_stamped_kernel); else RTGS_BWD_LAUNCH(blend_bwd_entry_kernel);
+                     g_bwd_stamps, tc, pre, lg)
+  if (fold) { if (g_bwd_stamps) RTGS_BWD_LAUNCH(blend_bwd_entry_loss_stamped_kernel); else RTGS_BWD_LAUNCH(blend_bwd_entry_loss_kernel); }
+  else if (g_bwd_stamps) RTGS_BWD_LAUNCH(blend_bwd_entry_stamped_kernel); else RTGS_BWD_LAUNCH(blend_bwd_entry_kernel);
 #undef RTGS_BWD_LAUNCH
 }
 
diff --git a/rtg_slam_amd/csrc/raster_common.h b/rtg_slam_amd/csrc/raster_common.h
--- a/rtg_slam_amd/csrc/raster_common.h
+++ b/rtg_slam_amd/csrc/raster_common.h
@@ -115,13 +115,34 @@
   size_t slot_grads;
 };
 struct ImgLayout {
-  size_t ranges, n_contrib, bwd_info, tile_mode, depth_pos, tile_last, tile_recs, tile_masks, depth_aux, total;
+  size_t ranges, n_contrib, bwd_info, tile_mode, depth_pos, tile_last, tile_recs, tile_masks, depth_aux, loss_part, total;
 };
 constexpr int TILE_RECS = 256;
 struct TileCache {
   float4* recs;
   uint16_t* masks;
   float2* depth_aux;
+};
+struct LossFold {
+  const float* gt_color;
+  const float* gt_depth;
+  const uint8_t* rmask;
+  float depth_thr;
+  float4* part;
+};
+struct LossReduce {
+  const float4* part;
+  int ntiles;
+  float* sums;
+  float* loss4;
+  float cw, dw;
+};
+struct LossGrad {
+  const float* gt_color;
+  const float* gt_depth;
+  const uint8_t* rmask;
+  const float* sums;
+  float depth_thr, cw, dw;
 };
 #ifndef RTGS_ROWS_MAX_SHARE
 #define RTGS_ROWS_MAX_SHARE 0.6f
diff --git a/rtg_slam_amd/csrc/raster_fwd.hip b/rtg_slam_amd/csrc/raster_fwd.hip
--- a/rtg_slam_amd/csrc/raster_fwd.hip
+++ b/rtg_slam_amd/csrc/raster_fwd.hip
@@ -258,7 +258,21 @@
 typedef float f4v __attribute__((ext_vector_type(4)));
 typedef float f2v __attribute__((ext_vector_type(2)));
 
-template <int OCC, bool STAMP, bool COUNT, bool ASMW>
+__device__ __forceinline__ float wave_sum_f32(float v) {
+  int x = __builtin_bit_cast(int, v);
+  const auto r = __builtin_amdgcn_permlane32_swap(x, x, false, false);
+  v = __builtin_bit_cast(float, (int)r[0]) + __builtin_bit_cast(float, (int)r[1]);
+  x = __builtin_bit_cast(int, v);
+  const auto q = __builtin_amdgcn_permlane16_swap(x, x, false, false);
+  v = __builtin_bit_cast(float, (int)q[0]) + __builtin_bit_cast(float, (int)q[1]);
+  v += __builtin_bit_cast(float, __builtin_amdgcn_update_dpp(0, __builtin_bit_cast(int, v), 0x128, 0xf, 0xf, false));
+  v += __builtin_bit_cast(float, __builtin_amdgcn_update_dpp(0, __builtin_bit_cast(int, v), 0x124, 0xf, 0xf, false));
+  v += __builtin_bit_cast(float, __builtin_amdgcn_update_dpp(0, __builtin_bit_cast(int, v), 0x122, 0xf, 0xf, false));
+  v += __builtin_bit_cast(float, __builtin_amdgcn_update_dpp(0, __builtin_bit_cast(int, v), 0x121, 0xf, 0xf, false));
+  return v;
+}
+
+template <int OCC, bool STAMP, bool COUNT, bool ASMW, bool LOSS>
 __global__ void __launch_bounds__(256, OCC) blend_fwd_kernel(
     RasterParams p, const uint2* __restrict__ ranges, const uint32_t* __restrict__ point_list,
     const Splat* __restrict__ splats, float* __restrict__ out_color, float* __restrict__ out_depth,
@@ -266,7 +280,7 @@
     float* __restrict__ out_dw, float* __restrict__ out_T, uint32_t* __restrict__ n_contrib,
     unsigned long long* __restrict__ counters, SlicePass sp, uint32_t* __restrict__ tile_mode,
     uint32_t* __restrict__ depth_pos, uint32_t* __restrict__ tile_last, int walk, uint32_t* __restrict__ aux_zero,
-    TileCache tc, unsigned long long* __restrict__ stamps, uint32_t seg) {
+    TileCache tc, unsigned long long* __restrict__ stamps, uint32_t seg, LossFold lf) {
   __shared__ float4 s_rec[FWD_BATCH * 4];
 #define RI(e, j) ((e) * 4 + (j))
   __shared__ float s_z[FWD_BATCH];
@@ -523,6 +537,29 @@
   }
 
   __shared__ uint32_t s_ep[4][4];
+  __shared__ float s_lp[4][4];
+  float o0 = 0.f, o1 = 0.f, o2 = 0.f;
+  if constexpr (LOSS) {
+    o0 = C0 + T * p.bg[0]; o1 = C1 + T * p.bg[1]; o2 = C2 + T * p.bg[2];
+    float l_c = 0.f, l_d = 0.f, l_m = 0.f, l_n = 0.f;
+    if (inside) {
+      const size_t pix = (size_t)py * p.W + px;
+      const size_t HW = (size_t)p.H * p.W;
+      const bool msk = lf.rmask == nullptr || lf.rmask[pix] != 0;
+      const float t0 = lf.gt_color[pix], t1 = lf.gt_color[HW + pix], t2 = lf.gt_color[2 * HW + pix];
+      const float g = lf.gt_depth[pix], e = D - g;
+      if (msk) {
+        l_n = 1.f;
+        l_c = fabsf(o0 - t0) + fabsf(o1 - t1) + fabsf(o2 - t2);
+        if (d_id != -1 && g > 0.f && e < lf.depth_thr) { l_d = fabsf(e); l_m = 1.f; }
+      }
+    }
+#pragma unroll
+    for (int off = 32; off > 0; off >>= 1) {
+      l_c += __shfl_xor(l_c, off); l_d += __shfl_xor(l_d, off); l_m += __shfl_xor(l_m, off); l_n += __shfl_xor(l_n, off);
+    }
+    if (lane == 0) { s_lp[wv][0] = l_c; s_lp[wv][1] = l_d; s_lp[wv][2] = l_m; s_lp[wv][3] = l_n; }
+  }
   {
     const uint32_t wl = wave_max_u32(last_contributor);
     const bool wave_done = ASMW ? (Dm == ~0ull) : (__builtin_amdgcn_ballot_w64(done) == ~0ull);
@@ -546,9 +583,10 @@
   if (inside && write_out) {
     const size_t pix = (size_t)py * p.W + px;
     const size_t HW = (size_t)p.H * p.W;
-    out_color[pix] = C0 + T * p.bg[0];
-    out_color[HW + pix] = C1 + T * p.bg[1];
-    out_color[2 * HW + pix] = C2 + T * p.bg[2];
+    if constexpr (!LOSS) { o0 = C0 + T * p.bg[0]; o1 = C1 + T * p.bg[1]; o2 = C2 + T * p.bg[2]; }
+    out_color[pix] = o0;
+    out_color[HW + pix] = o1;
+    out_color[2 * HW + pix] = o2;
     out_depth[pix] = D;
     out_cidx[pix] = best_id;
     out_didx[pix] = d_id;
@@ -564,6 +602,9 @@
     tile_mode[tile] = (walk >= 0 ? (uint32_t)walk : (share < ROWS_MAX_SHARE ? 1u : 0u)) | (tc.recs != nullptr ? 4u : 0u) |
                       ((uint32_t)(share * 1000.f) << 8);
     tile_last[tile] = tl_all;
+    if constexpr (LOSS)
+      lf.part[tile] = make_float4((s_lp[0][0] + s_lp[1][0]) + (s_lp[2][0] + s_lp[3][0]), (s_lp[0][1] + s_lp[1][1]) + (s_lp[2][1] + s_lp[3][1]),
+                                  (s_lp[0][2] + s_lp[1][2]) + (s_lp[2][2] + s_lp[3][2]), (s_lp[0][3] + s_lp[1][3]) + (s_lp[2][3] + s_lp[3][3]));
   }
   if (COUNT && counters) {
     __shared__ unsigned int s_max;
@@ -595,6 +636,7 @@
 static int g_f1_asm = [] { const char* e = getenv("RTGS_F1_ASM"); return e ? atoi(e) : 1; }();
 static unsigned long long* g_fwd_stamps = nullptr;
 void set_fwd_stamps(void* dev) { g_fwd_stamps = (unsigned long long*)dev; }
+bool blend_fwd_folds_loss(bool counters) { return g_f1_asm != 0 && !counters && g_f1_occ != 5; }
 
 void launch_mask_sat(const int32_t* mask, int gx, int gy, int32_t* sat, hipStream_t st) {
   hipLaunchKernelGGL(mask_sat_kernel, dim3(1), dim3(256), 0, st, mask, gx, gy, sat);
@@ -637,12 +679,54 @@
   if (R == 0) return;
   hipLaunchKernelGGL(tile_ranges_kernel, dim3((unsigned)((R + 255) / 256)), dim3(256), 0, st, R, keys, ranges);
 }
+template <int NT>
+__device__ __forceinline__ void loss_reduce_wg(const LossReduce& lr) {
+  constexpr int LR_PRE = 4096 / NT;
+  float4 v[LR_PRE];
+#pragma unroll
+  for (int j = 0; j < LR_PRE; ++j) {
+    const int t = (int)threadIdx.x + j * NT;
+    v[j] = t < lr.ntiles ? lr.part[t] : make_float4(0.f, 0.f, 0.f, 0.f);
+  }
+  float a0 = 0.f, a1 = 0.f, a2 = 0.f, a3 = 0.f;
+#pragma unroll
+  for (int j = 0; j < LR_PRE; ++j) { a0 += v[j].x; a1 += v[j].y; a2 += v[j].z; a3 += v[j].w; }
+  for (int t = (int)threadIdx.x + LR_PRE * NT; t < lr.ntiles; t += NT) {
+    const float4 w = lr.part[t];
+    a0 += w.x; a1 += w.y; a2 += w.z; a3 += w.w;
+  }
+  a0 = wave_sum_f32(a0); a1 = wave_sum_f32(a1); a2 = wave_sum_f32(a2); a3 = wave_sum_f32(a3);
+  __shared__ float s_lr[NT / 64][4];
+  if ((threadIdx.x & 63) == 0) { float* o = s_lr[threadIdx.x >> 6]; o[0] = a0; o[1] = a1; o[2] = a2; o[3] = a3; }
+  __syncthreads();
+  if (threadIdx.x == 0) {
+    float t[4];
+#pragma unroll
+    for (int k = 0; k < 4; ++k) {
+      t[k] = 0.f;
+#pragma unroll
+      for (int w = 0; w < NT / 64; ++w) t[k] += s_lr[w][k];
+    }
+    lr.sums[0] = t[0]; lr.sums[1] = t[1]; lr.sums[2] = t[2]; lr.sums[3] = t[3]; lr.sums[4] = 0.f;
+    const float inv_c = 1.f / (3.f * fmaxf(t[3], 1.f));
+    const float inv_m = 1.f / fmaxf(t[2], 1.f);
+    const float lc = t[0] * inv_c, ld = t[1] * inv_m, ls = 0.f;
+    lr.loss4[1] = lc; lr.loss4[2] = ld; lr.loss4[3] = ls;
+    lr.loss4[0] = lr.dw * ld + lr.cw * lc;
+  }
+}
+__global__ void __launch_bounds__(1024) loss_reduce_kernel(LossReduce lr) { loss_reduce_wg<1024>(lr); }
+void launch_loss_reduce(const LossReduce& lr, hipStream_t st) {
+  if (lr.part) hipLaunchKernelGGL(loss_reduce_kernel, dim3(1), dim3(1024), 0, st, lr);
+}
+
 __global__ void __launch_bounds__(256) slice_publish_kernel(int ntiles, const int32_t* __restrict__ user_mask,
                                                             const int32_t* __restrict__ mask2,
                                                             const uint32_t* __restrict__ r1, uint32_t* __restrict__ ctr,
                                                             uint32_t* __restrict__ host, uint32_t seq,
                                                             uint32_t* __restrict__ spec_fail,
-                                                            const uint32_t* __restrict__ seg_count) {
+                                                            const uint32_t* __restrict__ seg_count, LossReduce lr) {
+  if (lr.part) loss_reduce_wg<256>(lr);
   int left = 0, fin = 0, inst = 0;
   for (int t = threadIdx.x; t < ntiles; t += 256) {
     const bool on = user_mask[t] != 0, l = mask2[t] != 0;
@@ -665,23 +749,26 @@
   }
 }
 void launch_slice_publish(int ntiles, const int32_t* user_mask, const int32_t* mask2, const uint32_t* r1, uint32_t* ctr,
-                          uint32_t* host, uint32_t seq, uint32_t* spec_fail, hipStream_t st, const uint32_t* seg_count) {
+                          uint32_t* host, uint32_t seq, uint32_t* spec_fail, hipStream_t st, const uint32_t* seg_count,
+                          const LossReduce* lr) {
   hipLaunchKernelGGL(slice_publish_kernel, dim3(1), dim3(256), 0, st, ntiles, user_mask, mask2, r1, ctr, host, seq, spec_fail,
-                     seg_count);
+                     seg_count, lr ? *lr : LossReduce{nullptr, 0, nullptr, nullptr, 0.f, 0.f});
 }
 
 void launch_blend_fwd(const RasterParams& p, const uint2* ranges, const uint32_t* point_list, const Splat* splats,
                       float* out_color, float* out_depth, int32_t* out_cidx, int32_t* out_didx, float* out_cw,
                       float* out_dw, float* out_T, uint32_t* n_contrib, unsigned long long* counters,
                       SlicePass sp, uint32_t* tile_mode, uint32_t* depth_pos, uint32_t* tile_last, int walk, uint32_t* aux_zero,
-                      TileCache tc, uint32_t seg, hipStream_t st) {
-#define RTGS_FWD1(OCC, STAMP, COUNT, ASMW) hipLaunchKernelGGL((blend_fwd_kernel<OCC, STAMP, COUNT, ASMW>), dim3(p.gx, p.gy), dim3(BLOCK), 0, st, p, ranges, point_list, splats, \
+                      TileCache tc, uint32_t seg, hipStream_t st, const LossFold* fold) {
+  const LossFold lf = fold ? *fold : LossFold{nullptr, nullptr, nullptr, 0.f, nullptr};
+#define RTGS_FWD1(OCC, STAMP, COUNT, ASMW, LOSS) hipLaunchKernelGGL((blend_fwd_kernel<OCC, STAMP, COUNT, ASMW, LOSS>), dim3(p.gx, p.gy), dim3(BLOCK), 0, st, p, ranges, point_list, splats, \
                        out_color, out_depth, out_cidx, out_didx, out_cw, out_dw, out_T, n_contrib, counters, sp, tile_mode, \
-                       depth_pos, tile_last, walk, aux_zero, tc, g_fwd_stamps, seg)
-  if (g_f1_asm == 0) RTGS_FWD1(6, false, true, false);
-  else if (counters) RTGS_FWD1(6, false, true, true);
-  else if (g_fwd_stamps) RTGS_FWD1(6, true, false, true);
-  else if (g_f1_occ == 5) RTGS_FWD1(5, false, false, true); else RTGS_FWD1(6, false, false, true);
+                       depth_pos, tile_last, walk, aux_zero, tc, g_fwd_stamps, seg, lf)
+  if (lf.part != nullptr) { if (g_fwd_stamps) RTGS_FWD1(6, true, false, true, true); else RTGS_FWD1(6, false, false, true, true); }
+  else if (g_f1_asm == 0) RTGS_FWD1(6, false, true, false, false);
+  else if (counters) RTGS_FWD1(6, false, true, true, false);
+  else if (g_fwd_stamps) RTGS_FWD1(6, true, false, true, false);
+  else if (g_f1_occ == 5) RTGS_FWD1(5, false, false, true, false); else RTGS_FWD1(6, false, false, true, false);
 #undef RTGS_FWD1
 }
 
diff --git a/rtg_slam_amd/map_optim.py b/rtg_slam_amd/map_optim.py
--- a/rtg_slam_amd/map_optim.py
+++ b/rtg_slam_amd/map_optim.py
@@ -209,6 +209,7 @@
         self._cap_peak, self._cap_steps, self._shrink_every = 0, 0, 32
         self._act_valid = False
         self.tail_mode = 1 if __import__("os").environ.get("RTGS_TAIL_MODE", "0") == "1" else 0
+        self.loss_mode = 0
         self.live_counts = torch.zeros(2, dtype=torch.int32, device=self.device) if packed.is_cuda else None
         self._mode = None
 
@@ -700,7 +701,8 @@
             C.pointer(attach) if attach is not None else None, P(confidence) if confidence is not None else None,
             int(self._act_valid), geom.cb, None, binning.cb, None, img.cb, None,
             float(normal_weight) if gt_normal is not None else 0.0, P(gt_normal) if gt_normal is not None else None,
-            int(nf), int(N), int(self.tail_mode), P(self.live_counts) if self.live_counts is not None else None)
+            int(nf), int(N), int(self.tail_mode), P(self.live_counts) if self.live_counts is not None else None,
+            int(self.loss_mode))
         R = C.c_int64(0)
         stream = torch.cuda.current_stream(dev).cuda_stream
         if tile_band and self.world > 1:
```
